# zijieli-Jlee/Temporal-Pointcloud-Upsampling-GAN

Measured on AMD Instinct MI355X. Metric: GAN train-steps/sec (G+D) on 4096-pt x3-frame clips, higher is better.
Workload: dtype bf16; 1 GPU; cfg2: 4096-pt x3-frame fluid clips, full G+D adversarial step (SRNet(3,128) + FluidTempoDis(3) + FluidSpatialDis, Adam), all-keep mask regime, gate open, even iteration; batch 8 per GPU; per_gpu_batch=8, global_batch=8, parallelism=dp1, step_mode=hipgraph (1 graph per step)

## Files before the change

include/tpgan_ops.h:

```cpp
#ifndef TPGAN_OPS_H
#define TPGAN_OPS_H

#include <stddef.h>
#include <stdint.h>

#ifdef __cplusplus
extern "C" {
#endif

typedef enum {
    TPG_OK = 0,
    TPG_ERR_ARG = -1,
    TPG_ERR_LAUNCH = -2,
    TPG_ERR_UNSUPPORTED = -3
} tpg_status;

#define TPG_MAX_K 64

const char *tpg_version(void);
const char *tpg_target_arch(void);

int tpg_knn_f32(const float *p1, const float *p2, const int64_t *len1,
                const int64_t *len2, int B, int P1, int P2, int D, int K,
                float r2, float *dist, int64_t *idx, void *stream);

int tpg_knn_grid_f32(const float *p1, const float *p2, const int64_t *len1, const int64_t *len2, int B,
                     int P1, int P2, int K, float *dist, int64_t *idx, void *ws, void *stream);

int tpg_knn_mfma_f32(const float *p1, const float *p2, const int64_t *len1,
                     const int64_t *len2, int B, int P1, int P2, int D, int K,
                     float *dist, int64_t *idx, int redo, void *stream);

size_t tpg_frnn_grid_workspace_bytes(int B, int P2);
int tpg_frnn_grid_f32(const float *p1, const float *p2, const int64_t *len1, const int64_t *len2, int B, int P1,
                      int P2, int K, float r, float *dist, int64_t *idx, void *ws, void *stream);

int tpg_chamfer_fwd_f32(const float *src, const float *tgt, int B, int N, int M,
                        float *d1, int64_t *i1, float *d2, int64_t *i2,
                        void *stream);
size_t tpg_chamfer_bwd_workspace_bytes(int B, int N, int M);
int tpg_chamfer_bwd_f32(const float *src, const float *tgt, int B, int N, int M,
                        const int64_t *i1, const int64_t *i2, const float *g1,
                        const float *g2, float *gsrc, float *gtgt, void *ws, void *stream);

int tpg_fps_f32(const float *xyz, int B, int N, int m, float *temp, int32_t *idx,
                void *stream);

int tpg_fps_prefix_f32(const float *xyz, int B, int N, int m, float *temp, int32_t *idx,
                       const int32_t *prefix_in, int32_t *prefix_out, void *stream);

int tpg_fps_start_f32(const float *xyz, const int32_t *start, int skip_origin, int B, int N, int m,
                      float *temp, int32_t *idx, void *stream);

int tpg_gather_fwd_f32(const float *feat, const int32_t *idx, int B, int C, int N,
                       int S, float *out, void *stream);
int tpg_gather_bwd_f32(const float *gout, const int32_t *idx, int B, int C, int N,
                       int S, float *gfeat, void *stream);

int tpg_gather_rows_fwd_f32(const float *rows, const int32_t *idx, int B, int N, int S, int C, float *out, void *stream);
int tpg_gather_rows_bwd_f32(const float *gout, const int32_t *idx, int B, int N, int S, int C, float *grows,
                            void *stream);

int tpg_ball_query_f32(const float *xyz, const float *new_xyz, int B, int N, int S,
                       float radius, int nsample, int32_t *idx, void *stream);

int tpg_group_fwd_f32(const float *feat, const int32_t *idx, int B, int C, int N,
                      int S, int K, float *out, void *stream);
int tpg_group_bwd_f32(const float *gout, const int32_t *idx, int B, int C, int N,
                      int S, int K, float *gfeat, void *stream);

int tpg_three_nn_f32(const float *unknown, const float *known, int B, int n, int m,
                     float *dist2, int32_t *idx, void *stream);
int tpg_three_interp_fwd_f32(const float *feat, const int32_t *idx, const float *w,
                             int B, int C, int m, int n, float *out, void *stream);
int tpg_three_interp_bwd_f32(const float *gout, const int32_t *idx, const float *w,
                             int B, int C, int m, int n, float *gfeat,
                             void *stream);

typedef enum { TPG_DTYPE_F32 = 0, TPG_DTYPE_BF16 = 1 } tpg_dtype;

int tpg_rowcombine_fwd(const void *U, const void *QE, const int32_t *idx, int mode, int dtype_in,
                       int dtype_out, int B, int N, int S, int K, int C, float slope, void *out,
                       void *stream);

int tpg_invert_index(const int32_t *idx, int B, int N, int SK, int32_t *offs, int32_t *list,
                     int32_t *tmp, void *stream);

int tpg_rowcombine_bwd(const void *gout, const int32_t *idx, const int32_t *offs, const int32_t *list,
                       const void *E, int mode, int dtype_in, int dtype_out, int B, int N, int S, int K,
                       int C, float slope, void *gU, void *gQE, void *stream);

int tpg_rowcombine_edge_fwd(const void *Y, const int32_t *idx, int dtype_in, int dtype_out, int B, int N, int K, int C,
                            float slope_a, float slope_e, void *out, void *stream);
int tpg_rowcombine_edge_bwd(const void *gout, const int32_t *idx, const int32_t *offs, const int32_t *list,
                            const void *Y, int dtype_in, int dtype_out, int B, int N, int K, int C, float slope_a,
                            float slope_e, void *gY, void *stream);

int tpg_head_bn_act_fwd(const float *h, int B, int C, const float *gamma, const float *beta, float *running_mean,
                        float *running_var, long long *num_batches_tracked, float momentum, float eps, float slope,
                        const float *mask, float *y, float *mean, float *rstd, void *stream);
int tpg_head_bn_act_bwd(const float *gy, const float *h, const float *mean, const float *rstd, const float *gamma,
                        const float *beta, float slope, const float *mask, int B, int C, float *dh, float *dgamma,
                        float *dbeta, void *stream);

#define TPG_BN_PHASE_ALL 0
#define TPG_BN_PHASE_STATS 1
#define TPG_BN_PHASE_APPLY 2
size_t tpg_rowbn_workspace_bytes(int C, int nseg);
int tpg_rowbn_fwd(const void *x, int dtype_in, long long P, int K, int C, float eps, float momentum,
                  int training, float *running_mean, float *running_var, long long *num_batches_tracked,
                  const float *mean_shift, const float *gamma, const float *beta, float slope, float *mean,
                  float *rstd, void *y,
                  int dtype_out, uint8_t *argmax, void *ws, int nseg, int phase, void *stream);
int tpg_rowbn_bwd(const void *gy, int dtype_g, const void *x, int dtype_in, const uint8_t *argmax,
                  const void *y, int dtype_y, long long P, int K, int C, int training, const float *mean,
                  const float *rstd, const float *gamma, const float *beta, float slope, float *dgamma,
                  float *dbeta, void *dx, void *ws, int nseg, int phase, void *stream);

int tpg_rowbn_bwd_sums(const void *gy, int dtype_g, const void *x, int dtype_in, const uint8_t *argmax,
                       const void *y, int dtype_y, long long P, int K, int C, int training, const float *mean,
                       const float *rstd, const float *gamma, const float *beta, float slope, float *dgamma,
                       float *dbeta, float *c12, void *ws, int nseg, void *stream);

int tpg_rowbn_stats_consts(const void *x, int dtype_in, long long P, int C, float eps, float momentum,
                           float *running_mean, float *running_var, long long *num_batches_tracked,
                           const float *mean_shift, const float *gamma, const float *beta, float *mean, float *rstd,
                           float *ci, void *ws, int nseg, void *stream);
int tpg_rowbn_bwd_sums_consts(const void *gy, int dtype_g, const void *x, int dtype_in, const uint8_t *argmax,
                              const void *y, int dtype_y, long long P, int K, int C, int training, const float *mean,
                              const float *rstd, const float *gamma, const float *beta, float slope, float *dgamma,
                              float *dbeta, float *c12, float *cb, void *ag, void *ws, int nseg, void *stream);

size_t tpg_mlp_workspace_bytes(int C, int nseg);
int tpg_mlp_fwd(const void *x, long long P, int Cin, int Cout, int nseg, const float *ss_in, int ss_stride,
                float slope_in, const float *W, int w_per_seg, void *y, float eps, float momentum,
                float *running_mean, float *running_var, long long *num_batches_tracked, const float *mean_shift,
                const float *gamma_out, const float *beta_out, float *mean_out, float *rstd_out, float *ci_out,
                void *ws, void *stream);

int tpg_mlp_consts(const float *mean, const float *rstd, const float *gamma, const float *beta, const float *c12,
                   int C, int nseg, float *ci, float *cb, void *stream);
int tpg_mlp_max_prep(const void *gout, const void *y, const float *cb_out, float slope_out, long long rows, int C,
                     int nseg, void *ag, void *stream);
int tpg_mlp_dgrad(const void *x_out, const void *g_out, const uint8_t *arg, int K, const float *cb_out,
                  const void *x_in, const float *ci_in, float slope_in, const float *W,
                  int w_per_seg, long long P, int Cin, int Cout, int nseg, int mode, void *g_in, float *c12_in,
                  float *dgamma_in, float *dbeta_in, float *cb_in, void *ws, void *stream);
size_t tpg_mlp_wgrad_workspace_bytes(long long P, int Cin, int Cout, int nseg);
int tpg_mlp_wgrad(const void *x_out, const void *g_out, const uint8_t *arg, int K, const float *cb_out,
                  const void *x_in, const float *ci_in, float slope_in, long long P, int Cin,
                  int Cout, int nseg, int mode, float *dW, void *ws, void *stream);
int tpg_mlp_bn_bwd_apply(const void *g, const void *x, const float *ci, const float *c12, long long P, int C,
                         int nseg, void *dx, void *stream);
int tpg_mlp_bn_bwd_apply_rowsum(const void *g, const void *x, const float *ci, const float *c12, long long P, int K,
                                int C, int nseg, void *dx, float *qneg, void *stream);

int tpg_spectral_norm_fwd(const float *W, float *u, float *v, int R, int Cn, int iterate, float eps,
                          float *Wsn, float *sigma, void *stream);
int tpg_spectral_norm_bwd(const float *G, const float *Wsn, const float *u, const float *v,
                          const float *sigma, int R, int Cn, float *dW, void *stream);

long long tpg_spectral_norm_multi_stride(int R, int Cn);
int tpg_spectral_norm_multi_fwd(const void *desc, int M, int max_rc, float *out, int iterate, float eps,
                                void *stream);
int tpg_spectral_norm_multi_fwd_split(const void *desc, const void *part_map, int total_parts, int max_cn, float *out,
                                      void *xws, long long xws_words, float eps, void *stream);
int tpg_spectral_norm_split_rows(void);
int tpg_spectral_norm_split_max_cn(void);
int tpg_spectral_norm_split_max_rows(void);
long long tpg_spectral_norm_multi_bwd_scratch(int M, int max_uses);
int tpg_spectral_norm_multi_bwd(const void *desc, int M, int max_uses, const float *g, const float *out,
                                float *dw, float *scratch, void *stream);

int tpg_cubic_interp_f32(const float *query, const float *pos, const float *field, int B, int Nq, int Np,
                         int F, float cutoff, float *out_plain, float *out_pad, int32_t *hits,
                         void *stream);

size_t tpg_small_tail_workspace_bytes(long long P, int K);
int tpg_small_tail_fwd(const void *h, int is_bf16, const float *W1, const float *W2, float slope1, float slope2,
                       long long P, int K, int H, int C1, int C2, void *out, unsigned char *arg, void *stream);
int tpg_small_tail_bwd(const void *h, const void *out, const void *gout, const unsigned char *arg, int is_bf16,
                       const float *W1, const float *W2, float slope1, float slope2, long long P, int K, int H,
                       int C1, int C2, void *gh, float *dW1, float *dW2, void *ws, void *stream);

int tpg_rowlinear_supported(int Cin, int Cout, int has_bias);
size_t tpg_rowlinear_wgrad_workspace_bytes(long long P, int nseg, int Cin, int Cout, int has_bias);
int tpg_rowlinear_fwd(const void *x, int dtype_in, const float *W, const float *bias, long long P, int nseg, int Cin,
                      int Cout, float slope, void *y, int dtype_out, void *stream);
int tpg_rowlinear_dgrad(const void *gy, const void *y, int dtype_g, const float *W, long long P, int nseg, int Cin,
                        int Cout, float slope, void *dx, int dtype_x, void *stream);
int tpg_rowlinear_wgrad(const void *x, int dtype_x, const void *gy, const void *y, int dtype_g, long long P, int nseg,
                        int Cin, int Cout, float slope, float *dW, float *db, void *ws, void *stream);

#define TPG_CTX_NONE (-2147483647 - 1)
size_t tpg_context_expand_workspace_bytes(int T, int N);
int tpg_context_expand_f32(const float *pos, const float *edge, const float *mask, int T, int N, int r, int t0,
                           int32_t *state, float *out, int64_t *offsets, void *ws, void *stream);

int tpg_radius_reduce_f32(const float *query, const float *pos, const int64_t *lenq, const int64_t *lenp, int B,
                          int Nq, int Np, float r, int kernel, int32_t *count, float *sum, void *ws, void *stream);
int tpg_radius_reduce_exhaustive_f32(const float *query, const float *pos, const int64_t *lenq, const int64_t *lenp,
                                     int B, int Nq, int Np, float r, int kernel, int32_t *count, float *sum,
                                     void *stream);

#define TPG_PATCH_SELECT_MAX_K 16384
int tpg_patch_select_max_k(void);
size_t tpg_patch_select_workspace_bytes(int B, int max_count, int K);
int tpg_patch_select_f32(const float *points, long long P, const int32_t *first, const int32_t *count,
                         const int32_t *seed, int B, int K, int32_t *idx, void *ws, void *stream);

int tpg_clip_gather_high_f32(const float *pos, const float *vel, long long P, const int32_t *frame_first,
                             const int32_t *count, const float *centroids, int F, const int32_t *centroid_row,
                             const int32_t *patch, int T, int B, int K, float *high_pos, float *high_vel, void *stream);

int tpg_clip_gather_low_f32(const float *high_pos, const int32_t *fps, const float *noise, float jitter,
                            const float *vel, long long P, const int32_t *frame_first, const int32_t *count, int T,
                            int B, int K, int M, float *low_pos, float *low_vel, void *stream);

#ifdef __cplusplus
}
#endif
#endif
```

temporal-pointcloud-upsampling-gan_amd/_lib.py:

```python
import ctypes as C
import os

_HERE = os.path.dirname(os.path.abspath(__file__))
LIB_PATH = os.environ.get("TPGAN_HIP_LIBRARY") or os.path.join(_HERE, "csrc", "libtpgan_hip.so")

_P = C.c_void_p
_I = C.c_int
_F = C.c_float
_L = C.c_longlong

SIGNATURES = {
    "tpg_knn_f32": [_P, _P, _P, _P, _I, _I, _I, _I, _I, _F, _P, _P, _P],
    "tpg_knn_mfma_f32": [_P, _P, _P, _P, _I, _I, _I, _I, _I, _P, _P, _I, _P],
    "tpg_knn_grid_f32": [_P, _P, _P, _P, _I, _I, _I, _I, _P, _P, _P, _P],
    "tpg_frnn_grid_f32": [_P, _P, _P, _P, _I, _I, _I, _I, _F, _P, _P, _P, _P],
    "tpg_chamfer_fwd_f32": [_P, _P, _I, _I, _I, _P, _P, _P, _P, _P],
    "tpg_chamfer_bwd_f32": [_P, _P, _I, _I, _I, _P, _P, _P, _P, _P, _P, _P, _P],
    "tpg_fps_f32": [_P, _I, _I, _I, _P, _P, _P],
    "tpg_fps_prefix_f32": [_P, _I, _I, _I, _P, _P, _P, _P, _P],
    "tpg_fps_start_f32": [_P, _P, _I, _I, _I, _I, _P, _P, _P],
    "tpg_gather_fwd_f32": [_P, _P, _I, _I, _I, _I, _P, _P],
    "tpg_gather_bwd_f32": [_P, _P, _I, _I, _I, _I, _P, _P],
    "tpg_ball_query_f32": [_P, _P, _I, _I, _I, _F, _I, _P, _P],
    "tpg_group_fwd_f32": [_P, _P, _I, _I, _I, _I, _I, _P, _P],
    "tpg_group_bwd_f32": [_P, _P, _I, _I, _I, _I, _I, _P, _P],
    "tpg_three_nn_f32": [_P, _P, _I, _I, _I, _P, _P, _P],
    "tpg_three_interp_fwd_f32": [_P, _P, _P, _I, _I, _I, _I, _P, _P],
    "tpg_three_interp_bwd_f32": [_P, _P, _P, _I, _I, _I, _I, _P, _P],
    "tpg_gather_rows_fwd_f32": [_P, _P, _I, _I, _I, _I, _P, _P],
    "tpg_gather_rows_bwd_f32": [_P, _P, _I, _I, _I, _I, _P, _P],
    "tpg_rowcombine_fwd": [_P, _P, _P, _I, _I, _I, _I, _I, _I, _I, _I, _F, _P, _P],
    "tpg_invert_index": [_P, _I, _I, _I, _P, _P, _P, _P],
    "tpg_rowcombine_bwd": [_P, _P, _P, _P, _P, _I, _I, _I, _I, _I, _I, _I, _I, _F, _P, _P, _P],
    "tpg_rowcombine_edge_fwd": [_P, _P, _I, _I, _I, _I, _I, _I, _F, _F, _P, _P],
    "tpg_rowcombine_edge_bwd": [_P, _P, _P, _P, _P, _I, _I, _I, _I, _I, _I, _F, _F, _P, _P],
    "tpg_head_bn_act_fwd": [_P, _I, _I, _P, _P, _P, _P, _P, _F, _F, _F, _P, _P, _P, _P, _P],
    "tpg_head_bn_act_bwd": [_P, _P, _P, _P, _P, _P, _F, _P, _I, _I, _P, _P, _P, _P],
    "tpg_rowbn_fwd": [_P, _I, _L, _I, _I, _F, _F, _I, _P, _P, _P, _P, _P, _P, _F, _P, _P, _P, _I, _P, _P, _I, _I, _P],
    "tpg_rowbn_bwd": [_P, _I, _P, _I, _P, _P, _I, _L, _I, _I, _I, _P, _P, _P, _P, _F, _P, _P, _P, _P, _I, _I, _P],
    "tpg_cubic_interp_f32": [_P, _P, _P, _I, _I, _I, _I, _F, _P, _P, _P, _P],
    "tpg_spectral_norm_fwd": [_P, _P, _P, _I, _I, _I, _F, _P, _P, _P],
    "tpg_spectral_norm_bwd": [_P, _P, _P, _P, _P, _I, _I, _P, _P],
    "tpg_spectral_norm_multi_fwd": [_P, _I, _I, _P, _I, _F, _P],
    "tpg_spectral_norm_multi_fwd_split": [_P, _P, _I, _I, _P, _P, _L, _F, _P],
    "tpg_spectral_norm_multi_bwd": [_P, _I, _I, _P, _P, _P, _P, _P],
    "tpg_rowbn_bwd_sums": [_P, _I, _P, _I, _P, _P, _I, _L, _I, _I, _I, _P, _P, _P, _P, _F, _P, _P, _P, _P, _I, _P],
    "tpg_rowbn_bwd_sums_consts": [_P, _I, _P, _I, _P, _P, _I, _L, _I, _I, _I, _P, _P, _P, _P, _F, _P, _P, _P, _P, _P, _P, _I, _P],
    "tpg_rowbn_stats_consts": [_P, _I, _L, _I, _F, _F, _P, _P, _P, _P, _P, _P, _P, _P, _P, _P, _I, _P],
    "tpg_mlp_consts": [_P, _P, _P, _P, _P, _I, _I, _P, _P, _P],
    "tpg_mlp_max_prep": [_P, _P, _P, _F, _L, _I, _I, _P, _P],
    "tpg_mlp_dgrad": [_P, _P, _P, _I, _P, _P, _P, _F, _P, _I, _L, _I, _I, _I, _I, _P, _P, _P, _P, _P, _P, _P],
    "tpg_mlp_wgrad": [_P, _P, _P, _I, _P, _P, _P, _F, _L, _I, _I, _I, _I, _P, _P, _P],
    "tpg_mlp_bn_bwd_apply": [_P, _P, _P, _P, _L, _I, _I, _P, _P],
    "tpg_mlp_bn_bwd_apply_rowsum": [_P, _P, _P, _P, _L, _I, _I, _I, _P, _P, _P],
    "tpg_small_tail_fwd": [_P, _I, _P, _P, _F, _F, _L, _I, _I, _I, _I, _P, _P, _P],
    "tpg_small_tail_bwd": [_P, _P, _P, _P, _I, _P, _P, _F, _F, _L, _I, _I, _I, _I, _P, _P, _P, _P, _P],
    "tpg_rowlinear_fwd": [_P, _I, _P, _P, _L, _I, _I, _I, _F, _P, _I, _P],
    "tpg_rowlinear_dgrad": [_P, _P, _I, _P, _L, _I, _I, _I, _F, _P, _I, _P],
    "tpg_rowlinear_wgrad": [_P, _I, _P, _P, _I, _L, _I, _I, _I, _F, _P, _P, _P, _P],
    "tpg_mlp_fwd": [_P, _L, _I, _I, _I, _P, _I, _F, _P, _I, _P, _F, _F, _P, _P, _P, _P, _P, _P, _P, _P, _P, _P, _P],
    "tpg_context_expand_f32": [_P, _P, _P, _I, _I, _I, _I, _P, _P, _P, _P, _P],
    "tpg_radius_reduce_f32": [_P, _P, _P, _P, _I, _I, _I, _F, _I, _P, _P, _P, _P],
    "tpg_radius_reduce_exhaustive_f32": [_P, _P, _P, _P, _I, _I, _I, _F, _I, _P, _P, _P],
    "tpg_patch_select_f32": [_P, _L, _P, _P, _P, _I, _I, _P, _P, _P],
    "tpg_clip_gather_high_f32": [_P, _P, _L, _P, _P, _P, _I, _P, _P, _I, _I, _I, _P, _P, _P],
    "tpg_clip_gather_low_f32": [_P, _P, _P, _F, _P, _L, _P, _P, _I, _I, _I, _I, _P, _P, _P],
}
SIZE_GETTERS = ("tpg_rowbn_workspace_bytes", "tpg_mlp_workspace_bytes", "tpg_context_expand_workspace_bytes")
OTHER_GETTERS = ("tpg_spectral_norm_multi_stride", "tpg_spectral_norm_multi_bwd_scratch",
                 "tpg_mlp_wgrad_workspace_bytes", "tpg_frnn_grid_workspace_bytes", "tpg_small_tail_workspace_bytes",
                 "tpg_chamfer_bwd_workspace_bytes", "tpg_rowlinear_wgrad_workspace_bytes", "tpg_rowlinear_supported",
                 "tpg_spectral_norm_split_rows", "tpg_spectral_norm_split_max_cn", "tpg_spectral_norm_split_max_rows",
                 "tpg_patch_select_workspace_bytes", "tpg_patch_select_max_k")
STRING_GETTERS = ("tpg_version", "tpg_target_arch")

STATUS = {0: "TPG_OK", -1: "TPG_ERR_ARG", -2: "TPG_ERR_LAUNCH", -3: "TPG_ERR_UNSUPPORTED"}

_lib = None


class HipLibraryMissing(RuntimeError):
    pass


def load():
    global _lib
    if _lib is not None:
        return _lib
    if not os.path.exists(LIB_PATH):
        raise HipLibraryMissing(
            f"{LIB_PATH} not found: build it with `python __graft_entry__.py` "
            "(hipcc --offload-arch=gfx950).  There is no CPU fallback.")
    lib = C.CDLL(LIB_PATH)
    for name, argtypes in SIGNATURES.items():
        fn = getattr(lib, name)
        fn.argtypes = argtypes
        fn.restype = C.c_int
    for name in STRING_GETTERS:
        getattr(lib, name).restype = C.c_char_p
    for name in SIZE_GETTERS:
        getattr(lib, name).argtypes = [C.c_int, C.c_int]
        getattr(lib, name).restype = C.c_size_t
    lib.tpg_spectral_norm_multi_stride.argtypes = [C.c_int, C.c_int]
    lib.tpg_spectral_norm_multi_stride.restype = C.c_longlong
    lib.tpg_spectral_norm_multi_bwd_scratch.argtypes = [C.c_int, C.c_int]
    lib.tpg_spectral_norm_multi_bwd_scratch.restype = C.c_longlong
    lib.tpg_mlp_wgrad_workspace_bytes.argtypes = [C.c_longlong, C.c_int, C.c_int, C.c_int]
    lib.tpg_mlp_wgrad_workspace_bytes.restype = C.c_size_t
    lib.tpg_small_tail_workspace_bytes.argtypes = [C.c_longlong, C.c_int]
    lib.tpg_small_tail_workspace_bytes.restype = C.c_size_t
    lib.tpg_frnn_grid_workspace_bytes.argtypes = [C.c_int, C.c_int]
    lib.tpg_frnn_grid_workspace_bytes.restype = C.c_size_t
    lib.tpg_chamfer_bwd_workspace_bytes.argtypes = [C.c_int, C.c_int, C.c_int]
    lib.tpg_chamfer_bwd_workspace_bytes.restype = C.c_size_t
    lib.tpg_rowlinear_wgrad_workspace_bytes.argtypes = [C.c_longlong, C.c_int, C.c_int, C.c_int, C.c_int]
    lib.tpg_rowlinear_wgrad_workspace_bytes.restype = C.c_size_t
    lib.tpg_patch_select_workspace_bytes.argtypes = [C.c_int, C.c_int, C.c_int]
    lib.tpg_patch_select_workspace_bytes.restype = C.c_size_t
    for name in ("tpg_spectral_norm_split_rows", "tpg_spectral_norm_split_max_cn", "tpg_spectral_norm_split_max_rows",
                 "tpg_patch_select_max_k"):
        getattr(lib, name).argtypes = []
        getattr(lib, name).restype = C.c_int
    lib.tpg_rowlinear_supported.argtypes = [C.c_int, C.c_int, C.c_int]
    lib.tpg_rowlinear_supported.restype = C.c_int
    _lib = lib
    return lib


def check(rc, name):
    if rc != 0:
        raise RuntimeError(f"{name} failed: {STATUS.get(rc, rc)}")
```

temporal-pointcloud-upsampling-gan_amd/csrc/mlp_fused.hip:

```cpp
#include "tpg_bn_finalize.hpp"
#include "tpg_rows.hpp"

namespace {

typedef __attribute__((ext_vector_type(8))) short bf16x8;

constexpr int ML_THREADS = 256;
constexpr int ML_WAVES = ML_THREADS / 64;
constexpr int ML_MAX_BLOCKS = 512;
constexpr int ML_WPAD = 8;

template <int COUT> __device__ __forceinline__ int w_lds_row(int n) {
    constexpr int T = COUT / 16;
    return (n % T) * 16 + n / T;
}

template <int CIN, int COUT, int STRIPS>
__global__ __launch_bounds__(ML_THREADS, 2) void mlp_fwd_kernel(
    const __hip_bfloat16 *__restrict__ x, long long P, const float *__restrict__ ss, int ss_stride, float slope,
    const float *__restrict__ W, int w_per_seg, __hip_bfloat16 *__restrict__ y, float *__restrict__ part) {
    constexpr int T = COUT / 16;
    constexpr int KS = CIN / 32;
    constexpr int BM = ML_WAVES * STRIPS * 16;
    constexpr int WROW = CIN + ML_WPAD;
    extern __shared__ __attribute__((aligned(16))) unsigned char ml_smem[];
    unsigned short *wl = reinterpret_cast<unsigned short *>(ml_smem);
    float *cst = reinterpret_cast<float *>(ml_smem + (size_t)COUT * WROW * 2);
    float *red = reinterpret_cast<float *>(ml_smem);
    const int tid = threadIdx.x, lane = tid & 63, wave = tid >> 6;
    const int li = lane & 15, lq = lane >> 4;
    const int seg = blockIdx.y;
    x += (size_t)seg * P * CIN;
    y += (size_t)seg * P * COUT;
    {
        const float *Ws = W + (w_per_seg ? (size_t)seg * COUT * CIN : 0);
        for (int e = tid; e < COUT * CIN / 4; e += ML_THREADS) {
            const int n = e / (CIN / 4), k = (e - n * (CIN / 4)) * 4;
            const float4 w4 = *reinterpret_cast<const float4 *>(Ws + (size_t)n * CIN + k);
            uint2 p;
            p.x = tpg_pack_bf16x2(w4.x, w4.y);
            p.y = tpg_pack_bf16x2(w4.z, w4.w);
            *reinterpret_cast<uint2 *>(wl + (size_t)w_lds_row<COUT>(n) * WROW + k) = p;
        }
        for (int c = tid; c < 2 * CIN; c += ML_THREADS)
            cst[c] = ss ? ss[(size_t)seg * ss_stride + c] : (c < CIN ? 1.0f : 0.0f);
    }
    __syncthreads();
    float piv[T], s1[T], s2[T];
#pragma unroll
    for (int t = 0; t < T; ++t) { piv[t] = 0.0f; s1[t] = 0.0f; s2[t] = 0.0f; }
    bool have_piv = false;
    float nrows = 0.0f;
    const long long ntiles = (P + BM - 1) / BM;
    const unsigned short *wfrag = wl + (size_t)li * WROW + 8 * lq;
    const float *csc = cst + 8 * lq, *csh = cst + CIN + 8 * lq;
    uint4 araw[STRIPS][KS];
    auto load_tile = [&](long long tile) {
#pragma unroll
        for (int st = 0; st < STRIPS; ++st) {
            long long row = tile * BM + (wave * STRIPS + st) * 16 + li;
            row = row < P ? row : P - 1;
            const __hip_bfloat16 *px = x + (size_t)row * CIN + 8 * lq;
#pragma unroll
            for (int s = 0; s < KS; ++s) araw[st][s] = *reinterpret_cast<const uint4 *>(px + 32 * s);
        }
    };
    long long tile = blockIdx.x;
    if (tile < ntiles) load_tile(tile);
    for (; tile < ntiles; tile += gridDim.x) {
        const long long row_base = tile * BM + (long long)wave * STRIPS * 16;
        tpg_f32x4 acc[STRIPS][T];
#pragma unroll
        for (int st = 0; st < STRIPS; ++st)
#pragma unroll
            for (int t = 0; t < T; ++t) acc[st][t] = tpg_f32x4{0.0f, 0.0f, 0.0f, 0.0f};
#pragma unroll
        for (int s = 0; s < KS; ++s) {
            float sc[8], sh[8];
            {
                const float4 a0 = *reinterpret_cast<const float4 *>(csc + 32 * s), a1 = *reinterpret_cast<const float4 *>(csc + 32 * s + 4);
                const float4 b0 = *reinterpret_cast<const float4 *>(csh + 32 * s), b1 = *reinterpret_cast<const float4 *>(csh + 32 * s + 4);
                sc[0] = a0.x; sc[1] = a0.y; sc[2] = a0.z; sc[3] = a0.w; sc[4] = a1.x; sc[5] = a1.y; sc[6] = a1.z; sc[7] = a1.w;
                sh[0] = b0.x; sh[1] = b0.y; sh[2] = b0.z; sh[3] = b0.w; sh[4] = b1.x; sh[5] = b1.y; sh[6] = b1.z; sh[7] = b1.w;
            }
            bf16x8 afrag[STRIPS];
#pragma unroll
            for (int st = 0; st < STRIPS; ++st) {
                const unsigned w[4] = {araw[st][s].x, araw[st][s].y, araw[st][s].z, araw[st][s].w};
                union { unsigned u[4]; bf16x8 v; } cv;
#pragma unroll
                for (int i = 0; i < 4; ++i) {
                    float a = __builtin_fmaf(tpg_bf16_lo(w[i]), sc[2 * i], sh[2 * i]);
                    float b = __builtin_fmaf(tpg_bf16_hi(w[i]), sc[2 * i + 1], sh[2 * i + 1]);
                    a = fmaxf(a, a * slope);
                    b = fmaxf(b, b * slope);
                    cv.u[i] = tpg_pack_bf16x2(a, b);
                }
                afrag[st] = cv.v;
            }
#pragma unroll
            for (int t = 0; t < T; ++t) {
                const bf16x8 b = *reinterpret_cast<const bf16x8 *>(wfrag + (size_t)t * 16 * WROW + 32 * s);
#pragma unroll
                for (int st = 0; st < STRIPS; ++st)
                    acc[st][t] = __builtin_amdgcn_mfma_f32_16x16x32_bf16(afrag[st], b, acc[st][t], 0, 0, 0);
                if ((t & 3) == 3) __builtin_amdgcn_sched_barrier(0);
            }
        }
        if (tile + gridDim.x < ntiles) load_tile(tile + gridDim.x);
        if (!have_piv) {
#pragma unroll
            for (int t = 0; t < T; ++t) {
                const float v = tpg_bf16_lo(tpg_pack_bf16x2(acc[0][t][0], 0.0f));
                piv[t] = __shfl(v, li, 64);
            }
            have_piv = true;
        }
#pragma unroll
        for (int st = 0; st < STRIPS; ++st)
#pragma unroll
            for (int r = 0; r < 4; ++r) {
                const long long row = row_base + st * 16 + 4 * lq + r;
                const bool valid = row < P;
                unsigned o[T / 2];
#pragma unroll
                for (int t = 0; t < T; t += 2) {
                    const unsigned w = tpg_pack_bf16x2(acc[st][t][r], acc[st][t + 1][r]);
                    o[t / 2] = w;
                    const float d0 = valid ? tpg_bf16_lo(w) - piv[t] : 0.0f;
                    const float d1 = valid ? tpg_bf16_hi(w) - piv[t + 1] : 0.0f;
                    s1[t] += d0;
                    s1[t + 1] += d1;
                    s2[t] = __builtin_fmaf(d0, d0, s2[t]);
                    s2[t + 1] = __builtin_fmaf(d1, d1, s2[t + 1]);
                }
                if (valid) {
                    __hip_bfloat16 *py = y + (size_t)row * COUT + li * T;
#pragma unroll
                    for (int v4 = 0; v4 < T / 8; ++v4)
                        reinterpret_cast<uint4 *>(py)[v4] = make_uint4(o[4 * v4], o[4 * v4 + 1], o[4 * v4 + 2], o[4 * v4 + 3]);
                    if constexpr (T == 4) *reinterpret_cast<uint2 *>(py) = make_uint2(o[0], o[1]);
                }
            }
        {
            const long long left = P - row_base;
            nrows += (float)(left <= 0 ? 0 : (left < STRIPS * 16 ? left : STRIPS * 16));
        }
    }
#pragma unroll
    for (int t = 0; t < T; ++t) {
        s1[t] += __shfl_xor(s1[t], 16, 64);
        s1[t] += __shfl_xor(s1[t], 32, 64);
        s2[t] += __shfl_xor(s2[t], 16, 64);
        s2[t] += __shfl_xor(s2[t], 32, 64);
    }
    __syncthreads();
    if (lq == 0) {
#pragma unroll
        for (int t = 0; t < T; ++t) {
            const int c = li * T + t;
            const float n = nrows;
            const float m = n > 0.0f ? s1[t] / n : 0.0f;
            red[(wave * 3 + 0) * COUT + c] = piv[t] + m;
            red[(wave * 3 + 1) * COUT + c] = n > 0.0f ? s2[t] - s1[t] * m : 0.0f;
            red[(wave * 3 + 2) * COUT + c] = n;
        }
    }
    __syncthreads();
    float *out = part + ((size_t)seg * gridDim.x + blockIdx.x) * 3 * COUT;
    for (int c = tid; c < COUT; c += ML_THREADS) {
        float n = 0.0f, mean = 0.0f, m2 = 0.0f;
#pragma unroll
        for (int w = 0; w < ML_WAVES; ++w) {
            const float nw = red[(w * 3 + 2) * COUT + c];
            if (nw > 0.0f) {
                const float mw = red[(w * 3 + 0) * COUT + c], qw = red[(w * 3 + 1) * COUT + c];
                const float tot = n + nw, delta = mw - mean;
                mean += delta * (nw / tot);
                m2 += qw + delta * delta * (n * nw / tot);
                n = tot;
            }
        }
        out[c] = mean;
        out[COUT + c] = m2;
        out[2 * COUT + c] = n;
    }
}

using tpg_bn::FIN_CH;
using tpg_bn::FIN_THREADS;
using tpg_bn::FIN_R;

__global__ __launch_bounds__(FIN_THREADS) void mlp_stats_finalize_kernel(
    const float *__restrict__ part, int G, int C, int nseg, float eps, float momentum,
    float *__restrict__ running_mean, float *__restrict__ running_var, long long *__restrict__ num_batches_tracked,
    const float *__restrict__ mean_shift, const float *__restrict__ gamma, const float *__restrict__ beta,
    float *__restrict__ mean, float *__restrict__ rstd, float *__restrict__ ci_out) {
    const int lane = threadIdx.x & 63;
    const int c = blockIdx.x * FIN_CH + (threadIdx.x >> 6);
    if (num_batches_tracked && blockIdx.x == 0 && threadIdx.x == 0) *num_batches_tracked += nseg;
    if (c >= C) return;
    const tpg_bn::Split sp = tpg_bn::split(nseg);
    const int grp = lane / sp.L, sub = lane - grp * sp.L;
    const bool fits = G <= sp.L * FIN_R;
    float rmean = running_mean ? running_mean[c] : 0.0f, rvar = running_mean ? running_var[c] : 0.0f;
    const double shift = mean_shift ? (double)mean_shift[c] : 0.0;
    for (int seg0 = 0; seg0 < nseg; seg0 += sp.SP) {
        const int seg = seg0 + grp;
        const bool live = seg < nseg;
        const float *ps = part + (size_t)(live ? seg : nseg - 1) * G * 3 * C + c;
        float pn[FIN_R], pm[FIN_R], pq[FIN_R];
        auto fetch = [&](int g0) {
#pragma unroll
            for (int i = 0; i < FIN_R; ++i) {
                const int g = g0 + sub + i * sp.L;
                const bool ok = live && g < G;
                const float *pg = ps + (size_t)(ok ? g : 0) * 3 * C;
                const float m_ = pg[0], q_ = pg[C], n_ = pg[2 * C];
                pm[i] = m_;
                pq[i] = q_;
                pn[i] = ok ? n_ : 0.0f;
            }
        };
        double n = 0.0, sm = 0.0;
        for (int g0 = 0; g0 < G; g0 += sp.L * FIN_R) {
            fetch(g0);
#pragma unroll
            for (int i = 0; i < FIN_R; ++i) {
                n += (double)pn[i];
                sm += (double)pn[i] * (double)pm[i];
            }
        }
        const double N = tpg_bn::group_sum(n, sp.L);
        const double m = N > 0.0 ? tpg_bn::group_sum(sm, sp.L) / N : 0.0;
        double q = 0.0;
        for (int g0 = 0; g0 < G; g0 += sp.L * FIN_R) {
            if (!fits) fetch(g0);
#pragma unroll
            for (int i = 0; i < FIN_R; ++i) {
                const double d = (double)pm[i] - m;
                q += pn[i] > 0.0f ? (double)pq[i] + (double)pn[i] * d * d : 0.0;
            }
        }
        double var = N > 0.0 ? tpg_bn::group_sum(q, sp.L) / N : 0.0;
        var = var < 0.0 ? 0.0 : var;
        const float mu = (float)m, rs = (float)(1.0 / sqrt(var + (double)eps));
        if (live && sub == 0) {
            if (mean) mean[(size_t)seg * C + c] = mu;
            if (rstd) rstd[(size_t)seg * C + c] = rs;
            if (ci_out) {
                const float a = (gamma ? gamma[c] : 1.0f) * rs;
                tpg_bn::write_ci(ci_out + (size_t)seg * 4 * C + c, C, a, beta ? beta[c] : 0.0f, mu, rs);
            }
        }
        if (running_mean) {
            const int last = nseg - seg0 < sp.SP ? nseg - seg0 : sp.SP;
            for (int k = 0; k < last; ++k) {
                const double Nk = tpg_bn::readlane(N, k * sp.L), mk = tpg_bn::readlane(m, k * sp.L), vk = tpg_bn::readlane(var, k * sp.L);
                const double unbiased = Nk > 1.0 ? vk * Nk / (Nk - 1.0) : vk;
                rmean = (float)((1.0 - momentum) * rmean + momentum * (mk + shift));
                rvar = (float)((1.0 - momentum) * rvar + momentum * unbiased);
            }
        }
    }
    if (running_mean && lane == 0) { running_mean[c] = rmean; running_var[c] = rvar; }
}

enum { MODE_DENSE = 0, MODE_MAX = 1 };

__device__ __forceinline__ void ld8(const float *p, float (&v)[8]) {
    const float4 a = *reinterpret_cast<const float4 *>(p), b = *reinterpret_cast<const float4 *>(p + 4);
    v[0] = a.x; v[1] = a.y; v[2] = a.z; v[3] = a.w; v[4] = b.x; v[5] = b.y; v[6] = b.z; v[7] = b.w;
}

template <int MODE>
__device__ __forceinline__ void d_out8(const uint4 xr, const uint4 gr, const uint2 ar, int k, const float (&a)[8],
                                       const float (&f)[8], const float (&fm)[8], unsigned (&o)[4]) {
    const unsigned xw[4] = {xr.x, xr.y, xr.z, xr.w}, gw[4] = {gr.x, gr.y, gr.z, gr.w};
#pragma unroll
    for (int i = 0; i < 4; ++i) {
        float v[2];
#pragma unroll
        for (int h = 0; h < 2; ++h) {
            const int j = 2 * i + h;
            const float x = h ? tpg_bf16_hi(xw[i]) : tpg_bf16_lo(xw[i]);
            const float g = h ? tpg_bf16_hi(gw[i]) : tpg_bf16_lo(gw[i]);
            const float c = __builtin_fmaf(-f[j], x, fm[j]);
            if (MODE == MODE_MAX) {
                const int ak = (int)__builtin_amdgcn_ubfe(j < 4 ? ar.x : ar.y, 8 * (j & 3), 8);
                v[h] = c + (ak == k ? g : 0.0f);
            } else {
                v[h] = __builtin_fmaf(a[j], g, c);
            }
        }
        o[i] = tpg_pack_bf16x2(v[0], v[1]);
    }
}

__global__ void mlp_max_prep_kernel(const __hip_bfloat16 *__restrict__ g, const __hip_bfloat16 *__restrict__ y,
                                    const float *__restrict__ cb, float slope, long long rows, int C,
                                    __hip_bfloat16 *__restrict__ ag) {
    const int seg = blockIdx.y;
    const long long n8 = rows * C / 8;
    const float *a = cb + (size_t)seg * 4 * C;
    for (long long i = (long long)blockIdx.x * blockDim.x + threadIdx.x; i < n8; i += (long long)gridDim.x * blockDim.x) {
        const size_t off = (size_t)seg * rows * C + (size_t)i * 8;
        const int c = (int)((i * 8) % C);
        const uint4 gv = *reinterpret_cast<const uint4 *>(g + off), yv = *reinterpret_cast<const uint4 *>(y + off);
        const unsigned gw[4] = {gv.x, gv.y, gv.z, gv.w}, yw[4] = {yv.x, yv.y, yv.z, yv.w};
        float av[8];
        ld8(a + c, av);
        unsigned o[4];
#pragma unroll
        for (int q = 0; q < 4; ++q) {
            const float g0 = tpg_bf16_lo(gw[q]), g1 = tpg_bf16_hi(gw[q]);
            const float v0 = av[2 * q] * (tpg_bf16_lo(yw[q]) > 0.0f ? g0 : g0 * slope);
            const float v1 = av[2 * q + 1] * (tpg_bf16_hi(yw[q]) > 0.0f ? g1 : g1 * slope);
            o[q] = tpg_pack_bf16x2(v0, v1);
        }
        *reinterpret_cast<uint4 *>(ag + off) = make_uint4(o[0], o[1], o[2], o[3]);
    }
}

template <int CIN, int COUT, int MODE, int STRIPS, int OCC>
__global__ __launch_bounds__(ML_THREADS, OCC) void mlp_dgrad_kernel(
    const __hip_bfloat16 *__restrict__ x_out, const __hip_bfloat16 *__restrict__ g_out,
    const uint8_t *__restrict__ arg, int K, const float *__restrict__ cbo,
    const __hip_bfloat16 *__restrict__ x_in, const float *__restrict__ cbi, float slope_in,
    const float *__restrict__ W, int w_per_seg, long long P, __hip_bfloat16 *__restrict__ g_in,
    float *__restrict__ part) {
    constexpr int TI = CIN / 16;
    constexpr int KS = COUT / 32;
    constexpr int BM = ML_WAVES * STRIPS * 16;
    constexpr int WROW = COUT + ML_WPAD;
    extern __shared__ __attribute__((aligned(16))) unsigned char ml_smem[];
    unsigned short *wl = reinterpret_cast<unsigned short *>(ml_smem);
    float *cst = reinterpret_cast<float *>(ml_smem + (size_t)CIN * WROW * 2);
    float *bias = cst + 4 * COUT;
    float *red = bias + CIN;
    const int tid = threadIdx.x, lane = tid & 63, wave = tid >> 6;
    const int li = lane & 15, lq = lane >> 4;
    const int seg = blockIdx.y;
    x_out += (size_t)seg * P * COUT;
    x_in += (size_t)seg * P * CIN;
    g_in += (size_t)seg * P * CIN;
    if (MODE == MODE_DENSE) g_out += (size_t)seg * P * COUT;
    else { g_out += (size_t)seg * (P / K) * COUT; arg += (size_t)seg * (P / K) * COUT; }
    {
        const float *Ws = W + (w_per_seg ? (size_t)seg * COUT * CIN : 0);
        for (int e = tid; e < COUT * CIN / 4; e += ML_THREADS) {
            const int n = e / (CIN / 4), k = (e - n * (CIN / 4)) * 4;
            const float4 w4 = *reinterpret_cast<const float4 *>(Ws + (size_t)n * CIN + k);
            const float wv[4] = {w4.x, w4.y, w4.z, w4.w};
#pragma unroll
            for (int i = 0; i < 4; ++i) wl[(size_t)w_lds_row<CIN>(k + i) * WROW + n] = tpg_bf16_bits(wv[i]);
        }
        const float *cb = cbo + (size_t)seg * 4 * COUT;
        for (int c = tid; c < COUT; c += ML_THREADS) {
            cst[c] = cb[c];
            cst[COUT + c] = cb[3 * COUT + c];
            cst[2 * COUT + c] = cb[2 * COUT + c];
            cst[3 * COUT + c] = cb[COUT + c];
        }
    }
    __syncthreads();
    for (int ci = tid; ci < CIN; ci += ML_THREADS) {
        const unsigned short *wr = wl + (size_t)w_lds_row<CIN>(ci) * WROW;
        float acc = 0.0f;
        for (int co = 0; co < COUT; ++co) acc = __builtin_fmaf(cst[2 * COUT + co], __uint_as_float((unsigned)wr[co] << 16), acc);
        bias[ci] = acc;
    }
    __syncthreads();
    float sc[TI], sh[TI], mu[TI], bi[TI], sg[TI], sgx[TI];
#pragma unroll
    for (int t = 0; t < TI; ++t) {
        const int c = li * TI + t;
        sc[t] = cbi[((size_t)seg * 4 + 0) * CIN + c];
        sh[t] = cbi[((size_t)seg * 4 + 1) * CIN + c];
        mu[t] = cbi[((size_t)seg * 4 + 2) * CIN + c];
        bi[t] = bias[c];
        sg[t] = 0.0f;
        sgx[t] = 0.0f;
    }
    const long long ntiles = (P + BM - 1) / BM;
    const unsigned short *wfrag = wl + (size_t)li * WROW + 8 * lq;
    uint4 xraw[STRIPS][KS], graw[STRIPS][KS];
    uint2 araw[STRIPS][KS];
    unsigned xin[STRIPS][4][TI / 2];
    constexpr bool DEFER = OCC == 1 && CIN == 128;
    unsigned xnext[DEFER ? STRIPS : 1][4][TI / 2];
    unsigned held[DEFER ? STRIPS : 1][4][TI / 2];
    long long held_base = -1;
    auto load_xin = [&](long long tile, unsigned (&xin)[STRIPS][4][TI / 2]) {
#pragma unroll
        for (int st = 0; st < STRIPS; ++st) {
#pragma unroll
            for (int r = 0; r < 4; ++r) {
                long long rr = tile * BM + (wave * STRIPS + st) * 16 + 4 * lq + r;
                rr = rr < P ? rr : P - 1;
                const __hip_bfloat16 *pi = x_in + (size_t)rr * CIN + li * TI;
                if constexpr (TI == 4) {
                    const uint2 v = *reinterpret_cast<const uint2 *>(pi);
                    xin[st][r][0] = v.x; xin[st][r][1] = v.y;
                } else {
#pragma unroll
                    for (int v4 = 0; v4 < TI / 8; ++v4) {
                        const uint4 v = reinterpret_cast<const uint4 *>(pi)[v4];
                        xin[st][r][4 * v4] = v.x; xin[st][r][4 * v4 + 1] = v.y; xin[st][r][4 * v4 + 2] = v.z; xin[st][r][4 * v4 + 3] = v.w;
                    }
                }
            }
        }
    };
    const __hip_bfloat16 *px[STRIPS], *pg[STRIPS];
    const uint8_t *pa[STRIPS];
    auto point_at = [&](long long tile) {
#pragma unroll
        for (int st = 0; st < STRIPS; ++st) {
            long long row = tile * BM + (wave * STRIPS + st) * 16 + li;
            row = row < P ? row : P - 1;
            px[st] = x_out + (size_t)row * COUT + 8 * lq;
            const long long grow = MODE == MODE_MAX ? (long long)((unsigned)row / (unsigned)K) : row;
            pg[st] = g_out + (size_t)grow * COUT + 8 * lq;
            pa[st] = MODE == MODE_MAX ? arg + (size_t)grow * COUT + 8 * lq : nullptr;
        }
    };
    auto load_step = [&](int st, int s) {
        xraw[st][s] = *reinterpret_cast<const uint4 *>(px[st] + 32 * s);
        graw[st][s] = *reinterpret_cast<const uint4 *>(pg[st] + 32 * s);
        if (MODE == MODE_MAX) araw[st][s] = *reinterpret_cast<const uint2 *>(pa[st] + 32 * s);
        else araw[st][s] = make_uint2(0u, 0u);
    };
    long long tile = blockIdx.x;
    if (tile < ntiles) {
        point_at(tile);
#pragma unroll
        for (int st = 0; st < STRIPS; ++st)
#pragma unroll
            for (int s = 0; s < KS; ++s) load_step(st, s);
        load_xin(tile, xin);
    }
    for (; tile < ntiles; tile += gridDim.x) {
        const long long row_base = tile * BM + (long long)wave * STRIPS * 16;
        const bool has_next = tile + gridDim.x < ntiles;
        const long long tnext = has_next ? tile + gridDim.x : tile;
        point_at(tnext);
        if constexpr (DEFER) load_xin(tnext, xnext);
        auto store_held = [&]() {
#pragma unroll
            for (int st = 0; st < STRIPS; ++st)
#pragma unroll
                for (int r = 0; r < 4; ++r) {
                    const long long row = held_base + st * 16 + 4 * lq + r;
                    if (row < P) {
                        __hip_bfloat16 *pgo = g_in + (size_t)row * CIN + li * TI;
#pragma unroll
                        for (int v4 = 0; v4 < TI / 8; ++v4)
                            reinterpret_cast<uint4 *>(pgo)[v4] = make_uint4(held[DEFER ? st : 0][r][4 * v4], held[DEFER ? st : 0][r][4 * v4 + 1],
                                                                            held[DEFER ? st : 0][r][4 * v4 + 2], held[DEFER ? st : 0][r][4 * v4 + 3]);
                    }
                }
        };
        tpg_f32x4 acc[STRIPS][TI];
#pragma unroll
        for (int st = 0; st < STRIPS; ++st)
#pragma unroll
            for (int t = 0; t < TI; ++t) acc[st][t] = tpg_f32x4{0.0f, 0.0f, 0.0f, 0.0f};
#pragma unroll
        for (int s = 0; s < KS; ++s) {
            float ca[8], cf[8], cfm[8];
            if (MODE == MODE_DENSE) ld8(cst + 32 * s + 8 * lq, ca);
            ld8(cst + COUT + 32 * s + 8 * lq, cf);
            ld8(cst + 3 * COUT + 32 * s + 8 * lq, cfm);
            bf16x8 afrag[STRIPS];
#pragma unroll
            for (int st = 0; st < STRIPS; ++st) {
                const long long row = row_base + st * 16 + li;
                union { unsigned u[4]; bf16x8 v; } cv;
                d_out8<MODE>(xraw[st][s], graw[st][s], araw[st][s], MODE == MODE_MAX ? (int)((unsigned)row % (unsigned)K) : 0, ca,
                             cf, cfm, cv.u);
                if (row >= P) { cv.u[0] = 0u; cv.u[1] = 0u; cv.u[2] = 0u; cv.u[3] = 0u; }
                afrag[st] = cv.v;
                load_step(st, s);
            }
#pragma unroll
            for (int t = 0; t < TI; ++t) {
                const bf16x8 b = *reinterpret_cast<const bf16x8 *>(wfrag + (size_t)t * 16 * WROW + 32 * s);
#pragma unroll
                for (int st = 0; st < STRIPS; ++st)
                    acc[st][t] = __builtin_amdgcn_mfma_f32_16x16x32_bf16(afrag[st], b, acc[st][t], 0, 0, 0);
                if ((t & 3) == 3) __builtin_amdgcn_sched_barrier(0);
            }
            if constexpr (DEFER) {
                if (s == 0 && held_base >= 0) store_held();
            }
        }
#pragma unroll
        for (int st = 0; st < STRIPS; ++st)
#pragma unroll
            for (int r = 0; r < 4; ++r) {
                const long long row = row_base + st * 16 + 4 * lq + r;
                const bool valid = row < P;
                const float vm = valid ? 1.0f : 0.0f;
                unsigned o[TI / 2];
#pragma unroll
                for (int t = 0; t < TI; t += 2) {
                    const float x0 = tpg_bf16_lo(xin[st][r][t / 2]), x1 = tpg_bf16_hi(xin[st][r][t / 2]);
                    const float z0 = __builtin_fmaf(x0, sc[t], sh[t]), z1 = __builtin_fmaf(x1, sc[t + 1], sh[t + 1]);
                    const float g0 = (acc[st][t][r] + bi[t]) * (z0 > 0.0f ? vm : vm * slope_in);
                    const float g1 = (acc[st][t + 1][r] + bi[t + 1]) * (z1 > 0.0f ? vm : vm * slope_in);
                    o[t / 2] = tpg_pack_bf16x2(g0, g1);
                    sg[t] += g0;
                    sg[t + 1] += g1;
                    sgx[t] = __builtin_fmaf(g0, x0 - mu[t], sgx[t]);
                    sgx[t + 1] = __builtin_fmaf(g1, x1 - mu[t + 1], sgx[t + 1]);
                }
                if constexpr (DEFER) {
#pragma unroll
                    for (int w = 0; w < TI / 2; ++w) held[st][r][w] = o[w];
                } else if (valid) {
                    __hip_bfloat16 *pgo = g_in + (size_t)row * CIN + li * TI;
#pragma unroll
                    for (int v4 = 0; v4 < TI / 8; ++v4)
                        reinterpret_cast<uint4 *>(pgo)[v4] = make_uint4(o[4 * v4], o[4 * v4 + 1], o[4 * v4 + 2], o[4 * v4 + 3]);
                    if constexpr (TI == 4) *reinterpret_cast<uint2 *>(pgo) = make_uint2(o[0], o[1]);
                }
            }
        if constexpr (DEFER) {
            held_base = row_base;
#pragma unroll
            for (int st = 0; st < STRIPS; ++st)
#pragma unroll
                for (int r = 0; r < 4; ++r)
#pragma unroll
                    for (int w = 0; w < TI / 2; ++w) xin[st][r][w] = xnext[st][r][w];
        } else {
            load_xin(tnext, xin);
        }
    }
    if constexpr (DEFER) {
        if (held_base >= 0) {
            auto store_last = [&]() {
#pragma unroll
                for (int st = 0; st < STRIPS; ++st)
#pragma unroll
                    for (int r = 0; r < 4; ++r) {
                        const long long row = held_base + st * 16 + 4 * lq + r;
                        if (row < P) {
                            __hip_bfloat16 *pgo = g_in + (size_t)row * CIN + li * TI;
#pragma unroll
                            for (int v4 = 0; v4 < TI / 8; ++v4)
                                reinterpret_cast<uint4 *>(pgo)[v4] = make_uint4(held[st][r][4 * v4], held[st][r][4 * v4 + 1], held[st][r][4 * v4 + 2], held[st][r][4 * v4 + 3]);
                        }
                    }
            };
            store_last();
        }
    }
#pragma unroll
    for (int t = 0; t < TI; ++t) {
        sg[t] += __shfl_xor(sg[t], 16, 64);
        sg[t] += __shfl_xor(sg[t], 32, 64);
        sgx[t] += __shfl_xor(sgx[t], 16, 64);
        sgx[t] += __shfl_xor(sgx[t], 32, 64);
    }
    if (lq == 0) {
#pragma unroll
        for (int t = 0; t < TI; ++t) {
            red[(wave * 2 + 0) * CIN + li * TI + t] = sg[t];
            red[(wave * 2 + 1) * CIN + li * TI + t] = sgx[t];
        }
    }
    __syncthreads();
    float *out = part + ((size_t)seg * gridDim.x + blockIdx.x) * 2 * CIN;
    for (int c = tid; c < 2 * CIN; c += ML_THREADS) {
        float v = 0.0f;
#pragma unroll
        for (int w = 0; w < ML_WAVES; ++w) v += red[w * 2 * CIN + c];
        out[c] = v;
    }
}

__global__ __launch_bounds__(FIN_THREADS) void mlp_bwd_finalize_kernel(const float *__restrict__ part, int G, long long P,
                                                                      int C, int nseg, const float *__restrict__ rstd,
                                                                      int rstd_stride, float *__restrict__ c12,
                                                                      float *__restrict__ dgamma,
                                                                      float *__restrict__ dbeta,
                                                                      const float *__restrict__ ci,
                                                                      float *__restrict__ cb) {
    const int lane = threadIdx.x & 63;
    const int c = blockIdx.x * FIN_CH + (threadIdx.x >> 6);
    if (c >= C) return;
    const tpg_bn::Split sp = tpg_bn::split(nseg);
    const int grp = lane / sp.L, sub = lane - grp * sp.L;
    double ts = 0.0, tsx = 0.0;
    for (int seg0 = 0; seg0 < nseg; seg0 += sp.SP) {
        const int seg = seg0 + grp;
        const bool live = seg < nseg;
        const int segc = live ? seg : nseg - 1;
        const float *ps = part + (size_t)segc * G * 2 * C + c;
        const float rs = rstd[(size_t)segc * rstd_stride + c];
        double s, sx;
        tpg_bn::pair_sums(ps, C, sub, sp.L, G, live, s, sx);
        sx *= (double)rs;
        const bool owner = live && sub == 0;
        ts += tpg_bn::wave_sum(owner ? s : 0.0);
        tsx += tpg_bn::wave_sum(owner ? sx : 0.0);
        if (owner) {
            const float c1 = (float)(s / (double)P), c2 = (float)(sx / (double)P);
            if (c12) {
                c12[((size_t)seg * 2 + 0) * C + c] = c1;
                c12[((size_t)seg * 2 + 1) * C + c] = c2;
            }
            if (cb) {
                const float *ip = ci + (size_t)seg * 4 * C + c;
                tpg_bn::write_cb(cb + (size_t)seg * 4 * C + c, C, ip[0], ip[2 * C], ip[3 * C], c1, c2);
            }
        }
    }
    if (lane == 0) {
        if (dbeta) dbeta[c] = (float)ts;
        if (dgamma) dgamma[c] = (float)tsx;
    }
}

__global__ void mlp_consts_kernel(const float *__restrict__ mean, const float *__restrict__ rstd,
                                  const float *__restrict__ gamma, const float *__restrict__ beta,
                                  const float *__restrict__ c12, int C, int nseg, float *__restrict__ ci,
                                  float *__restrict__ cb) {
    const int i = blockIdx.x * blockDim.x + threadIdx.x;
    if (i >= nseg * C) return;
    const int seg = i / C, c = i - seg * C;
    const float mu = mean[i], rs = rstd[i];
    const float a = (gamma ? gamma[c] : 1.0f) * rs;
    const float be = beta ? beta[c] : 0.0f;
    if (ci) tpg_bn::write_ci(ci + (size_t)seg * 4 * C + c, C, a, be, mu, rs);
    if (cb) {
        const float c1 = c12[((size_t)seg * 2 + 0) * C + c], c2 = c12[((size_t)seg * 2 + 1) * C + c];
        tpg_bn::write_cb(cb + (size_t)seg * 4 * C + c, C, a, mu, rs, c1, c2);
    }
}

constexpr int WG_ROWS = 64;
constexpr int WG_PAD = 8;

__device__ __forceinline__ bf16x8 tr_frag(const unsigned short *tile, int row_stride, int r0, int c0, int lane) {
    typedef __attribute__((ext_vector_type(4))) short s4;
    const int i = lane & 15, q = i >> 2, p = i & 3;
    const unsigned short *a0 = tile + (size_t)(r0 + q) * row_stride + c0 + 4 * p;
    const s4 lo = __builtin_amdgcn_ds_read_tr16_b64_v4i16((__attribute__((address_space(3))) s4 *)(a0));
    const s4 hi = __builtin_amdgcn_ds_read_tr16_b64_v4i16((__attribute__((address_space(3))) s4 *)(a0 + 4 * row_stride));
    bf16x8 f;
    f[0] = lo[0]; f[1] = lo[1]; f[2] = lo[2]; f[3] = lo[3];
    f[4] = hi[0]; f[5] = hi[1]; f[6] = hi[2]; f[7] = hi[3];
    return f;
}

template <int CIN, int COUT, int MODE, int OCC>
__global__ __launch_bounds__(ML_THREADS, OCC) void mlp_wgrad_kernel(
    const __hip_bfloat16 *__restrict__ x_out, const __hip_bfloat16 *__restrict__ g_out,
    const uint8_t *__restrict__ arg, int K, const float *__restrict__ cbo,
    const __hip_bfloat16 *__restrict__ x_in, const float *__restrict__ cbi, float slope_in, long long P,
    float *__restrict__ slab) {
    constexpr int MT = COUT / 16 / ML_WAVES;
    constexpr int NT = CIN / 16;
    constexpr int DROW = COUT + WG_PAD, AROW = CIN + WG_PAD;
    constexpr int DCH = COUT / 8, ACH = CIN / 8;
    constexpr int DN = WG_ROWS * DCH / ML_THREADS;
    constexpr int AN = WG_ROWS * ACH / ML_THREADS;
    constexpr int DR = ML_THREADS / DCH, AR = ML_THREADS / ACH;
    static_assert(MT >= 1 && DN >= 1 && AN >= 1, "tile shape");
    extern __shared__ __attribute__((aligned(16))) unsigned char ml_smem[];
    unsigned short *dxt = reinterpret_cast<unsigned short *>(ml_smem);
    unsigned short *at = dxt + (size_t)WG_ROWS * DROW;
    float *ssum = reinterpret_cast<float *>(at + (size_t)WG_ROWS * AROW);
    const int tid = threadIdx.x, lane = tid & 63, wave = tid >> 6;
    const int lq = lane >> 4, li = lane & 15;
    const int seg = blockIdx.y;
    x_out += (size_t)seg * P * COUT;
    x_in += (size_t)seg * P * CIN;
    if (MODE == MODE_DENSE) g_out += (size_t)seg * P * COUT;
    else { g_out += (size_t)seg * (P / K) * COUT; arg += (size_t)seg * (P / K) * COUT; }
    const int dch = tid % DCH, drow = tid / DCH, ach = tid % ACH, arow = tid / ACH;
    float ca[8], cf[8], cfm[8], sc[8], sh[8], asum[8];
    ld8(cbo + ((size_t)seg * 4 + 0) * COUT + 8 * dch, ca);
    ld8(cbo + ((size_t)seg * 4 + 3) * COUT + 8 * dch, cf);
    ld8(cbo + ((size_t)seg * 4 + 1) * COUT + 8 * dch, cfm);
    ld8(cbi + ((size_t)seg * 4 + 0) * CIN + 8 * ach, sc);
    ld8(cbi + ((size_t)seg * 4 + 1) * CIN + 8 * ach, sh);
#pragma unroll
    for (int i = 0; i < 8; ++i) asum[i] = 0.0f;
    tpg_f32x4 acc[MT][NT];
#pragma unroll
    for (int m = 0; m < MT; ++m)
#pragma unroll
        for (int n = 0; n < NT; ++n) acc[m][n] = tpg_f32x4{0.0f, 0.0f, 0.0f, 0.0f};
    const long long ntiles = (P + WG_ROWS - 1) / WG_ROWS;
    uint4 xr[DN], gr[DN], xi[AN];
    uint2 ar[DN];
    auto load_raw = [&](long long tile) {
        const long long r0 = tile * WG_ROWS;
#pragma unroll
        for (int i = 0; i < DN; ++i) {
            long long rr = r0 + drow + i * DR;
            rr = rr < P ? rr : P - 1;
            const long long grow = MODE == MODE_MAX ? (long long)((unsigned)rr / (unsigned)K) : rr;
            xr[i] = *reinterpret_cast<const uint4 *>(x_out + (size_t)rr * COUT + 8 * dch);
            gr[i] = *reinterpret_cast<const uint4 *>(g_out + (size_t)grow * COUT + 8 * dch);
            ar[i] = MODE == MODE_MAX ? *reinterpret_cast<const uint2 *>(arg + (size_t)grow * COUT + 8 * dch) : make_uint2(0u, 0u);
        }
#pragma unroll
        for (int i = 0; i < AN; ++i) {
            long long rr = r0 + arow + i * AR;
            rr = rr < P ? rr : P - 1;
            xi[i] = *reinterpret_cast<const uint4 *>(x_in + (size_t)rr * CIN + 8 * ach);
        }
    };
    long long tile = blockIdx.x;
    if (tile < ntiles) load_raw(tile);
    for (; tile < ntiles; tile += gridDim.x) {
        const long long r0 = tile * WG_ROWS;
#pragma unroll
        for (int i = 0; i < DN; ++i) {
            const int r = drow + i * DR;
            const long long row = r0 + r;
            unsigned o[4];
            d_out8<MODE>(xr[i], gr[i], ar[i], MODE == MODE_MAX ? (int)((unsigned)(row < P ? row : P - 1) % (unsigned)K) : 0, ca, cf, cfm, o);
            if (row >= P) { o[0] = 0u; o[1] = 0u; o[2] = 0u; o[3] = 0u; }
            *reinterpret_cast<uint4 *>(dxt + (size_t)r * DROW + 8 * dch) = make_uint4(o[0], o[1], o[2], o[3]);
        }
#pragma unroll
        for (int i = 0; i < AN; ++i) {
            const int r = arow + i * AR;
            const bool valid = r0 + r < P;
            const unsigned xw[4] = {xi[i].x, xi[i].y, xi[i].z, xi[i].w};
            unsigned o[4];
#pragma unroll
            for (int q = 0; q < 4; ++q) {
                float a = __builtin_fmaf(tpg_bf16_lo(xw[q]), sc[2 * q], sh[2 * q]);
                float b = __builtin_fmaf(tpg_bf16_hi(xw[q]), sc[2 * q + 1], sh[2 * q + 1]);
                a = fmaxf(a, a * slope_in);
                b = fmaxf(b, b * slope_in);
                o[q] = valid ? tpg_pack_bf16x2(a, b) : 0u;
                asum[2 * q] += tpg_bf16_lo(o[q]);
                asum[2 * q + 1] += tpg_bf16_hi(o[q]);
            }
            *reinterpret_cast<uint4 *>(at + (size_t)r * AROW + 8 * ach) = make_uint4(o[0], o[1], o[2], o[3]);
        }
        __syncthreads();
        if (tile + gridDim.x < ntiles) load_raw(tile + gridDim.x);
#pragma unroll
        for (int ks = 0; ks < WG_ROWS / 32; ++ks) {
            bf16x8 af[MT];
#pragma unroll
            for (int m = 0; m < MT; ++m) af[m] = tr_frag(dxt, DROW, 32 * ks + 8 * lq, 16 * (wave * MT + m), lane);
#pragma unroll
            for (int n = 0; n < NT; ++n) {
                const bf16x8 bfr = tr_frag(at, AROW, 32 * ks + 8 * lq, 16 * n, lane);
#pragma unroll
                for (int m = 0; m < MT; ++m)
                    acc[m][n] = __builtin_amdgcn_mfma_f32_16x16x32_bf16(af[m], bfr, acc[m][n], 0, 0, 0);
                if ((n & 3) == 3) __builtin_amdgcn_sched_barrier(0);
            }
        }
        __syncthreads();
    }
#pragma unroll
    for (int i = 0; i < 8; ++i) ssum[(size_t)arow * CIN + 8 * ach + i] = asum[i];
    __syncthreads();
    float sv[NT];
#pragma unroll
    for (int n = 0; n < NT; ++n) {
        float t = 0.0f;
        for (int r = 0; r < AR; ++r) t += ssum[(size_t)r * CIN + 16 * n + li];
        sv[n] = t;
    }
    float *out = slab + ((size_t)seg * gridDim.x + blockIdx.x) * COUT * CIN;
    const float *ce = cbo + ((size_t)seg * 4 + 2) * COUT;
#pragma unroll
    for (int m = 0; m < MT; ++m)
#pragma unroll
        for (int r = 0; r < 4; ++r) {
            const int co = 16 * (wave * MT + m) + 4 * lq + r;
            const float e = ce[co];
#pragma unroll
            for (int n = 0; n < NT; ++n) out[(size_t)co * CIN + 16 * n + li] = __builtin_fmaf(e, sv[n], acc[m][n][r]);
        }
}

__global__ __launch_bounds__(256) void mlp_wgrad_reduce_kernel(const float *__restrict__ slab, int G, int n,
                                                                float *__restrict__ dW) {
    __shared__ float4 part[4][64];
    const int seg = blockIdx.y, col = threadIdx.x & 63, grp = threadIdx.x >> 6;
    const int i = (blockIdx.x * 64 + col) * 4;
    float4 s = make_float4(0.0f, 0.0f, 0.0f, 0.0f);
    if (i < n) {
        const float *ps = slab + (size_t)seg * G * n + i;
#pragma unroll 4
        for (int g = grp; g < G; g += 4) {
            const float4 v = *reinterpret_cast<const float4 *>(ps + (size_t)g * n);
            s.x += v.x; s.y += v.y; s.z += v.z; s.w += v.w;
        }
    }
    part[grp][col] = s;
    __syncthreads();
    if (grp == 0 && i < n) {
        float4 t = part[0][col];
#pragma unroll
        for (int q = 1; q < 4; ++q) { t.x += part[q][col].x; t.y += part[q][col].y; t.z += part[q][col].z; t.w += part[q][col].w; }
        *reinterpret_cast<float4 *>(dW + (size_t)seg * n + i) = t;
    }
}

__global__ __launch_bounds__(ML_THREADS) void mlp_bn_bwd_apply_kernel(
    const __hip_bfloat16 *__restrict__ g, const __hip_bfloat16 *__restrict__ x, long long P, int C,
    const float *__restrict__ ci, const float *__restrict__ c12, __hip_bfloat16 *__restrict__ dx) {
    const int cpr = C / 8, rpi = ML_THREADS / cpr;
    const int chunk = threadIdx.x % cpr, rsub = threadIdx.x / cpr, col = chunk * 8;
    if (rsub >= rpi) return;
    const int seg = blockIdx.y;
    g += (size_t)seg * P * C;
    x += (size_t)seg * P * C;
    dx += (size_t)seg * P * C;
    float a[8], mu[8], rs[8], c1[8], c2[8];
    ld8(ci + ((size_t)seg * 4 + 0) * C + col, a);
    ld8(ci + ((size_t)seg * 4 + 2) * C + col, mu);
    ld8(ci + ((size_t)seg * 4 + 3) * C + col, rs);
    ld8(c12 + ((size_t)seg * 2 + 0) * C + col, c1);
    ld8(c12 + ((size_t)seg * 2 + 1) * C + col, c2);
    float e[8], f[8];
#pragma unroll
    for (int i = 0; i < 8; ++i) {
        f[i] = a[i] * rs[i] * c2[i];
        e[i] = a[i] * (mu[i] * rs[i] * c2[i] - c1[i]);
    }
    const long long step = (long long)gridDim.x * rpi;
    long long r = (long long)blockIdx.x * rpi + rsub;
    for (; r + 3 * step < P; r += 4 * step) {
        uint4 gv[4], xv[4];
#pragma unroll
        for (int u = 0; u < 4; ++u) {
            gv[u] = *reinterpret_cast<const uint4 *>(g + (size_t)(r + u * step) * C + col);
            xv[u] = *reinterpret_cast<const uint4 *>(x + (size_t)(r + u * step) * C + col);
        }
#pragma unroll
        for (int u = 0; u < 4; ++u) {
            const unsigned gw[4] = {gv[u].x, gv[u].y, gv[u].z, gv[u].w}, xw[4] = {xv[u].x, xv[u].y, xv[u].z, xv[u].w};
            unsigned o[4];
#pragma unroll
            for (int i = 0; i < 4; ++i) {
                const float v0 = __builtin_fmaf(a[2 * i], tpg_bf16_lo(gw[i]), __builtin_fmaf(-f[2 * i], tpg_bf16_lo(xw[i]), e[2 * i]));
                const float v1 = __builtin_fmaf(a[2 * i + 1], tpg_bf16_hi(gw[i]), __builtin_fmaf(-f[2 * i + 1], tpg_bf16_hi(xw[i]), e[2 * i + 1]));
                o[i] = tpg_pack_bf16x2(v0, v1);
            }
            *reinterpret_cast<uint4 *>(dx + (size_t)(r + u * step) * C + col) = make_uint4(o[0], o[1], o[2], o[3]);
        }
    }
    for (; r < P; r += step) {
        const uint4 gv = *reinterpret_cast<const uint4 *>(g + (size_t)r * C + col);
        const uint4 xv = *reinterpret_cast<const uint4 *>(x + (size_t)r * C + col);
        const unsigned gw[4] = {gv.x, gv.y, gv.z, gv.w}, xw[4] = {xv.x, xv.y, xv.z, xv.w};
        unsigned o[4];
#pragma unroll
        for (int i = 0; i < 4; ++i) {
            const float v0 = __builtin_fmaf(a[2 * i], tpg_bf16_lo(gw[i]), __builtin_fmaf(-f[2 * i], tpg_bf16_lo(xw[i]), e[2 * i]));
            const float v1 = __builtin_fmaf(a[2 * i + 1], tpg_bf16_hi(gw[i]), __builtin_fmaf(-f[2 * i + 1], tpg_bf16_hi(xw[i]), e[2 * i + 1]));
            o[i] = tpg_pack_bf16x2(v0, v1);
        }
        *reinterpret_cast<uint4 *>(dx + (size_t)r * C + col) = make_uint4(o[0], o[1], o[2], o[3]);
    }
}

__global__ __launch_bounds__(ML_THREADS) void mlp_bn_bwd_apply_rowsum_kernel(
    const __hip_bfloat16 *__restrict__ g, const __hip_bfloat16 *__restrict__ x, long long P, int K, int C,
    const float *__restrict__ ci, const float *__restrict__ c12, __hip_bfloat16 *__restrict__ dx,
    float *__restrict__ qneg) {
    const int cpr = C / 8, gpi = ML_THREADS / cpr;
    const int chunk = threadIdx.x % cpr, gsub = threadIdx.x / cpr, col = chunk * 8;
    if (gsub >= gpi) return;
    const int seg = blockIdx.y;
    const long long groups = P / K;
    g += (size_t)seg * P * C;
    x += (size_t)seg * P * C;
    dx += (size_t)seg * P * C;
    qneg += (size_t)seg * groups * C;
    float a[8], mu[8], rs[8], c1[8], c2[8];
    ld8(ci + ((size_t)seg * 4 + 0) * C + col, a);
    ld8(ci + ((size_t)seg * 4 + 2) * C + col, mu);
    ld8(ci + ((size_t)seg * 4 + 3) * C + col, rs);
    ld8(c12 + ((size_t)seg * 2 + 0) * C + col, c1);
    ld8(c12 + ((size_t)seg * 2 + 1) * C + col, c2);
    float e[8], f[8];
#pragma unroll
    for (int i = 0; i < 8; ++i) {
        f[i] = a[i] * rs[i] * c2[i];
        e[i] = a[i] * (mu[i] * rs[i] * c2[i] - c1[i]);
    }
    for (long long s = (long long)blockIdx.x * gpi + gsub; s < groups; s += (long long)gridDim.x * gpi) {
        const size_t base = (size_t)s * K * C + col;
        float acc[8];
#pragma unroll
        for (int i = 0; i < 8; ++i) acc[i] = 0.0f;
        auto one = [&](const uint4 gv, const uint4 xv, size_t off) {
            const unsigned gw[4] = {gv.x, gv.y, gv.z, gv.w}, xw[4] = {xv.x, xv.y, xv.z, xv.w};
            unsigned o[4];
#pragma unroll
            for (int i = 0; i < 4; ++i) {
                const float v0 = __builtin_fmaf(a[2 * i], tpg_bf16_lo(gw[i]), __builtin_fmaf(-f[2 * i], tpg_bf16_lo(xw[i]), e[2 * i]));
                const float v1 = __builtin_fmaf(a[2 * i + 1], tpg_bf16_hi(gw[i]), __builtin_fmaf(-f[2 * i + 1], tpg_bf16_hi(xw[i]), e[2 * i + 1]));
                o[i] = tpg_pack_bf16x2(v0, v1);
                acc[2 * i] -= tpg_bf16_lo(o[i]);
                acc[2 * i + 1] -= tpg_bf16_hi(o[i]);
            }
            *reinterpret_cast<uint4 *>(dx + off) = make_uint4(o[0], o[1], o[2], o[3]);
        };
        int k = 0;
        for (; k + 4 <= K; k += 4) {
            uint4 gv[4], xv[4];
#pragma unroll
            for (int u = 0; u < 4; ++u) {
                gv[u] = *reinterpret_cast<const uint4 *>(g + base + (size_t)(k + u) * C);
                xv[u] = *reinterpret_cast<const uint4 *>(x + base + (size_t)(k + u) * C);
            }
#pragma unroll
            for (int u = 0; u < 4; ++u) one(gv[u], xv[u], base + (size_t)(k + u) * C);
        }
        for (; k < K; ++k)
            one(*reinterpret_cast<const uint4 *>(g + base + (size_t)k * C), *reinterpret_cast<const uint4 *>(x + base + (size_t)k * C),
                base + (size_t)k * C);
        float *q = qneg + (size_t)s * C + col;
        *reinterpret_cast<float4 *>(q) = make_float4(acc[0], acc[1], acc[2], acc[3]);
        *reinterpret_cast<float4 *>(q + 4) = make_float4(acc[4], acc[5], acc[6], acc[7]);
    }
}

template <int CIN, int COUT> constexpr int fwd_strips() {
    return (COUT <= 128 && CIN <= 128) ? 2 : 1;
}
template <int CIN, int COUT> constexpr size_t fwd_smem() {
    constexpr size_t w = (size_t)COUT * (CIN + ML_WPAD) * 2, red = sizeof(float) * ML_WAVES * 3 * COUT;
    return (w > red ? w : red) + sizeof(float) * 2 * CIN;
}

int fwd_blocks(long long P, int bm, int nseg, int slots = ML_MAX_BLOCKS) {
    const long long tiles = (P + bm - 1) / bm;
    long long cap = slots / nseg;
    if (cap < 16) cap = 16;
    return (int)(tiles < cap ? tiles : cap);
}

template <int CIN, int COUT>
int fwd_launch(const void *x, long long P, int nseg, const float *ss, int ss_stride, float slope, const float *W,
               int w_per_seg, void *y, float *part, int *G_out, hipStream_t st) {
    constexpr int STRIPS = fwd_strips<CIN, COUT>();
    constexpr int BM = ML_WAVES * STRIPS * 16;
    constexpr size_t smem = fwd_smem<CIN, COUT>();
    constexpr auto kern = mlp_fwd_kernel<CIN, COUT, STRIPS>;
    if (smem > 64 * 1024 && !tpg_allow_dynamic_lds<kern>((int)smem)) return TPG_ERR_UNSUPPORTED;
    const int G = fwd_blocks(P, BM, nseg, 2 * smem > 160 * 1024 ? 256 : 512);
    *G_out = G;
    hipLaunchKernelGGL(kern, dim3(G, nseg), dim3(ML_THREADS), smem, st, static_cast<const __hip_bfloat16 *>(x), P, ss,
                       ss_stride, slope, W, w_per_seg, static_cast<__hip_bfloat16 *>(y), part);
    return TPG_OK;
}

template <int CIN, int COUT> constexpr int bwd_strips() { return (CIN == 64 && COUT <= 128) ? 2 : 1; }
template <int CIN, int COUT> constexpr size_t dgrad_smem() {
    return (size_t)CIN * (COUT + ML_WPAD) * 2 + sizeof(float) * (4 * COUT + CIN + ML_WAVES * 2 * CIN);
}
template <int CIN, int COUT> constexpr size_t wgrad_smem() {
    return (size_t)WG_ROWS * ((COUT + WG_PAD) + (CIN + WG_PAD)) * 2 + sizeof(float) * (ML_THREADS / (CIN / 8)) * CIN;
}

template <int CIN, int COUT, int MODE>
int dgrad_launch(const void *x_out, const void *g_out, const uint8_t *arg, int K, const float *cbo,
                 const void *x_in, const float *cbi, float slope_in, const float *W, int w_per_seg, long long P, int nseg,
                 void *g_in, float *part, int *G_out, hipStream_t st) {
    constexpr int STRIPS = bwd_strips<CIN, COUT>();
    constexpr int BM = ML_WAVES * STRIPS * 16;
    constexpr size_t smem = dgrad_smem<CIN, COUT>();
    constexpr int OCC = (smem > 60 * 1024 || CIN == 256) ? 1 : 2;
    constexpr auto kern = mlp_dgrad_kernel<CIN, COUT, MODE, STRIPS, OCC>;
    if (smem > 64 * 1024 && !tpg_allow_dynamic_lds<kern>((int)smem)) return TPG_ERR_UNSUPPORTED;
    const int G = fwd_blocks(P, BM, nseg, OCC == 1 ? 256 : 512);
    *G_out = G;
    hipLaunchKernelGGL(kern, dim3(G, nseg), dim3(ML_THREADS), smem, st, static_cast<const __hip_bfloat16 *>(x_out),
                       static_cast<const __hip_bfloat16 *>(g_out), arg, K, cbo,
                       static_cast<const __hip_bfloat16 *>(x_in), cbi, slope_in, W, w_per_seg, P,
                       static_cast<__hip_bfloat16 *>(g_in), part);
    return TPG_OK;
}

int wgrad_blocks(long long P, int nseg, int Cin, int Cout) {
    const long long tiles = (P + WG_ROWS - 1) / WG_ROWS;
    const int d = nseg > 4 ? 4 : nseg;
    long long g = P * (Cin + Cout) / (8LL * Cin * Cout);
    const long long lo = 256 / d, hi = 768 / d;
    g = g < lo ? lo : (g > hi ? hi : g);
    const long long slots = ((long long)Cout * Cin / ML_THREADS >= 128) ? 256 : 512;
    long long k = g * nseg / slots;
    if (k < 1) k = 1;
    g = k * slots / nseg;
    if (g < 1) g = 1;
    return (int)(g < tiles ? g : tiles);
}

template <int CIN, int COUT, int MODE>
int wgrad_launch(const void *x_out, const void *g_out, const uint8_t *arg, int K, const float *cbo,
                 const void *x_in, const float *cbi, float slope_in, long long P, int nseg, float *slab, int G,
                 hipStream_t st) {
    constexpr size_t smem = wgrad_smem<CIN, COUT>();
    constexpr int OCC = (COUT * CIN / ML_THREADS >= 128) ? 1 : 2;
    constexpr auto kern = mlp_wgrad_kernel<CIN, COUT, MODE, OCC>;
    if (smem > 64 * 1024 && !tpg_allow_dynamic_lds<kern>((int)smem)) return TPG_ERR_UNSUPPORTED;
    hipLaunchKernelGGL(kern, dim3(G, nseg), dim3(ML_THREADS), smem, st, static_cast<const __hip_bfloat16 *>(x_out),
                       static_cast<const __hip_bfloat16 *>(g_out), arg, K, cbo,
                       static_cast<const __hip_bfloat16 *>(x_in), cbi, slope_in, P, slab);
    return TPG_OK;
}

bool ml_shape_ok(int Cin, int Cout) {
    return (Cin == 64 || Cin == 128 || Cin == 256) && (Cout == 64 || Cout == 128 || Cout == 256) &&
           !(Cin == 64 && Cout == 256) && !(Cin == 256 && Cout == 64);
}

}

#define TPG_ML_SHAPES(X) X(64, 64) X(64, 128) X(128, 64) X(128, 128) X(128, 256) X(256, 128) X(256, 256)

extern "C" size_t tpg_mlp_workspace_bytes(int C, int nseg) {
    if (nseg < 1) nseg = 1;
    return sizeof(float) * ((size_t)nseg * ML_MAX_BLOCKS * 3 * C + 64);
}

extern "C" int tpg_mlp_fwd(const void *x, long long P, int Cin, int Cout, int nseg, const float *ss_in, int ss_stride,
                           float slope_in, const float *W, int w_per_seg, void *y, float eps, float momentum,
                           float *running_mean, float *running_var, long long *num_batches_tracked,
                           const float *mean_shift, const float *gamma_out, const float *beta_out, float *mean_out,
                           float *rstd_out, float *ci_out, void *ws, void *stream) {
    if (P <= 0 || nseg < 1 || nseg > 65535 || P % nseg) return TPG_ERR_ARG;
    if (!x || !W || !y || !ws || (ss_in && ss_stride < 2 * Cin)) return TPG_ERR_ARG;
    if ((reinterpret_cast<uintptr_t>(x) | reinterpret_cast<uintptr_t>(y) | reinterpret_cast<uintptr_t>(W) |
         reinterpret_cast<uintptr_t>(ws)) & 15)
        return TPG_ERR_UNSUPPORTED;
    P /= nseg;
    hipStream_t st = tpg_stream(stream);
    float *part = static_cast<float *>(ws);
    int G = 0, rc = TPG_ERR_UNSUPPORTED;
#define TPG_ML_FWD(CI, CO)                                                                                 \
    if (Cin == CI && Cout == CO)                                                                           \
        rc = fwd_launch<CI, CO>(x, P, nseg, ss_in, ss_stride, slope_in, W, w_per_seg, y, part, &G, st);
    TPG_ML_SHAPES(TPG_ML_FWD)
#undef TPG_ML_FWD
    if (rc) return rc;
    if (mean_out || rstd_out || ci_out || running_mean)
        hipLaunchKernelGGL(mlp_stats_finalize_kernel, dim3((Cout + FIN_CH - 1) / FIN_CH), dim3(FIN_THREADS), 0, st, part, G,
                           Cout, nseg, eps, momentum, running_mean, running_var, num_batches_tracked, mean_shift,
                           gamma_out, beta_out, mean_out, rstd_out, ci_out);
    TPG_RETURN_IF_LAUNCH_FAILED();
    return TPG_OK;
}

extern "C" int tpg_mlp_consts(const float *mean, const float *rstd, const float *gamma, const float *beta,
                              const float *c12, int C, int nseg, float *ci, float *cb, void *stream) {
    if (C <= 0 || nseg < 1 || !mean || !rstd || (!ci && !cb) || (cb && !c12)) return TPG_ERR_ARG;
    const int n = nseg * C;
    hipLaunchKernelGGL(mlp_consts_kernel, dim3((n + 255) / 256), dim3(256), 0, tpg_stream(stream), mean, rstd, gamma,
                       beta, c12, C, nseg, ci, cb);
    TPG_RETURN_IF_LAUNCH_FAILED();
    return TPG_OK;
}

extern "C" int tpg_mlp_max_prep(const void *gout, const void *y, const float *cb_out, float slope_out, long long rows,
                                int C, int nseg, void *ag, void *stream) {
    if (rows <= 0 || nseg < 1 || nseg > 65535 || rows % nseg || C <= 0 || C % 8 || !gout || !y || !cb_out || !ag)
        return TPG_ERR_ARG;
    if ((reinterpret_cast<uintptr_t>(gout) | reinterpret_cast<uintptr_t>(y) | reinterpret_cast<uintptr_t>(ag)) & 15)
        return TPG_ERR_UNSUPPORTED;
    rows /= nseg;
    const long long n8 = rows * C / 8;
    long long b = (n8 + 255) / 256;
    b = b > 1024 ? 1024 : b;
    hipLaunchKernelGGL(mlp_max_prep_kernel, dim3((unsigned)b, nseg), dim3(256), 0, tpg_stream(stream),
                       static_cast<const __hip_bfloat16 *>(gout), static_cast<const __hip_bfloat16 *>(y), cb_out,
                       slope_out, rows, C, static_cast<__hip_bfloat16 *>(ag));
    TPG_RETURN_IF_LAUNCH_FAILED();
    return TPG_OK;
}

extern "C" int tpg_mlp_dgrad(const void *x_out, const void *g_out, const uint8_t *arg, int K, const float *cb_out,
                             const void *x_in, const float *ci_in, float slope_in, const float *W,
                             int w_per_seg, long long P, int Cin, int Cout, int nseg, int mode, void *g_in,
                             float *c12_in, float *dgamma_in, float *dbeta_in, float *cb_in, void *ws, void *stream) {
    if (P <= 0 || nseg < 1 || nseg > 65535 || P % nseg || (mode != MODE_DENSE && mode != MODE_MAX)) return TPG_ERR_ARG;
    if (!x_out || !g_out || !cb_out || !x_in || !ci_in || !W || !g_in || !ws) return TPG_ERR_ARG;
    P /= nseg;
    if (mode == MODE_MAX && (!arg || K <= 0 || K > 256 || P % K)) return TPG_ERR_ARG;
    if (P >= 0x7fffffffLL || !ml_shape_ok(Cin, Cout)) return TPG_ERR_UNSUPPORTED;
    if ((reinterpret_cast<uintptr_t>(x_out) | reinterpret_cast<uintptr_t>(g_out) | reinterpret_cast<uintptr_t>(x_in) |
         reinterpret_cast<uintptr_t>(g_in) | reinterpret_cast<uintptr_t>(W) | reinterpret_cast<uintptr_t>(ws) |
         reinterpret_cast<uintptr_t>(arg)) & 7)
        return TPG_ERR_UNSUPPORTED;
    hipStream_t st = tpg_stream(stream);
    float *part = static_cast<float *>(ws);
    int G = 0, rc = TPG_ERR_UNSUPPORTED;
#define TPG_ML_DG(CI, CO)                                                                                            \
    if (Cin == CI && Cout == CO)                                                                                     \
        rc = mode == MODE_MAX ? dgrad_launch<CI, CO, MODE_MAX>(x_out, g_out, arg, K, cb_out, x_in, ci_in,   \
                                                               slope_in, W, w_per_seg, P, nseg, g_in, part, &G, st)  \
                              : dgrad_launch<CI, CO, MODE_DENSE>(x_out, g_out, arg, K, cb_out, x_in, ci_in, \
                                                                 slope_in, W, w_per_seg, P, nseg, g_in, part, &G, st);
    TPG_ML_SHAPES(TPG_ML_DG)
#undef TPG_ML_DG
    if (rc) return rc;
    if (c12_in || dgamma_in || dbeta_in || cb_in)
        hipLaunchKernelGGL(mlp_bwd_finalize_kernel, dim3((Cin + FIN_CH - 1) / FIN_CH), dim3(FIN_THREADS), 0, st, part, G, P,
                           Cin, nseg, ci_in + 3 * Cin, 4 * Cin, c12_in, dgamma_in, dbeta_in, ci_in, cb_in);
    TPG_RETURN_IF_LAUNCH_FAILED();
    return TPG_OK;
}

extern "C" size_t tpg_mlp_wgrad_workspace_bytes(long long P, int Cin, int Cout, int nseg) {
    if (nseg < 1 || P <= 0) return 0;
    const int G = wgrad_blocks(P / nseg, nseg, Cin, Cout);
    return sizeof(float) * (size_t)G * nseg * Cin * Cout;
}

extern "C" int tpg_mlp_wgrad(const void *x_out, const void *g_out, const uint8_t *arg, int K, const float *cb_out,
                             const void *x_in, const float *ci_in, float slope_in, long long P, int Cin,
                             int Cout, int nseg, int mode, float *dW, void *ws, void *stream) {
    if (P <= 0 || nseg < 1 || nseg > 65535 || P % nseg || (mode != MODE_DENSE && mode != MODE_MAX)) return TPG_ERR_ARG;
    if (!x_out || !g_out || !cb_out || !x_in || !ci_in || !dW || !ws) return TPG_ERR_ARG;
    P /= nseg;
    if (mode == MODE_MAX && (!arg || K <= 0 || K > 256 || P % K)) return TPG_ERR_ARG;
    if (P >= 0x7fffffffLL || !ml_shape_ok(Cin, Cout)) return TPG_ERR_UNSUPPORTED;
    if ((reinterpret_cast<uintptr_t>(x_out) | reinterpret_cast<uintptr_t>(g_out) | reinterpret_cast<uintptr_t>(x_in) |
         reinterpret_cast<uintptr_t>(dW) | reinterpret_cast<uintptr_t>(ws) | reinterpret_cast<uintptr_t>(arg)) & 7)
        return TPG_ERR_UNSUPPORTED;
    hipStream_t st = tpg_stream(stream);
    float *slab = static_cast<float *>(ws);
    const int G = wgrad_blocks(P, nseg, Cin, Cout);
    int rc = TPG_ERR_UNSUPPORTED;
#define TPG_ML_WG(CI, CO)                                                                                           \
    if (Cin == CI && Cout == CO)                                                                                    \
        rc = mode == MODE_MAX ? wgrad_launch<CI, CO, MODE_MAX>(x_out, g_out, arg, K, cb_out, x_in, ci_in,  \
                                                               slope_in, P, nseg, slab, G, st)                      \
                              : wgrad_launch<CI, CO, MODE_DENSE>(x_out, g_out, arg, K, cb_out, x_in, ci_in, \
                                                                 slope_in, P, nseg, slab, G, st);
    TPG_ML_SHAPES(TPG_ML_WG)
#undef TPG_ML_WG
    if (rc) return rc;
    const int n = Cin * Cout;
    hipLaunchKernelGGL(mlp_wgrad_reduce_kernel, dim3((n / 4 + 63) / 64, nseg), dim3(256), 0, st, slab, G, n, dW);
    TPG_RETURN_IF_LAUNCH_FAILED();
    return TPG_OK;
}

extern "C" int tpg_mlp_bn_bwd_apply(const void *g, const void *x, const float *ci, const float *c12, long long P, int C,
                                    int nseg, void *dx, void *stream) {
    if (P <= 0 || nseg < 1 || nseg > 65535 || P % nseg || !g || !x || !ci || !c12 || !dx) return TPG_ERR_ARG;
    if (C <= 0 || C % 8 || C > 2048) return TPG_ERR_UNSUPPORTED;
    if ((reinterpret_cast<uintptr_t>(g) | reinterpret_cast<uintptr_t>(x) | reinterpret_cast<uintptr_t>(dx)) & 15)
        return TPG_ERR_UNSUPPORTED;
    P /= nseg;
    const int rpi = ML_THREADS / (C / 8);
    long long b = (P + (long long)rpi * 8 - 1) / ((long long)rpi * 8);
    const long long cap = 512 / (nseg > 4 ? 4 : nseg);
    b = b < 1 ? 1 : (b > cap ? cap : b);
    hipLaunchKernelGGL(mlp_bn_bwd_apply_kernel, dim3((unsigned)b, nseg), dim3(ML_THREADS), 0, tpg_stream(stream),
                       static_cast<const __hip_bfloat16 *>(g), static_cast<const __hip_bfloat16 *>(x), P, C, ci, c12,
                       static_cast<__hip_bfloat16 *>(dx));
    TPG_RETURN_IF_LAUNCH_FAILED();
    return TPG_OK;
}

extern "C" int tpg_mlp_bn_bwd_apply_rowsum(const void *g, const void *x, const float *ci, const float *c12, long long P,
                                           int K, int C, int nseg, void *dx, float *qneg, void *stream) {
    if (P <= 0 || K <= 0 || nseg < 1 || nseg > 65535 || P % nseg || (P / nseg) % K || !g || !x || !ci || !c12 || !dx || !qneg)
        return TPG_ERR_ARG;
    if (C <= 0 || C % 8 || C > 2048) return TPG_ERR_UNSUPPORTED;
    if ((reinterpret_cast<uintptr_t>(g) | reinterpret_cast<uintptr_t>(x) | reinterpret_cast<uintptr_t>(dx) |
         reinterpret_cast<uintptr_t>(qneg)) & 15)
        return TPG_ERR_UNSUPPORTED;
    P /= nseg;
    const int gpi = ML_THREADS / (C / 8);
    long long b = (P / K + gpi - 1) / gpi;
    static const long long slots = [] { const char *e = getenv("TPG_BNROWSUM_SLOTS"); return e ? atoll(e) : 1024ll; }();
    const long long cap = slots / nseg > 0 ? slots / nseg : 1;
    b = b < 1 ? 1 : (b > cap ? cap : b);
    hipLaunchKernelGGL(mlp_bn_bwd_apply_rowsum_kernel, dim3((unsigned)b, nseg), dim3(ML_THREADS), 0, tpg_stream(stream),
                       static_cast<const __hip_bfloat16 *>(g), static_cast<const __hip_bfloat16 *>(x), P, K, C, ci, c12,
                       static_cast<__hip_bfloat16 *>(dx), qneg);
    TPG_RETURN_IF_LAUNCH_FAILED();
    return TPG_OK;
}
```

temporal-pointcloud-upsampling-gan_amd/ops.py:

```python
import ctypes as C

import os

import numpy as np
import torch

from . import _lib

_BACKENDS = {}


class OpTimer:

    def __init__(self):
        self.pending = {}

    def record(self, name, nbytes, stream_of, launch, flops=0):
        st = torch.cuda.current_stream(stream_of.device)
        a = torch.cuda.Event(enable_timing=True)
        b = torch.cuda.Event(enable_timing=True)
        a.record(st)
        out = launch()
        b.record(st)
        self.pending.setdefault(name, []).append((a, b, nbytes, flops))
# ... 282 lines not shown
                   _ptr(rows), _ptr(idx), B, N, S, Cc, _ptr(out))
        return out

    def gather_rows_bwd(self, gout, idx, N):
        B, S, Cc = gout.shape
        g = torch.empty((B, N, Cc), dtype=torch.float32, device=gout.device)
        self._call("tpg_gather_rows_bwd_f32", "gather_bwd", 4 * B * (Cc * N + S + 2 * Cc * S), gout,
                   _ptr(gout), _ptr(idx), B, N, S, Cc, _ptr(g))
        return g

    def ball_query(self, radius, nsample, xyz, new_xyz):
        B, N, _ = xyz.shape
        S = new_xyz.shape[1]
        idx = torch.empty((B, S, nsample), dtype=torch.int32, device=xyz.device)
        self._call("tpg_ball_query_f32", "ball_query", 12 * B * (N + S) + 4 * B * S * nsample, xyz,
                   _ptr(xyz), _ptr(new_xyz), B, N, S, float(radius), nsample, _ptr(idx))
        return idx

    def group_fwd(self, feat, idx):
        B, Cc, N = feat.shape
        _, S, K = idx.shape
        out = torch.empty((B, Cc, S, K), dtype=torch.float32, device=feat.device)
        self._call("tpg_group_fwd_f32", "group_fwd", 4 * B * (Cc * N + S * K + Cc * S * K), feat,
                   _ptr(feat), _ptr(idx), B, Cc, N, S, K, _ptr(out))
        return out

    def group_bwd(self, gout, idx, N):
        B, Cc, S, K = gout.shape
        g = torch.empty((B, Cc, N), dtype=torch.float32, device=gout.device)
        self._call("tpg_group_bwd_f32", "group_bwd", 4 * B * (Cc * N + S * K + Cc * S * K), gout,
                   _ptr(gout), _ptr(idx), B, Cc, N, S, K, _ptr(g))
        return g

    def three_nn(self, unknown, known):
        B, n, _ = unknown.shape
        m = known.shape[1]
        d2 = torch.empty((B, n, 3), dtype=torch.float32, device=unknown.device)
        idx = torch.empty((B, n, 3), dtype=torch.int32, device=unknown.device)
        self._call("tpg_three_nn_f32", "three_nn", 12 * B * (n + m) + 24 * B * n, unknown,
                   _ptr(unknown), _ptr(known), B, n, m, _ptr(d2), _ptr(idx))
        return d2, idx

    def three_interp_fwd(self, feat, idx, w):
        B, Cc, m = feat.shape
        n = idx.shape[1]
        out = torch.empty((B, Cc, n), dtype=torch.float32, device=feat.device)
        self._call("tpg_three_interp_fwd_f32", "three_interp_fwd", 4 * B * (Cc * m + 6 * n + Cc * n), feat,
                   _ptr(feat), _ptr(idx), _ptr(w), B, Cc, m, n, _ptr(out))
        return out

    def three_interp_bwd(self, gout, idx, w, m):
        B, Cc, n = gout.shape
        g = torch.empty((B, Cc, m), dtype=torch.float32, device=gout.device)
        self._call("tpg_three_interp_bwd_f32", "three_interp_bwd", 4 * B * (Cc * m + 6 * n + Cc * n), gout,
                   _ptr(gout), _ptr(idx), _ptr(w), B, Cc, m, n, _ptr(g))
        return g

    def rowcombine_fwd(self, U, QE, idx, mode, slope, out_dtype):
        B, N, Cc = U.shape
        _, S, K = idx.shape
        out = torch.empty((B, S, K, Cc), dtype=out_dtype, device=U.device)
        nbytes = (U.element_size() * B * Cc * (N + (S if QE is not None else 0)) + 4 * B * S * K
                  + out.element_size() * B * S * K * Cc)
        self._call("tpg_rowcombine_fwd", "rowcombine_fwd", nbytes, U,
                   _ptr(U), _ptr(QE), _ptr(idx), mode, _DTYPE_CODE[U.dtype], _DTYPE_CODE[out_dtype],
                   B, N, S, K, Cc, float(slope), _ptr(out))
        return out

    def invert_index(self, idx, N):
        B = idx.shape[0]
        SK = idx[0].numel()
        offs = torch.empty((B, N + 1), dtype=torch.int32, device=idx.device)
        lst = torch.empty((B, SK), dtype=torch.int32, device=idx.device)
        tmp = torch.empty((B, SK), dtype=torch.int32, device=idx.device) if N > 256 else None
        self._call("tpg_invert_index", "invert_index", 4 * B * (2 * SK + N + 1), idx,
                   _ptr(idx), B, N, SK, _ptr(offs), _ptr(lst), _ptr(tmp))
        return offs, lst

    def rowcombine_bwd(self, gout, idx, E, mode, N, slope, in_dtype, inverse=None):
        B, S, K, Cc = gout.shape
        if inverse is None:
            inverse = self.invert_index(idx, N)
        offs, lst = inverse
        gU = torch.empty((B, N, Cc), dtype=in_dtype, device=gout.device)
        gQE = torch.empty((B, S, Cc), dtype=in_dtype, device=gout.device) if mode != 0 else None
        nbytes = (gout.element_size() * B * S * K * Cc * (2 if mode == 1 else 1) + 8 * B * S * K
                  + gU.element_size() * B * Cc * (N + (S if mode else 0)))
        self._call("tpg_rowcombine_bwd", "rowcombine_bwd", nbytes, gout,
                   _ptr(gout), _ptr(idx), _ptr(offs), _ptr(lst), _ptr(E), mode, _DTYPE_CODE[in_dtype],
                   _DTYPE_CODE[gout.dtype], B, N, S, K, Cc, float(slope), _ptr(gU), _ptr(gQE))
        return gU, gQE


    def rowcombine_edge_fwd(self, Y, idx, slope_a, slope_e, out_dtype):
        B, N, C2 = Y.shape
        Cc, K = C2 // 2, idx.shape[2]
        out = torch.empty((B, N, K, Cc), dtype=out_dtype, device=Y.device)
        nbytes = Y.element_size() * B * N * C2 + 4 * B * N * K + out.element_size() * B * N * K * Cc
        self._call("tpg_rowcombine_edge_fwd", "rowcombine_fwd", nbytes, Y,
                   _ptr(Y), _ptr(idx), _DTYPE_CODE[Y.dtype], _DTYPE_CODE[out_dtype], B, N, K, Cc, float(slope_a),
                   float(slope_e), _ptr(out))
        return out

    def rowcombine_edge_bwd(self, gout, idx, Y, slope_a, slope_e, inverse=None):
        B, N, K, Cc = gout.shape
        if inverse is None:
            inverse = self.invert_index(idx, N)
        offs, lst = inverse
        gY = torch.empty_like(Y)
        nbytes = gout.element_size() * B * N * K * Cc * 2 + 8 * B * N * K + 2 * Y.element_size() * B * N * 2 * Cc
        self._call("tpg_rowcombine_edge_bwd", "rowcombine_bwd", nbytes, gout,
                   _ptr(gout), _ptr(idx), _ptr(offs), _ptr(lst), _ptr(Y), _DTYPE_CODE[Y.dtype], _DTYPE_CODE[gout.dtype],
                   B, N, K, Cc, float(slope_a), float(slope_e), _ptr(gY))
        return gY

    def head_bn_act_fwd(self, h, gamma, beta, running_mean, running_var, nbt, momentum, eps, slope, mask):
        B, Cc = h.shape
        y = torch.empty_like(h)
        mean = torch.empty(Cc, dtype=torch.float32, device=h.device)
        rstd = torch.empty(Cc, dtype=torch.float32, device=h.device)
        self._call("tpg_head_bn_act_fwd", "head_bn_act", 4 * B * Cc * (3 if mask is not None else 2), h,
                   _ptr(h), B, Cc, _ptr(gamma), _ptr(beta), _ptr(running_mean), _ptr(running_var), _ptr(nbt),
                   float(momentum), float(eps), float(slope), _ptr(mask), _ptr(y), _ptr(mean), _ptr(rstd))
        return y, mean, rstd

    def head_bn_act_bwd(self, gy, h, mean, rstd, gamma, beta, slope, mask, need_affine):
        B, Cc = h.shape
        dh = torch.empty_like(h)
        dg = torch.empty(Cc, dtype=torch.float32, device=h.device) if need_affine else None
        db = torch.empty(Cc, dtype=torch.float32, device=h.device) if need_affine else None
        self._call("tpg_head_bn_act_bwd", "head_bn_act_bwd", 4 * B * Cc * (4 if mask is not None else 3), h,
                   _ptr(gy), _ptr(h), _ptr(mean), _ptr(rstd), _ptr(gamma), _ptr(beta), float(slope), _ptr(mask), B, Cc,
                   _ptr(dh), _ptr(dg), _ptr(db))
        return dh, dg, db

    def _bn_ws(self, x, C_, nseg=1):
        need = self.lib.tpg_rowbn_workspace_bytes(max(C_, 256), max(nseg, 1)) // 4
        return self._workspace("rowbn", x, need, zeroed=True)

    def rowbn_fwd(self, x, K, eps, momentum, training, running_mean, running_var, gamma, beta, slope,
                  mean, rstd, out_dtype, num_batches_tracked=None, nseg=1, mean_shift=None):
        P, Cc = x.shape
        rows = P // K if K else P
        y = torch.empty((rows, Cc), dtype=out_dtype, device=x.device)
        arg = torch.empty((rows, Cc), dtype=torch.uint8, device=x.device) if K else None
        ws = self._bn_ws(x, Cc, nseg)
        args = (_ptr(x), _DTYPE_CODE[x.dtype], P, K, Cc, float(eps), float(momentum), int(training),
                _ptr(running_mean), _ptr(running_var), _ptr(num_batches_tracked), _ptr(mean_shift), _ptr(gamma),
                _ptr(beta),
                float(slope), _ptr(mean),
                _ptr(rstd), _ptr(y), _DTYPE_CODE[out_dtype], _ptr(arg), _ptr(ws), int(nseg))
        b_stats = x.element_size() * P * Cc
        b_apply = x.element_size() * P * Cc + y.element_size() * rows * Cc + (rows * Cc if K else 0)
        if _timer is None:
            self._call("tpg_rowbn_fwd", "rowbn_fwd", b_stats + b_apply, x, *args, 0)
        else:
            if training:
                self._call("tpg_rowbn_fwd", "rowbn_fwd_stats", b_stats, x, *args, 1)
            self._call("tpg_rowbn_fwd", "rowbn_fwd_apply_max" if K else "rowbn_fwd_apply", b_apply, x, *args, 2)
        return y, arg

    def rowbn_bwd(self, gy, x, arg, K, training, mean, rstd, gamma, beta, slope, need_affine, y=None, nseg=1):
        P, Cc = x.shape
        dx = torch.empty_like(x)
        dgamma = torch.empty(Cc, dtype=torch.float32, device=x.device) if need_affine else None
        dbeta = torch.empty(Cc, dtype=torch.float32, device=x.device) if need_affine else None
        ws = self._bn_ws(x, Cc, nseg)
        if y is not None and (not K or y.dtype != gy.dtype):
            y = None
        args = (_ptr(gy), _DTYPE_CODE[gy.dtype], _ptr(x), _DTYPE_CODE[x.dtype], _ptr(arg), _ptr(y),
                _DTYPE_CODE[y.dtype] if y is not None else 0, P, K, Cc,
                int(training), _ptr(mean), _ptr(rstd), _ptr(gamma), _ptr(beta), float(slope), _ptr(dgamma),
                _ptr(dbeta), _ptr(dx), _ptr(ws), int(nseg))
        b_gy = gy.element_size() * gy.numel() + (gy.numel() if K else 0)
        b_reduce = (2 * gy.element_size() * gy.numel() if y is not None
                    else b_gy + x.element_size() * (gy.numel() if K else P * Cc))
        b_apply = b_gy + 2 * x.element_size() * P * Cc
        if _timer is None:
            self._call("tpg_rowbn_bwd", "rowbn_bwd", b_reduce + b_apply, x, *args, 0)
        else:
            self._call("tpg_rowbn_bwd", "rowbn_bwd_reduce", b_reduce, x, *args, 1)
            self._call("tpg_rowbn_bwd", "rowbn_bwd_apply", b_apply, x, *args, 2)
        return dx, dgamma, dbeta


    def _mlp_ws(self, x, C_, nseg):
        need = self.lib.tpg_mlp_workspace_bytes(max(C_, 256), max(nseg, 1)) // 4
        return self._workspace("mlp", x, need, zeroed=True)

    def mlp_fwd(self, x, ss_in, slope_in, W, nseg, eps=0.0, momentum=0.0, running_mean=None, running_var=None,
                num_batches_tracked=None, mean_shift=None, gamma_out=None, beta_out=None, stats=True, mean_rstd=False):
        P, Cin = x.shape
        w_per_seg = int(W.dim() == 3 and W.shape[0] == nseg and nseg > 1)
        Cout = W.shape[-2]
        y = torch.empty((P, Cout), dtype=torch.bfloat16, device=x.device)
        ci_out = torch.empty((nseg, 4, Cout), dtype=torch.float32, device=x.device) if stats else None
        ws = self._mlp_ws(x, max(Cin, Cout), nseg)
        mr = torch.empty((2, nseg, Cout), dtype=torch.float32, device=x.device) if (stats and mean_rstd) else None
        ss_stride = 0 if ss_in is None else ss_in.shape[1] * ss_in.shape[2]
        self._call("tpg_mlp_fwd", "mlp_fwd", 2 * P * (Cin + Cout), x,
                   _ptr(x), P, Cin, Cout, nseg, _ptr(ss_in), ss_stride, float(slope_in), _ptr(W), w_per_seg, _ptr(y),
                   float(eps), float(momentum), _ptr(running_mean), _ptr(running_var), _ptr(num_batches_tracked),
                   _ptr(mean_shift), _ptr(gamma_out), _ptr(beta_out), _ptr(None if mr is None else mr[0]),
                   _ptr(None if mr is None else mr[1]), _ptr(ci_out), _ptr(ws), flops=2 * P * Cin * Cout)
        if mr is not None:
            return y, ci_out, mr[0], mr[1]
        return y, ci_out

    def rowbn_stats(self, x, eps, momentum, running_mean, running_var, num_batches_tracked, nseg, mean_shift,
                    consts=None):
        P, Cc = x.shape
        mean = torch.empty((nseg, Cc), dtype=torch.float32, device=x.device)
        rstd = torch.empty((nseg, Cc), dtype=torch.float32, device=x.device)
        ws = self._bn_ws(x, Cc, nseg)
        if consts is not None:
            ci = torch.empty((nseg, 4, Cc), dtype=torch.float32, device=x.device)
            self._call("tpg_rowbn_stats_consts", "rowbn_fwd_stats", x.element_size() * P * Cc, x,
                       _ptr(x), _DTYPE_CODE[x.dtype], P, Cc, float(eps), float(momentum), _ptr(running_mean),
                       _ptr(running_var), _ptr(num_batches_tracked), _ptr(mean_shift), _ptr(consts[0]), _ptr(consts[1]),
                       _ptr(mean), _ptr(rstd), _ptr(ci), _ptr(ws), int(nseg))
            return mean, rstd, ci
        self._call("tpg_rowbn_fwd", "rowbn_fwd_stats", x.element_size() * P * Cc, x,
                   _ptr(x), _DTYPE_CODE[x.dtype], P, 0, Cc, float(eps), float(momentum), 1, _ptr(running_mean),
                   _ptr(running_var), _ptr(num_batches_tracked), _ptr(mean_shift), None, None, 1.0, _ptr(mean),
                   _ptr(rstd), _ptr(x), _DTYPE_CODE[x.dtype], None, _ptr(ws), int(nseg), 1)
        return mean, rstd

    def rowbn_apply_max(self, x, K, mean, rstd, gamma, beta, slope, out_dtype, nseg):
        P, Cc = x.shape
        rows = P // K if K else P
        y = torch.empty((rows, Cc), dtype=out_dtype, device=x.device)
        arg = torch.empty((rows, Cc), dtype=torch.uint8, device=x.device) if K else None
        ws = self._bn_ws(x, Cc, nseg)
        self._call("tpg_rowbn_fwd", "rowbn_fwd_apply_max" if K else "rowbn_fwd_apply",
                   x.element_size() * P * Cc + y.element_size() * rows * Cc + (rows * Cc if K else 0), x,
                   _ptr(x), _DTYPE_CODE[x.dtype], P, K, Cc, 0.0, 0.0, 1, None, None, None, None, _ptr(gamma), _ptr(beta),
                   float(slope), _ptr(mean), _ptr(rstd), _ptr(y), _DTYPE_CODE[out_dtype], _ptr(arg), _ptr(ws), int(nseg), 2)
        return y, arg

    def rowbn_bwd_sums(self, gy, x, arg, y, K, mean, rstd, gamma, beta, slope, need_affine, nseg, want_cb=False):
        P, Cc = x.shape
        c12 = torch.empty((nseg, 2, Cc), dtype=torch.float32, device=x.device)
        dgamma = torch.empty(Cc, dtype=torch.float32, device=x.device) if need_affine else None
        dbeta = torch.empty(Cc, dtype=torch.float32, device=x.device) if need_affine else None
        ws = self._bn_ws(x, Cc, nseg)
        if y is not None and (not K or y.dtype != gy.dtype):
            y = None
        if want_cb:
            cb = torch.empty((nseg, 4, Cc), dtype=torch.float32, device=x.device)
            ag = torch.empty_like(gy) if (K and y is not None) else None
            self._call("tpg_rowbn_bwd_sums_consts", "rowbn_bwd_reduce", (3 if ag is not None else 2) * gy.element_size() * gy.numel(), x,
                       _ptr(gy), _DTYPE_CODE[gy.dtype], _ptr(x), _DTYPE_CODE[x.dtype], _ptr(arg), _ptr(y),
                       _DTYPE_CODE[y.dtype] if y is not None else 0, P, K, Cc, 1, _ptr(mean), _ptr(rstd), _ptr(gamma),
                       _ptr(beta), float(slope), _ptr(dgamma), _ptr(dbeta), _ptr(c12), _ptr(cb), _ptr(ag), _ptr(ws), int(nseg))
            return c12, dgamma, dbeta, cb, ag
        self._call("tpg_rowbn_bwd_sums", "rowbn_bwd_reduce", 2 * gy.element_size() * gy.numel(), x,
                   _ptr(gy), _DTYPE_CODE[gy.dtype], _ptr(x), _DTYPE_CODE[x.dtype], _ptr(arg), _ptr(y),
                   _DTYPE_CODE[y.dtype] if y is not None else 0, P, K, Cc, 1, _ptr(mean), _ptr(rstd), _ptr(gamma),
                   _ptr(beta), float(slope), _ptr(dgamma), _ptr(dbeta), _ptr(c12), _ptr(ws), int(nseg))
        return c12, dgamma, dbeta

    def mlp_consts(self, mean, rstd, gamma, beta, c12, want_ci, want_cb):
        nseg, Cc = mean.shape
        ci = torch.empty((nseg, 4, Cc), dtype=torch.float32, device=mean.device) if want_ci else None
        cb = torch.empty((nseg, 4, Cc), dtype=torch.float32, device=mean.device) if want_cb else None
        self._call("tpg_mlp_consts", "mlp_consts", 32 * nseg * Cc, mean, _ptr(mean), _ptr(rstd), _ptr(gamma), _ptr(beta),
                   _ptr(c12), Cc, nseg, _ptr(ci), _ptr(cb))
        return ci, cb

    def mlp_max_prep(self, gout, y, cb_out, slope_out, nseg):
        rows, Cc = gout.shape
        ag = torch.empty_like(gout)
        self._call("tpg_mlp_max_prep", "mlp_max_prep", 6 * rows * Cc, gout, _ptr(gout), _ptr(y), _ptr(cb_out),
                   float(slope_out), rows, Cc, nseg, _ptr(ag))
        return ag

    def mlp_dgrad(self, x_out, g_out, arg, K, cb_out, x_in, ci_in, slope_in, W, nseg, need_affine, sums=True):
        P, Cout = x_out.shape
        Cin = x_in.shape[1]
        mode = 1 if arg is not None else 0
        w_per_seg = int(W.dim() == 3 and W.shape[0] == nseg and nseg > 1)
        dev = x_out.device
        g_in = torch.empty((P, Cin), dtype=torch.bfloat16, device=dev)
        c12 = torch.empty((nseg, 2, Cin), dtype=torch.float32, device=dev) if sums else None
        cb_in = torch.empty((nseg, 4, Cin), dtype=torch.float32, device=dev) if sums else None
        dgamma = torch.empty(Cin, dtype=torch.float32, device=dev) if (need_affine and sums) else None
        dbeta = torch.empty(Cin, dtype=torch.float32, device=dev) if (need_affine and sums) else None
        ws = self._mlp_ws(x_out, max(Cin, Cout), nseg)
        self._call("tpg_mlp_dgrad", "mlp_dgrad", 2 * P * (Cout + 2 * Cin) + (0 if mode else 2 * P * Cout), x_out,
                   _ptr(x_out), _ptr(g_out), _ptr(arg), int(K), _ptr(cb_out), _ptr(x_in), _ptr(ci_in),
                   float(slope_in), _ptr(W), w_per_seg, P, Cin, Cout, nseg, mode, _ptr(g_in), _ptr(c12), _ptr(dgamma),
                   _ptr(dbeta), _ptr(cb_in), _ptr(ws), flops=2 * P * Cin * Cout)
        return g_in, c12, cb_in, dgamma, dbeta

    def mlp_wgrad(self, x_out, g_out, arg, K, cb_out, x_in, ci_in, slope_in, nseg):
        P, Cout = x_out.shape
        Cin = x_in.shape[1]
        mode = 1 if arg is not None else 0
        dW = torch.empty((nseg, Cout, Cin), dtype=torch.float32, device=x_out.device)
        ws = self._workspace("wgrad", x_out, self.lib.tpg_mlp_wgrad_workspace_bytes(P, Cin, Cout, nseg) // 4)
        self._call("tpg_mlp_wgrad", "mlp_wgrad", 2 * P * (Cout + Cin) + (0 if mode else 2 * P * Cout), x_out,
                   _ptr(x_out), _ptr(g_out), _ptr(arg), int(K), _ptr(cb_out), _ptr(x_in), _ptr(ci_in),
                   float(slope_in), P, Cin, Cout, nseg, mode, _ptr(dW), _ptr(ws), flops=2 * P * Cin * Cout)
        return dW

    def small_tail_fwd(self, h, W1, W2, s1, s2, K):
        E, H = h.shape
        P = E // K
        C1, C2 = W1.shape[0], W2.shape[0]
        out = torch.empty((P, C2), dtype=h.dtype, device=h.device)
        arg = torch.empty((P, C2), dtype=torch.uint8, device=h.device)
        self._call("tpg_small_tail_fwd", "small_tail_fwd", h.element_size() * (E * H + P * C2) + P * C2, h,
                   _ptr(h), 1 if h.dtype == torch.bfloat16 else 0, _ptr(W1), _ptr(W2), float(s1), float(s2), P, int(K),
                   H, C1, C2, _ptr(out), _ptr(arg), flops=2 * E * (H * C1 + C1 * C2))
        return out, arg

    def small_tail_bwd(self, h, out, gout, arg, W1, W2, s1, s2, K):
        E, H = h.shape
        P = E // K
        C1, C2 = W1.shape[0], W2.shape[0]
        gh = torch.empty_like(h)
        dW1 = torch.empty((C1, H), dtype=torch.float32, device=h.device)
        dW2 = torch.empty((C2, C1), dtype=torch.float32, device=h.device)
        ws = self._workspace("small_tail", h, max(16, self.lib.tpg_small_tail_workspace_bytes(P, int(K)) // 4))
        self._call("tpg_small_tail_bwd", "small_tail_bwd", h.element_size() * (2 * E * H + 2 * P * C2) + P * C2, h,
                   _ptr(h), _ptr(out), _ptr(gout), _ptr(arg), 1 if h.dtype == torch.bfloat16 else 0, _ptr(W1), _ptr(W2),
                   float(s1), float(s2), P, int(K), H, C1, C2, _ptr(gh), _ptr(dW1), _ptr(dW2), _ptr(ws),
                   flops=2 * E * (2 * H * C1 + 2 * C1 * C2 + H * C1))
        return gh, dW1, dW2

    def mlp_bn_bwd_apply(self, g, x, ci, c12, nseg, K=0):
        P, Cc = x.shape
        dx = torch.empty_like(x)
        if K:
            qneg = torch.empty((P // K, Cc), dtype=torch.float32, device=x.device)
            self._call("tpg_mlp_bn_bwd_apply_rowsum", "mlp_bn_bwd_apply", 6 * P * Cc + 4 * (P // K) * Cc, x, _ptr(g),
                       _ptr(x), _ptr(ci), _ptr(c12), P, K, Cc, nseg, _ptr(dx), _ptr(qneg))
            return dx, qneg
        self._call("tpg_mlp_bn_bwd_apply", "mlp_bn_bwd_apply", 6 * P * Cc, x, _ptr(g), _ptr(x), _ptr(ci), _ptr(c12), P,
                   Cc, nseg, _ptr(dx))
        return dx

    def spectral_norm_fwd(self, W, u, v, iterate, eps):
        R, Cn = W.shape
        Wsn = torch.empty_like(W)
        sigma = torch.empty(1, dtype=torch.float32, device=W.device)
        self._call("tpg_spectral_norm_fwd", "spectral_norm_fwd", 4 * (2 * R * Cn + 2 * (R + Cn)), W,
                   _ptr(W), _ptr(u), _ptr(v), R, Cn, int(iterate), float(eps), _ptr(Wsn), _ptr(sigma))
        return Wsn, sigma

    def spectral_norm_bwd(self, G, Wsn, u, v, sigma):
        R, Cn = Wsn.shape
        dW = torch.empty_like(Wsn)
        self._call("tpg_spectral_norm_bwd", "spectral_norm_bwd", 4 * 3 * R * Cn, G,
                   _ptr(G), _ptr(Wsn), _ptr(u), _ptr(v), _ptr(sigma), R, Cn, _ptr(dW))
        return dW


    def _sn_plan(self, Ws, us, vs, uses):
        key = tuple(t.data_ptr() for t in (*Ws, *us, *vs)) + tuple(uses)
        plan = self._sn_plans.get(key)
        if plan is None:
            _need(max(int(n) for n in uses) <= 64, "at most 64 uses of one spectrally-normalised weight per forward")
            dev = Ws[0].device
            fwd, bwd, layout, goffs, dwoffs = [], [], [], [], []
            out_total = g_total = dw_total = 0
            for W, u, v, n in zip(Ws, us, vs, uses):
                R, Cn = W.shape
                st = sn_multi_stride(R, Cn)
                fwd += [W.data_ptr(), u.data_ptr(), v.data_ptr(), R, Cn, n, out_total]
                bwd += [R, Cn, n, out_total, g_total, dw_total]
                layout.append((out_total, st))
                goffs.append(g_total)
                dwoffs.append(dw_total)
                out_total += st * n
                g_total += R * Cn * n
                dw_total += R * Cn
            rows, split = self.lib.tpg_spectral_norm_split_rows(), None
            if (SN_SPLIT[0] and max(W.shape[1] for W in Ws) <= self.lib.tpg_spectral_norm_split_max_cn()
                    and max(W.shape[0] for W in Ws) <= self.lib.tpg_spectral_norm_split_max_rows()):
                sd, pmap, words, off = [], [], 0, 0
                for m, (W, u, v, n) in enumerate(zip(Ws, us, vs, uses)):
                    R, Cn = W.shape
                    parts = (R + rows - 1) // rows
                    sd += [W.data_ptr(), u.data_ptr(), v.data_ptr(), R, Cn, n, off, parts, words]
                    pmap += [(m, g) for g in range(parts)]
                    words += 2 * parts * (Cn + 1)
                    off += sn_multi_stride(R, Cn) * n
                words = (words + 1 + 1) & ~1
                split = dict(desc=torch.tensor(sd, dtype=torch.int64).to(dev),
                             pmap=torch.tensor(pmap, dtype=torch.int32).to(dev).contiguous(), parts=len(pmap),
                             xws=torch.zeros(words, dtype=torch.int64, device=dev), words=words,
                             max_cn=max(W.shape[1] for W in Ws))
            plan = dict(split=split,
                        fwd=torch.tensor(fwd, dtype=torch.int64).to(dev), bwd=torch.tensor(bwd, dtype=torch.int64).to(dev),
                        layout=layout, goffs=goffs, dwoffs=dwoffs, out_total=out_total, g_total=g_total,
                        dw_total=dw_total, max_rc=max(W.shape[0] + W.shape[1] for W in Ws), M=len(Ws),
                        max_uses=max(int(n) for n in uses))
            self._sn_plans[key] = plan
        return plan

    def rowlinear_fwd(self, x, W, bias, nseg, slope, out_dtype):
        P, Cin = x.shape
        Cout = W.shape[-2]
        y = torch.empty((P, Cout), dtype=out_dtype, device=x.device)
        self._call("tpg_rowlinear_fwd", "rowlinear_fwd", x.element_size() * P * Cin + y.element_size() * P * Cout + 4 * W.numel(), x,
                   _ptr(x), _DTYPE_CODE[x.dtype], _ptr(W), _ptr(bias), P, int(nseg), Cin, Cout, float(slope), _ptr(y),
                   _DTYPE_CODE[out_dtype], flops=2 * P * Cin * Cout)
        return y

    def rowlinear_dgrad(self, gy, y, W, nseg, slope, x_dtype):
        P, Cout = gy.shape
        Cin = W.shape[-1]
        dx = torch.empty((P, Cin), dtype=x_dtype, device=gy.device)
        self._call("tpg_rowlinear_dgrad", "rowlinear_dgrad", gy.element_size() * P * Cout * (2 if y is not None else 1)
                   + dx.element_size() * P * Cin + 4 * W.numel(), gy,
                   _ptr(gy), _ptr(y), _DTYPE_CODE[gy.dtype], _ptr(W), P, int(nseg), Cin, Cout, float(slope), _ptr(dx),
                   _DTYPE_CODE[x_dtype], flops=2 * P * Cin * Cout)
        return dx

    def rowlinear_wgrad(self, x, gy, y, nseg, slope, need_bias):
        P, Cin = x.shape
        Cout = gy.shape[1]
        dW = torch.empty((nseg, Cout, Cin), dtype=torch.float32, device=x.device)
        db = torch.empty(Cout, dtype=torch.float32, device=x.device) if need_bias else None
        need = self.lib.tpg_rowlinear_wgrad_workspace_bytes(P, int(nseg), Cin, Cout, int(bool(need_bias))) // 4 + 4
        ws = self._workspace("rowlinear", x, need)
        self._call("tpg_rowlinear_wgrad", "rowlinear_wgrad", x.element_size() * P * Cin + gy.element_size() * P * Cout
                   * (2 if y is not None else 1), x,
                   _ptr(x), _DTYPE_CODE[x.dtype], _ptr(gy), _ptr(y), _DTYPE_CODE[gy.dtype], P, int(nseg), Cin, Cout,
                   float(slope), _ptr(dW), _ptr(db), _ptr(ws), flops=2 * P * Cin * Cout)
        return dW, db

    def spectral_norm_multi_fwd(self, Ws, us, vs, uses, iterate, eps):
        plan = self._sn_plan(Ws, us, vs, uses)
        out = torch.empty(plan["out_total"], dtype=torch.float32, device=Ws[0].device)
        nbytes = 4 * sum((1 + n) * W.numel() for W, n in zip(Ws, uses))
        sp = plan["split"]
        if iterate and sp is not None:
            self._call("tpg_spectral_norm_multi_fwd_split", "spectral_norm_fwd", nbytes, out,
                       _ptr(sp["desc"]), _ptr(sp["pmap"]), sp["parts"], sp["max_cn"], _ptr(out), _ptr(sp["xws"]),
                       sp["words"], float(eps))
            return out, plan
        self._call("tpg_spectral_norm_multi_fwd", "spectral_norm_fwd", nbytes, out,
                   _ptr(plan["fwd"]), plan["M"], plan["max_rc"], _ptr(out), int(iterate), float(eps))
        return out, plan

    def spectral_norm_multi_bwd(self, out, plan, gflat):
        dw = torch.empty(plan["dw_total"], dtype=torch.float32, device=out.device)
        maxu = plan["max_uses"]
        scratch = torch.empty(self.lib.tpg_spectral_norm_multi_bwd_scratch(plan["M"], maxu), dtype=torch.float32,
                              device=out.device)
        self._call("tpg_spectral_norm_multi_bwd", "spectral_norm_bwd", 4 * (3 * plan["g_total"] + plan["dw_total"]),
                   out, _ptr(plan["bwd"]), plan["M"], maxu, _ptr(gflat), _ptr(out), _ptr(dw), _ptr(scratch))
        return dw


SN_SPLIT = [os.environ.get("TPGAN_SN_SPLIT", "1") != "0"]


def sn_multi_stride(R, Cn):
    return (R * Cn + R + Cn + 1 + 3) & ~3


_DTYPE_CODE = {torch.float32: 0, torch.bfloat16: 1}
_hip = None


def backend_for(t):
    global _hip
    if t.is_cuda:
        if _hip is None:
            _hip = HipBackend()
        return _hip
    impl = _BACKENDS.get(t.device.type)
    if impl is None:
        raise RuntimeError(
            f"tpgan_amd ops: {t.device.type} tensors are not supported (HIP only); "
            "the product has no CPU fallback")
    return impl


def _need(cond, msg):
    if not cond:
        raise RuntimeError(msg)


def _check_float(t, name, ndim):
    _need(isinstance(t, torch.Tensor), f"{name} must be a tensor")
    _need(t.dim() == ndim, f"{name} must have {ndim} dims, got {tuple(t.shape)}")
    _need(t.dtype == torch.float32, f"{name} must be a float tensor, got {t.dtype}")
    _need(t.is_contiguous(), f"{name} must be a contiguous tensor")


def _check_int(t, name, ndim):
    _need(isinstance(t, torch.Tensor), f"{name} must be a tensor")
    _need(t.dim() == ndim, f"{name} must have {ndim} dims, got {tuple(t.shape)}")
    _need(t.dtype == torch.int32, f"{name} must be an int tensor, got {t.dtype}")
    _need(t.is_contiguous(), f"{name} must be a contiguous tensor")


def _same_device(*ts):
    d = ts[0].device
    for t in ts[1:]:
        _need(t.device == d, "all tensors must be on the same device")


def furthest_point_sample(xyz, npoint):
    _check_float(xyz, "xyz", 3)
    _need(xyz.shape[2] == 3, "xyz must be (B,N,3)")
    _need(int(npoint) > 0 and xyz.shape[1] > 0, "npoint and N must be positive")
    with torch.no_grad():
        return backend_for(xyz).fps(xyz.detach(), int(npoint))


def furthest_point_sample_prefix(xyz, npoint, prefix_flag=None):
    _check_float(xyz, "xyz", 3)
    _need(xyz.shape[2] == 3 and int(npoint) > 0 and xyz.shape[1] > 0, "xyz must be (B,N,3), npoint and N positive")
    be = backend_for(xyz)
    with torch.no_grad():
        if hasattr(be, "fps_prefix"):
            return be.fps_prefix(xyz.detach(), int(npoint), prefix_flag)
        return be.fps(xyz.detach(), int(npoint)), None


CONTEXT_WINDOW = 25
CONTEXT_NONE = -2 ** 31


def context_state(N, device):
    return torch.full((2, N), CONTEXT_NONE, dtype=torch.int32, device=device)


def context_keep(mask, state, t0):
    T = mask.shape[0]
    t = torch.arange(t0, t0 + T, dtype=torch.int32, device=mask.device).view(T, 1)
    none = torch.full_like(mask, CONTEXT_NONE, dtype=torch.int32)
    hit = torch.cummax(torch.cat([state[:1], torch.where(mask >= 0.6, t, none)]), 0).values[1:]
    nan = torch.cummax(torch.cat([state[1:], torch.where(torch.isnan(mask), t, none)]), 0).values[1:]
    lo = t - (CONTEXT_WINDOW - 1)
    state.copy_(torch.stack([hit[-1], nan[-1]]))
    return (hit >= lo) & (nan < lo)


def _context_expand_torch(pos, edge, mask, state, t0):
    T, N, _ = pos.shape
    r = edge.shape[1] // N
    keep = context_keep(mask, state, t0).view(T, N, 1)
    expanded = pos.repeat(1, 1, r).view(T, -1, 3) + (edge.view(T, N, 3 * r) * keep.float()).view(T, -1, 3)
    hard = keep.repeat(1, 1, r)
    hard[:, :, 0] = True
    counts = hard.view(T, -1).sum(1)
    offsets = torch.cat([counts.new_zeros(1), torch.cumsum(counts, 0)])
    return expanded[hard.view(T, -1)], offsets


def context_expand(pos, edge, mask, state, t0):
    _check_float(pos, "pos", 3)
    _check_float(edge, "edge", 3)
    _check_int(state, "state", 2)
    if mask.dim() == 3 and mask.shape[2] == 1:
        mask = mask.view(mask.shape[0], mask.shape[1])
    _check_float(mask, "mask", 2)
    _same_device(pos, edge, mask, state)
    T, N, _ = pos.shape
    _need(pos.shape[2] == 3 and edge.shape[2] == 3, "pos and edge must hold 3-D points")
    _need(N > 0 and edge.shape[0] == T and edge.shape[1] % N == 0, "edge must be (T, N*r, 3)")
    _need(tuple(mask.shape) == (T, N) and tuple(state.shape) == (2, N), "mask must be (T, N) and state (2, N)")
    _need(2 <= edge.shape[1] // N <= 16, "upsampling ratio must be 2..16")
    _need(int(t0) >= 0, "t0 must be >= 0")
    be = backend_for(pos)
    with torch.no_grad():
        if hasattr(be, "context_expand"):
            return be.context_expand(pos.detach(), edge.detach(), mask.detach(), state, int(t0))
        return _context_expand_torch(pos.detach(), edge.detach(), mask.detach(), state, int(t0))


PATCH_SELECT_NAN_KEY = 0x7FC00000


def _host_ints(a, name, shape):
    if isinstance(a, torch.Tensor):
        _need(not a.is_cuda, f"{name} is a host table (the sampler draws it on the host): pass a CPU tensor or a list")
        a = a.numpy()
    a = np.asarray(a)
    _need(a.dtype.kind in "iu", f"{name} must hold integers, got {a.dtype}")
    _need(a.shape == tuple(shape), f"{name} must have shape {tuple(shape)}, got {a.shape}")
    _need(a.size == 0 or (a.min() >= -2 ** 31 and a.max() < 2 ** 31), f"{name} does not fit int32")
    return np.ascontiguousarray(a, dtype=np.int32)


def _patch_select_torch(points, first, count, seed, K):
    out = []
    for f, n, s in zip(first.tolist(), count.tolist(), seed.tolist()):
        x = points[f:f + n]
        d = x - x[s]
        d2 = (d[:, 0] * d[:, 0] + d[:, 1] * d[:, 1]) + d[:, 2] * d[:, 2]
        bits = d2.view(torch.int32).long()
        bits = torch.where(torch.isnan(d2), torch.full_like(bits, PATCH_SELECT_NAN_KEY), bits)
        key = (bits << 32) | torch.arange(n, device=points.device)
        out.append((torch.sort(key).values[:K] & 0xFFFFFFFF).int())
    return torch.stack(out)


def patch_select(points, first, count, seed, K):
    _check_float(points, "points", 2)
# ... 378 lines not shown
    _ROWSUM_SLOT[("dev", dx0.device.index)] = (dx0, qneg, K)


def _take_rowsum(gout):
    slot = _ROWSUM_SLOT.pop(("dev", gout.device.index), None)
    if slot is None:
        return None
    dx0, qneg, K = slot
    if (gout.data_ptr() == dx0.data_ptr() and gout.numel() == dx0.numel() and gout.dtype == dx0.dtype
            and gout.dim() == 4 and gout.shape[2] == K and gout.shape[3] == dx0.shape[1]):
        return qneg
    return None


class _RowCombine(torch.autograd.Function):
    @staticmethod
    def forward(ctx, U, QE, idx, mode, slope, out_dtype, inverse):
        be = backend_for(U)
        out = be.rowcombine_fwd(U, QE, idx, mode, slope, out_dtype)
        ctx.save_for_backward(idx, QE if mode == ROW_EDGE else None)
        ctx.inverse = inverse
        ctx.mode, ctx.slope, ctx.N, ctx.in_dtype = mode, slope, U.shape[1], U.dtype
        ctx.has_q = QE is not None
        return out

    @staticmethod
    def backward(ctx, gout):
        idx, E = ctx.saved_tensors
        gout = gout.contiguous()
        if gout.dtype not in _DTYPE_CODE:
            gout = gout.float()
        kw = {} if ctx.inverse is None else {"inverse": ctx.inverse}
        ready = _take_rowsum(gout) if (ctx.mode == ROW_SUB and ctx.in_dtype == torch.float32) else None
        if ready is not None:
            gU, _ = backend_for(gout).rowcombine_bwd(gout, idx, None, ROW_GATHER, ctx.N, ctx.slope, ctx.in_dtype, **kw)
            return gU, (ready.view(gout.shape[0], gout.shape[1], gout.shape[3]) if ctx.has_q else None), None, None, None, None, None
        gU, gQE = backend_for(gout).rowcombine_bwd(gout, idx, E, ctx.mode, ctx.N, ctx.slope, ctx.in_dtype, **kw)
        return gU, (gQE if ctx.has_q else None), None, None, None, None, None


_DEFERRED_INVERSES = []


class NeighbourList:
    __slots__ = ("idx", "n_src", "inverse")

    def __init__(self, idx, n_src, inverse=None):
        _need(idx.dtype == torch.int32 and idx.dim() == 3 and idx.is_contiguous(), "idx must be contiguous (B,S,K) int32")
        self.idx, self.n_src, self.inverse = idx, int(n_src), inverse

    def clouds(self, lo, hi):
        return NeighbourList(self.idx[lo:hi], self.n_src)

    @staticmethod
    def cat(lists):
        _need(all(l.n_src == lists[0].n_src for l in lists), "neighbour lists into different numbers of source rows")
        return NeighbourList(torch.cat([l.idx for l in lists], 0), lists[0].n_src)

    def with_inverse(self):
        if _DEFERRED_INVERSES:
            _DEFERRED_INVERSES[-1].append(self)
            return self
        be = backend_for(self.idx)
        if hasattr(be, "invert_index"):
            self.inverse = be.invert_index(self.idx, self.n_src)
        return self

    def tensors(self):
        return [self.idx] + list(self.inverse or ())


def neighbour_list(idx, n_src):
    if isinstance(idx, NeighbourList):
        _need(idx.n_src == n_src, f"neighbour list into {idx.n_src} source rows used on {n_src}")
        return idx
    _need(torch.is_tensor(idx) and idx.dim() == 3 and idx.dtype == torch.int32, "idx must be (B,S,K) int32")
    return NeighbourList(idx.contiguous(), n_src)


def row_combine(U, QE, idx, mode, slope=0.2, out_dtype=None):
    _need(U.dim() == 3, "U (B,N,C), idx (B,S,K) int32")
    nl = neighbour_list(idx, U.shape[1])
    idx = nl.idx
    _need(U.dtype in _DTYPE_CODE, f"row_combine supports fp32/bf16, got {U.dtype}")
    _need(U.shape[0] == idx.shape[0], "batch mismatch")
    out_dtype = out_dtype or U.dtype
    U = U.contiguous()
    if mode == ROW_GATHER:
        QE = None
    else:
        _need(QE is not None and QE.shape == (U.shape[0], idx.shape[1], U.shape[2]), "QE must be (B,S,C)")
        QE = QE.to(U.dtype).contiguous()
        if mode == ROW_EDGE:
            _need(idx.shape[1] == U.shape[1], "EDGE mode needs S == N")
    ne = 4 if (U.dtype == torch.float32 and out_dtype == torch.float32) else 8
    _need(U.shape[2] % ne == 0, f"channel count {U.shape[2]} must be a multiple of {ne}")
    return _RowCombine.apply(U, QE, idx, mode, float(slope), out_dtype, nl.inverse)


class deferred_inverses:

    def __enter__(self):
        self.pending = []
        _DEFERRED_INVERSES.append(self.pending)
        return self.pending

    def __exit__(self, *exc):
        _DEFERRED_INVERSES.pop()
        return False


def run_inverses(pending):
    for nl in pending:
        nl.with_inverse()
    del pending[:]


def attach_inverse(idx, N):
    return NeighbourList(idx, N).with_inverse()


class _HeadBNAct(torch.autograd.Function):
    @staticmethod
    def forward(ctx, h, gamma, beta, running_mean, running_var, nbt, momentum, eps, slope, mask):
        be = backend_for(h)
        y, mean, rstd = be.head_bn_act_fwd(h, gamma, beta, running_mean, running_var, nbt, momentum, eps, slope, mask)
        ctx.save_for_backward(h, mean, rstd, gamma, beta, mask)
        ctx.slope = slope
        return y

    @staticmethod
    def backward(ctx, gy):
        h, mean, rstd, gamma, beta, mask = ctx.saved_tensors
        need_affine = (gamma is not None and ctx.needs_input_grad[1]) or (beta is not None and ctx.needs_input_grad[2])
        dh, dg, db = backend_for(gy).head_bn_act_bwd(gy.contiguous().float(), h, mean, rstd, gamma, beta, ctx.slope, mask,
                                                     need_affine)
        return (dh, dg if gamma is not None else None, db if beta is not None else None, None, None, None, None, None,
                None, None)


def head_bn_act(h, bn, slope, mask=None):
    _need(h.dim() == 2 and h.dtype == torch.float32, "h must be (B,C) fp32")
    _need(bn.momentum is not None and bn.track_running_stats, "needs a BatchNorm1d with a fixed momentum and running statistics")
    _need(h.shape[0] > 1, "Expected more than 1 value per channel when training")
    return _HeadBNAct.apply(h.contiguous(), bn.weight, bn.bias, bn.running_mean, bn.running_var, bn.num_batches_tracked,
                            float(bn.momentum), float(bn.eps), float(slope),
                            None if mask is None else mask.contiguous().float())


class _RowBNAct(torch.autograd.Function):
    @staticmethod
    def forward(ctx, x, gamma, beta, running_mean, running_var, training, momentum, eps, slope, K, out_dtype,
                num_batches_tracked, nseg, mean_shift):
        be = backend_for(x)
        C_ = x.shape[1]
        if training:
            mean = torch.empty((nseg, C_), dtype=torch.float32, device=x.device)
            rstd = torch.empty((nseg, C_), dtype=torch.float32, device=x.device)
        elif running_mean is None:
            mean = rstd = None
        else:
            mean = running_mean.float().contiguous()
            if mean_shift is not None:
                mean = mean - mean_shift.float()
            rstd = torch.rsqrt(running_var.float() + eps)
        y, arg = be.rowbn_fwd(x, K, eps, momentum, training, running_mean if training else None,
                              running_var if training else None, gamma, beta, slope, mean, rstd, out_dtype,
                              num_batches_tracked if training else None, **({"nseg": nseg} if nseg != 1 else {}),
                              **({"mean_shift": mean_shift} if mean_shift is not None and training else {}))
        ctx.save_for_backward(x, gamma, beta, mean, rstd, arg, y if K else None)
        ctx.cfg = (training, slope, K, nseg)
        return y

    @staticmethod
    def backward(ctx, gy):
        x, gamma, beta, mean, rstd, arg, y = ctx.saved_tensors
        training, slope, K, nseg = ctx.cfg
        gy = gy.contiguous()
        if gy.dtype not in _DTYPE_CODE:
            gy = gy.float()
        need_affine = gamma is not None and (ctx.needs_input_grad[1] or ctx.needs_input_grad[2])
        dx, dgamma, dbeta = backend_for(x).rowbn_bwd(gy, x, arg, K, training, mean, rstd, gamma, beta, slope,
                                                    need_affine, y, **({"nseg": nseg} if nseg != 1 else {}))
        return dx, dgamma, dbeta, None, None, None, None, None, None, None, None, None, None, None


def row_bn_act(x, gamma, beta, running_mean, running_var, training, momentum, eps, slope=1.0, K=0,
               out_dtype=None, num_batches_tracked=None, nseg=1, mean_shift=None):
    _need(x.dim() == 2 and x.dtype in _DTYPE_CODE, "x must be (P,C) fp32/bf16")
    _need(K == 0 or (0 < K <= 256 and x.shape[0] % K == 0), "K must divide the row count (<= 256)")
    _need(nseg >= 1 and x.shape[0] % nseg == 0 and (K == 0 or (x.shape[0] // nseg) % K == 0),
          "nseg must divide the rows (and K the rows of a segment)")
    if not training:
        nseg = 1
    out_dtype = out_dtype or x.dtype
    ne = 4 if (x.dtype == torch.float32 and out_dtype == torch.float32) else 8
    _need(x.shape[1] % ne == 0 and x.shape[1] <= 1024, f"channels must be a multiple of {ne}, <= 1024")
    if not training:
        _need((running_mean is None) == (running_var is None), "eval mode: both running statistics or neither")
    if num_batches_tracked is not None:
        _need(num_batches_tracked.dtype == torch.int64 and num_batches_tracked.numel() == 1
              and num_batches_tracked.device == x.device, "num_batches_tracked must be an int64 scalar on x's device")
    g = None if gamma is None else gamma.float().contiguous()
    b = None if beta is None else beta.float().contiguous()
    return _RowBNAct.apply(x.contiguous(), g, b, running_mean, running_var, bool(training), float(momentum),
                           float(eps), float(slope), int(K), out_dtype, num_batches_tracked, int(nseg),
                           None if mean_shift is None else mean_shift.detach().float().contiguous())


def row_act_max(x, slope, K, out_dtype=None):
    return row_bn_act(x, None, None, None, None, False, 0.0, 0.0, slope, K, out_dtype)


MLP_CHANNELS = ((64, 64), (64, 128), (128, 64), (128, 128), (128, 256), (256, 128), (256, 256))


class _MlpTail(torch.autograd.Function):

    @staticmethod
    def forward(ctx, x0, cfg, *tensors):
        nseg, K, slopes, eps, moms, states, shifts = cfg
        be = backend_for(x0)
        L = (len(tensors) - 2) // 3
        gam = [tensors[0]] + [tensors[3 * l + 3] for l in range(L)]
        bet = [tensors[1]] + [tensors[3 * l + 4] for l in range(L)]
        Ws = [tensors[3 * l + 2] for l in range(L)]
        xs, cis = [x0], []
        rm, rv, nbt = states[0]
        cis.append(be.rowbn_stats(x0, eps[0], moms[0], rm, rv, nbt, nseg, shifts[0], consts=(gam[0], bet[0]))[2])
        for l in range(L):
            rm, rv, nbt = states[l + 1]
            y, ci, *mr = be.mlp_fwd(xs[-1], cis[-1], slopes[l], Ws[l], nseg, eps[l + 1], moms[l + 1], rm, rv, nbt,
                                    shifts[l + 1], gam[l + 1], bet[l + 1], mean_rstd=(l == L - 1))
            xs.append(y)
            cis.append(ci)
        mean_L, rstd_L = mr
        out, arg = be.rowbn_apply_max(xs[-1], K, mean_L, rstd_L, gam[-1], bet[-1], slopes[L], torch.bfloat16, nseg)
        ctx.save_for_backward(*xs, *cis, *gam, *bet, *Ws, mean_L, rstd_L, out, *([arg] if arg is not None else []))
        ctx.cfg = (nseg, K, slopes, L)
        return out

    @staticmethod
    def backward(ctx, gout):
        nseg, K, slopes, L = ctx.cfg
        t = list(ctx.saved_tensors)
        n = L + 1
        xs, cis, gam, bet = t[:n], t[n:2 * n], t[2 * n:3 * n], t[3 * n:4 * n]
        Ws = t[4 * n:4 * n + L]
        mean_L, rstd_L, out = t[4 * n + L:4 * n + L + 3]
        arg = t[4 * n + L + 3] if K else None
        be = backend_for(xs[0])
        gout = gout.contiguous()
        if gout.dtype != torch.bfloat16:
            gout = gout.to(torch.bfloat16)
        need = ctx.needs_input_grad
        need_aff = [need[2] or need[3]] + [need[3 * l + 5] or need[3 * l + 6] for l in range(L)]
        need_w = [need[3 * l + 4] for l in range(L)]
        grads_aff = [None] * n
        grads_w = [None] * L
        c12, dg, db, cb, ag = be.rowbn_bwd_sums(gout, xs[L], arg, out if K else None, K, mean_L, rstd_L, gam[L], bet[L],
                                                slopes[L], need_aff[L], nseg, want_cb=True)
        grads_aff[L] = (dg, db)
        g_next, arg_next, K_next = (ag if ag is not None else be.mlp_max_prep(gout, out, cb, slopes[L], nseg)), arg, K
        for l in range(L, 0, -1):
            if need_w[l - 1]:
                grads_w[l - 1] = be.mlp_wgrad(xs[l], g_next, arg_next, K_next, cb, xs[l - 1], cis[l - 1], slopes[l - 1],
                                              nseg)
            g_in, c12, cb, dg, db = be.mlp_dgrad(xs[l], g_next, arg_next, K_next, cb, xs[l - 1], cis[l - 1],
                                                 slopes[l - 1], Ws[l - 1], nseg, need_aff[l - 1])
            grads_aff[l - 1] = (dg, db)
            g_next, arg_next, K_next = g_in, None, 0
        dx0 = None
        if need[0] and K and _ROWSUM_HANDOFF[0]:
            dx0, qneg = be.mlp_bn_bwd_apply(g_next, xs[0], cis[0], c12, nseg, K)
            _offer_rowsum(dx0, qneg, K)
        elif need[0]:
            dx0 = be.mlp_bn_bwd_apply(g_next, xs[0], cis[0], c12, nseg)
        res = [dx0, None, grads_aff[0][0], grads_aff[0][1]]
        for l in range(L):
            gw = grads_w[l]
            if gw is not None and Ws[l].dim() == 2:
                gw = gw.sum(0) if gw.shape[0] > 1 else gw[0]
            elif gw is not None and Ws[l].shape[0] != gw.shape[0]:
                gw = gw.sum(0, keepdim=True)
            res += [gw, grads_aff[l + 1][0], grads_aff[l + 1][1]]
        return tuple(res)


_IDENT = {}


def _ident_consts(C_, device):
    key = (C_, device)
    if key not in _IDENT:
        cb = torch.zeros((1, 4, C_), dtype=torch.float32, device=device)
        cb[0, 0] = 1.0
        ci = torch.zeros((1, 4, C_), dtype=torch.float32, device=device)
        ci[0, 0] = 1.0
        ci[0, 3] = 1.0
        _IDENT[key] = (cb, ci)
    return _IDENT[key]


class _MlpTailPlain(torch.autograd.Function):

    @staticmethod
    def forward(ctx, x0, K, slopes, *Ws):
        be = backend_for(x0)
        L = len(Ws)
        xs = [x0]
        for l in range(L):
            y, _ = be.mlp_fwd(xs[-1], None, slopes[l], Ws[l], 1, stats=False)
            xs.append(y)
        out, arg = be.rowbn_fwd(xs[-1], K, 0.0, 0.0, False, None, None, None, None, slopes[L], None, None, torch.bfloat16)
        ctx.save_for_backward(*xs, *Ws, out, arg)
        ctx.cfg = (K, slopes, L)
        return out

    @staticmethod
    def backward(ctx, gout):
        K, slopes, L = ctx.cfg
        t = list(ctx.saved_tensors)
        xs, Ws, out, arg = t[:L + 1], t[L + 1:2 * L + 1], t[2 * L + 1], t[2 * L + 2]
        be = backend_for(xs[0])
        gout = gout.contiguous()
        if gout.dtype != torch.bfloat16:
            gout = gout.to(torch.bfloat16)
        need = ctx.needs_input_grad
        grads_w = [None] * L
        cb = _ident_consts(out.shape[1], out.device)[0]
        g_next, arg_next, K_next = be.mlp_max_prep(gout, out, cb, slopes[L], 1), arg, K
        for l in range(L, 0, -1):
            cb = _ident_consts(xs[l].shape[1], out.device)[0]
            ci = _ident_consts(xs[l - 1].shape[1], out.device)[1]
            if need[3 + l - 1]:
                grads_w[l - 1] = be.mlp_wgrad(xs[l], g_next, arg_next, K_next, cb, xs[l - 1], ci, slopes[l - 1], 1)[0]
            if l > 1 or need[0]:
                g_next = be.mlp_dgrad(xs[l], g_next, arg_next, K_next, cb, xs[l - 1], ci, slopes[l - 1], Ws[l - 1], 1,
                                      False, sums=False)[0]
            arg_next, K_next = None, 0
        return (g_next if need[0] else None, None, None) + tuple(grads_w)


def mlp_tail_plain(x0, weights, slopes, K):
    L = len(weights)
    _need(len(slopes) == L + 1 and L >= 1, "mlp_tail_plain: L weights, L+1 slopes")
    _need(all(0.0 <= float(sl) <= 1.0 for sl in slopes), "mlp_tail_plain: LeakyReLU slopes in [0, 1]")
    _need(all(w.dtype == torch.float32 and w.dim() == 2 for w in weights), "mlp_tail_plain: 2-D fp32 weights")
    return _MlpTailPlain.apply(x0.contiguous(), int(K), tuple(float(s) for s in slopes), *[w.contiguous() for w in weights])


SMALL_TAIL_CHANNELS = (16, 16, 32)


class _SmallTail(torch.autograd.Function):

    @staticmethod
    def forward(ctx, h, W1, W2, s1, s2, K):
        be = backend_for(h)
        w1, w2 = W1.detach().float().contiguous(), W2.detach().float().contiguous()
        out, arg = be.small_tail_fwd(h, w1, w2, s1, s2, K)
        ctx.save_for_backward(h, out, arg, w1, w2)
        ctx.cfg = (s1, s2, K, W1.dtype, W2.dtype)
        return out

    @staticmethod
    def backward(ctx, gout):
        h, out, arg, w1, w2 = ctx.saved_tensors
        s1, s2, K, t1, t2 = ctx.cfg
        be = backend_for(h)
        gh, dW1, dW2 = be.small_tail_bwd(h, out, gout.to(h.dtype).contiguous(), arg, w1, w2, s1, s2, K)
        return (gh if ctx.needs_input_grad[0] else None, dW1.to(t1) if ctx.needs_input_grad[1] else None,
                dW2.to(t2) if ctx.needs_input_grad[2] else None, None, None, None)


def small_tail_supported(h, channels, K):
    return (h.is_cuda and h.dtype in (torch.bfloat16, torch.float32) and tuple(channels) == SMALL_TAIL_CHANNELS
            and 0 < K <= 255)


def small_tail(h, W1, W2, slope1, slope2, K):
    _need(0.0 <= float(slope1) <= 1.0 and 0.0 <= float(slope2) <= 1.0, "small_tail: LeakyReLU slopes in [0, 1]")
    _need(h.dim() == 2 and h.shape[0] % int(K) == 0, "small_tail: (P*K, 16) rows")
    return _SmallTail.apply(h.contiguous(), W1, W2, float(slope1), float(slope2), int(K))


def mlp_tail_supported(x, channels, K):
    if not (x.is_cuda and x.dtype == torch.bfloat16 and 0 < K <= 255 and len(channels) >= 2):
        return False
    return all((a, b) in MLP_CHANNELS for a, b in zip(channels[:-1], channels[1:]))


def mlp_tail(x0, bns, weights, slopes, K, nseg=1, shifts=None):
    L = len(weights)
    _need(len(bns) == L + 1 and len(slopes) == L + 1 and L >= 1, "mlp_tail: L weights, L+1 BatchNorms / slopes")
    _need(all(0.0 <= float(sl) <= 1.0 for sl in slopes), "mlp_tail: LeakyReLU slopes in [0, 1] (lrelu = max(z, slope*z))")
    shifts = list(shifts) if shifts is not None else [None] * (L + 1)
    states, eps, moms = [], [], []
    for bn in bns:
        _need(bn.training and bn.momentum is not None, "mlp_tail needs training-mode BatchNorm with a fixed momentum")
        track = bn.track_running_stats and bn.running_mean is not None
        states.append((bn.running_mean if track else None, bn.running_var if track else None,
                       bn.num_batches_tracked if (track and bn.num_batches_tracked is not None) else None))
        eps.append(float(bn.eps))
        moms.append(float(bn.momentum))
    tensors = [bns[0].weight.float(), bns[0].bias.float()]
    for l in range(L):
        w = weights[l]
        _need(w.dtype == torch.float32, "mlp_tail weights are fp32 (rounded to bf16 inside the kernel)")
        tensors += [w.contiguous(), bns[l + 1].weight.float(), bns[l + 1].bias.float()]
    cfg = (int(nseg), int(K), tuple(float(s) for s in slopes), tuple(eps), tuple(moms), tuple(states),
           tuple(None if s is None else s.detach().float().contiguous() for s in shifts))
    return _MlpTail.apply(x0.contiguous(), cfg, *tensors)


class _RowLinear(torch.autograd.Function):

    @staticmethod
    def forward(ctx, x, W, bias, nseg, slope, out_dtype):
        be = backend_for(x)
        Wf = W if W.dtype == torch.float32 else W.float()
        Wf = Wf.contiguous()
        bf = None if bias is None else bias.float().contiguous()
        y = be.rowlinear_fwd(x, Wf, bf, nseg, slope, out_dtype)
        ctx.save_for_backward(x, Wf, y if slope != 1.0 else None)
        ctx.cfg = (int(nseg), float(slope), W.dtype, W.shape, None if bias is None else bias.dtype)
        return y

    @staticmethod
    def backward(ctx, gy):
        x, Wf, y = ctx.saved_tensors
        nseg, slope, w_dtype, w_shape, b_dtype = ctx.cfg
        be = backend_for(x)
        gy = gy.contiguous()
        if gy.dtype not in _DTYPE_CODE:
            gy = gy.float()
        if y is not None and y.dtype != gy.dtype:
            gy = gy.to(y.dtype)
        dx = dW = db = None
        if ctx.needs_input_grad[0]:
            dx = be.rowlinear_dgrad(gy, y, Wf, nseg, slope, x.dtype)
        if ctx.needs_input_grad[1] or (b_dtype is not None and ctx.needs_input_grad[2]):
            dW, db = be.rowlinear_wgrad(x, gy, y, nseg, slope, b_dtype is not None and ctx.needs_input_grad[2])
            dW = dW.view(w_shape).to(w_dtype) if ctx.needs_input_grad[1] else None
            if db is not None:
                db = db.to(b_dtype)
        return dx, dW, db, None, None, None


ROW_LINEAR = [False]


def row_linear_supported(x, W, nseg=1):
    if not (ROW_LINEAR[0] and x.is_cuda and x.dtype in _DTYPE_CODE and W.dtype in (torch.float32, torch.bfloat16)):
        return False
    P = x.numel() // x.shape[-1] if x.numel() else 0
    if P == 0 or not _lib.load().tpg_rowlinear_supported(int(x.shape[-1]), int(W.shape[-2]), 1):
        return False
    return nseg == 1 or (P % nseg == 0 and (P // nseg) % 128 == 0)


def row_linear(x, W, bias=None, slope=1.0, nseg=1, out_dtype=None):
    _need(x.dtype in _DTYPE_CODE, f"row_linear supports fp32/bf16 rows, got {x.dtype}")
    _need(0.0 <= float(slope) <= 1.0, "row_linear: LeakyReLU slope in [0, 1]")
    lead = x.shape[:-1]
    x2 = x.reshape(-1, x.shape[-1]).contiguous()
    if x2.data_ptr() % 16:
        x2 = x2.clone()
    _need((W.dim() == 2 and nseg == 1) or (W.dim() == 3 and W.shape[0] == nseg), "W (Cout,Cin) or (nseg,Cout,Cin)")
    _need(W.shape[-1] == x2.shape[1], "row_linear: channel mismatch")
    y = _RowLinear.apply(x2, W, bias, int(nseg), float(slope), out_dtype or x.dtype)
    return y.view(*lead, W.shape[-2])


class _SpectralNorm(torch.autograd.Function):
    @staticmethod
    def forward(ctx, W, u, v, iterate, eps):
        Wsn, sigma = backend_for(W).spectral_norm_fwd(W, u, v, iterate, eps)
        ctx.save_for_backward(Wsn, u.clone(), v.clone(), sigma)
        return Wsn

    @staticmethod
    def backward(ctx, G):
        Wsn, u, v, sigma = ctx.saved_tensors
        return backend_for(Wsn).spectral_norm_bwd(G.float().contiguous(), Wsn, u, v, sigma), None, None, None, None


def spectral_normalize(weight_orig, u, v, training, eps=1e-12):
    _need(weight_orig.dtype == torch.float32 and u.dtype == torch.float32 and v.dtype == torch.float32,
          "spectral_normalize works on fp32 parameters")
    W2 = weight_orig.reshape(weight_orig.shape[0], -1).contiguous()
    _need(u.numel() == W2.shape[0] and v.numel() == W2.shape[1] and u.is_contiguous() and v.is_contiguous(),
          "u / v do not match the weight")
    return _SpectralNorm.apply(W2, u, v, bool(training), float(eps)).view_as(weight_orig)


class _SpectralNormMulti(torch.autograd.Function):

    @staticmethod
    def forward(ctx, training, eps, uses, *tensors):
        n = len(uses)
        Ws, us, vs = tensors[:n], tensors[n:2 * n], tensors[2 * n:]
        flat, plan = backend_for(Ws[0]).spectral_norm_multi_fwd(list(Ws), list(us), list(vs), list(uses),
                                                                training, eps)
        outs = []
        for W, (off, st), k in zip(Ws, plan["layout"], uses):
            R, Cn = W.shape
            for t in range(k):
                outs.append(flat[off + t * st: off + t * st + R * Cn].view(R, Cn))
        ctx.flat, ctx.plan, ctx.uses = flat, plan, tuple(uses)
        ctx.shapes = [tuple(W.shape) for W in Ws]
        return tuple(outs)

    @staticmethod
    def backward(ctx, *grads):
        parts, i = [], 0
        for (R, Cn), k in zip(ctx.shapes, ctx.uses):
            for _ in range(k):
                g = grads[i]
                i += 1
                parts.append(torch.zeros(R * Cn, dtype=torch.float32, device=ctx.flat.device) if g is None
                             else g.reshape(-1).float())
        gflat = torch.cat(parts)
        dw = backend_for(ctx.flat).spectral_norm_multi_bwd(ctx.flat, ctx.plan, gflat)
        dWs = [dw[off:off + R * Cn].view(R, Cn) for (R, Cn), off in zip(ctx.shapes, ctx.plan["dwoffs"])]
        n = len(ctx.uses)
        return (None, None, None) + tuple(dWs) + (None,) * (2 * n)


def spectral_normalize_many(modules, uses, training, eps=1e-12):
    Ws = [m.weight_orig.reshape(m.weight_orig.shape[0], -1) for m in modules]
    for W in Ws:
        _need(W.dtype == torch.float32 and W.is_contiguous(), "spectral norm works on contiguous fp32 weights")
    us = [m.weight_u for m in modules]
    vs = [m.weight_v for m in modules]
    outs = _SpectralNormMulti.apply(bool(training), float(eps), tuple(int(k) for k in uses), *Ws, *us, *vs)
    res, i = [], 0
    for k in uses:
        res.append(list(outs[i:i + k]))
        i += k
    return res
```

Before: 82.49 steps/s.

## Fuse last plain-tail MLP layer with K-group max pooling in forward and backward

The last layer of the plain MLP tail now computes the matmul, applies LeakyReLU and max-reduces over each K-row group inside the forward kernel. It writes only the pooled output and argmax indices, so the full-resolution activation never goes to memory and the separate rowbn max pass is dropped. The backward path gains a MAX_PLAIN mode for dgrad and wgrad that rebuilds the routed gradient from the pooled output, gout and argmax on the fly, which removes the mlp_max_prep kernel. This adds in-kernel cross-strip reduction through shared memory and extra syncs when K does not divide 16, and it depends on K fitting within a tile.

Result: no change. 81.90 steps/s (-0.7%).

```diff
diff --git a/include/tpgan_ops.h b/include/tpgan_ops.h
--- a/include/tpgan_ops.h
+++ b/include/tpgan_ops.h
@@ -150,6 +150,15 @@
 int tpg_mlp_wgrad(const void *x_out, const void *g_out, const uint8_t *arg, int K, const float *cb_out,
                   const void *x_in, const float *ci_in, float slope_in, long long P, int Cin,
                   int Cout, int nseg, int mode, float *dW, void *ws, void *stream);
+int tpg_mlp_fwd_max_tile_rows(int Cin, int Cout);
+int tpg_mlp_fwd_max(const void *x, long long P, int Cin, int Cout, int nseg, float slope_in, const float *W,
+                    int w_per_seg, int K, float slope_out, void *y, uint8_t *arg, void *stream);
+int tpg_mlp_dgrad_max_plain(const void *y, const void *gout, const uint8_t *arg, int K, float slope_out,
+                            const void *x_in, const float *ci_in, float slope_in, const float *W, int w_per_seg,
+                            long long P, int Cin, int Cout, int nseg, void *g_in, void *ws, void *stream);
+int tpg_mlp_wgrad_max_plain(const void *y, const void *gout, const uint8_t *arg, int K, float slope_out,
+                            const void *x_in, const float *ci_in, float slope_in, long long P, int Cin, int Cout,
+                            int nseg, float *dW, void *ws, void *stream);
 int tpg_mlp_bn_bwd_apply(const void *g, const void *x, const float *ci, const float *c12, long long P, int C,
                          int nseg, void *dx, void *stream);
 int tpg_mlp_bn_bwd_apply_rowsum(const void *g, const void *x, const float *ci, const float *c12, long long P, int K,
diff --git a/temporal-pointcloud-upsampling-gan_amd/_lib.py b/temporal-pointcloud-upsampling-gan_amd/_lib.py
--- a/temporal-pointcloud-upsampling-gan_amd/_lib.py
+++ b/temporal-pointcloud-upsampling-gan_amd/_lib.py
@@ -51,6 +51,9 @@
     "tpg_mlp_max_prep": [_P, _P, _P, _F, _L, _I, _I, _P, _P],
     "tpg_mlp_dgrad": [_P, _P, _P, _I, _P, _P, _P, _F, _P, _I, _L, _I, _I, _I, _I, _P, _P, _P, _P, _P, _P, _P],
     "tpg_mlp_wgrad": [_P, _P, _P, _I, _P, _P, _P, _F, _L, _I, _I, _I, _I, _P, _P, _P],
+    "tpg_mlp_fwd_max": [_P, _L, _I, _I, _I, _F, _P, _I, _I, _F, _P, _P, _P],
+    "tpg_mlp_dgrad_max_plain": [_P, _P, _P, _I, _F, _P, _P, _F, _P, _I, _L, _I, _I, _I, _P, _P, _P],
+    "tpg_mlp_wgrad_max_plain": [_P, _P, _P, _I, _F, _P, _P, _F, _L, _I, _I, _I, _P, _P, _P],
     "tpg_mlp_bn_bwd_apply": [_P, _P, _P, _P, _L, _I, _I, _P, _P],
     "tpg_mlp_bn_bwd_apply_rowsum": [_P, _P, _P, _P, _L, _I, _I, _I, _P, _P, _P],
     "tpg_small_tail_fwd": [_P, _I, _P, _P, _F, _F, _L, _I, _I, _I, _I, _P, _P, _P],
@@ -71,7 +74,7 @@
                  "tpg_mlp_wgrad_workspace_bytes", "tpg_frnn_grid_workspace_bytes", "tpg_small_tail_workspace_bytes",
                  "tpg_chamfer_bwd_workspace_bytes", "tpg_rowlinear_wgrad_workspace_bytes", "tpg_rowlinear_supported",
                  "tpg_spectral_norm_split_rows", "tpg_spectral_norm_split_max_cn", "tpg_spectral_norm_split_max_rows",
-                 "tpg_patch_select_workspace_bytes", "tpg_patch_select_max_k")
+                 "tpg_patch_select_workspace_bytes", "tpg_patch_select_max_k", "tpg_mlp_fwd_max_tile_rows")
 STRING_GETTERS = ("tpg_version", "tpg_target_arch")
 
 STATUS = {0: "TPG_OK", -1: "TPG_ERR_ARG", -2: "TPG_ERR_LAUNCH", -3: "TPG_ERR_UNSUPPORTED"}
@@ -121,6 +124,8 @@
                  "tpg_patch_select_max_k"):
         getattr(lib, name).argtypes = []
         getattr(lib, name).restype = C.c_int
+    lib.tpg_mlp_fwd_max_tile_rows.argtypes = [C.c_int, C.c_int]
+    lib.tpg_mlp_fwd_max_tile_rows.restype = C.c_int
     lib.tpg_rowlinear_supported.argtypes = [C.c_int, C.c_int, C.c_int]
     lib.tpg_rowlinear_supported.restype = C.c_int
     _lib = lib
diff --git a/temporal-pointcloud-upsampling-gan_amd/csrc/mlp_fused.hip b/temporal-pointcloud-upsampling-gan_amd/csrc/mlp_fused.hip
--- a/temporal-pointcloud-upsampling-gan_amd/csrc/mlp_fused.hip
+++ b/temporal-pointcloud-upsampling-gan_amd/csrc/mlp_fused.hip
@@ -15,23 +15,29 @@
     return (n % T) * 16 + n / T;
 }
 
-template <int CIN, int COUT, int STRIPS>
+template <int CIN, int COUT, int STRIPS, bool MAXK>
 __global__ __launch_bounds__(ML_THREADS, 2) void mlp_fwd_kernel(
     const __hip_bfloat16 *__restrict__ x, long long P, const float *__restrict__ ss, int ss_stride, float slope,
-    const float *__restrict__ W, int w_per_seg, __hip_bfloat16 *__restrict__ y, float *__restrict__ part) {
+    const float *__restrict__ W, int w_per_seg, __hip_bfloat16 *__restrict__ y, float *__restrict__ part, int K,
+    float slope_out, uint8_t *__restrict__ arg) {
     constexpr int T = COUT / 16;
     constexpr int KS = CIN / 32;
     constexpr int BM = ML_WAVES * STRIPS * 16;
     constexpr int WROW = CIN + ML_WPAD;
+    constexpr int NSTRIPS = BM / 16;
     extern __shared__ __attribute__((aligned(16))) unsigned char ml_smem[];
     unsigned short *wl = reinterpret_cast<unsigned short *>(ml_smem);
     float *cst = reinterpret_cast<float *>(ml_smem + (size_t)COUT * WROW * 2);
+    float *zs = cst + 2 * CIN;
+    uint8_t *ks = reinterpret_cast<uint8_t *>(zs + (2 * NSTRIPS - 2) * COUT);
+    const int RT = MAXK ? (BM / K) * K : BM;
     float *red = reinterpret_cast<float *>(ml_smem);
     const int tid = threadIdx.x, lane = tid & 63, wave = tid >> 6;
     const int li = lane & 15, lq = lane >> 4;
     const int seg = blockIdx.y;
     x += (size_t)seg * P * CIN;
-    y += (size_t)seg * P * COUT;
+    if constexpr (MAXK) { y += (size_t)seg * (P / K) * COUT; arg += (size_t)seg * (P / K) * COUT; }
+    else y += (size_t)seg * P * COUT;
     {
         const float *Ws = W + (w_per_seg ? (size_t)seg * COUT * CIN : 0);
         for (int e = tid; e < COUT * CIN / 4; e += ML_THREADS) {
@@ -51,14 +57,14 @@
     for (int t = 0; t < T; ++t) { piv[t] = 0.0f; s1[t] = 0.0f; s2[t] = 0.0f; }
     bool have_piv = false;
     float nrows = 0.0f;
-    const long long ntiles = (P + BM - 1) / BM;
+    const long long ntiles = (P + RT - 1) / RT;
     const unsigned short *wfrag = wl + (size_t)li * WROW + 8 * lq;
     const float *csc = cst + 8 * lq, *csh = cst + CIN + 8 * lq;
     uint4 araw[STRIPS][KS];
     auto load_tile = [&](long long tile) {
 #pragma unroll
         for (int st = 0; st < STRIPS; ++st) {
-            long long row = tile * BM + (wave * STRIPS + st) * 16 + li;
+            long long row = tile * RT + (wave * STRIPS + st) * 16 + li;
             row = row < P ? row : P - 1;
             const __hip_bfloat16 *px = x + (size_t)row * CIN + 8 * lq;
 #pragma unroll
@@ -68,7 +74,7 @@
     long long tile = blockIdx.x;
     if (tile < ntiles) load_tile(tile);
     for (; tile < ntiles; tile += gridDim.x) {
-        const long long row_base = tile * BM + (long long)wave * STRIPS * 16;
+        const long long row_base = tile * RT + (long long)wave * STRIPS * 16;
         tpg_f32x4 acc[STRIPS][T];
 #pragma unroll
         for (int st = 0; st < STRIPS; ++st)
@@ -108,6 +114,92 @@
             }
         }
         if (tile + gridDim.x < ntiles) load_tile(tile + gridDim.x);
+        if constexpr (MAXK) {
+            const long long left = P - tile * RT;
+            const int rt = left < RT ? (int)left : RT;
+            const long long grp0 = tile * (RT / K);
+#pragma unroll
+            for (int st = 0; st < STRIPS; ++st) {
+#pragma unroll
+                for (int r = 0; r < 4; ++r)
+#pragma unroll
+                    for (int t = 0; t < T; t += 2) {
+                        const unsigned w = tpg_pack_bf16x2(acc[st][t][r], acc[st][t + 1][r]);
+                        const float v0 = tpg_bf16_lo(w), v1 = tpg_bf16_hi(w);
+                        acc[st][t][r] = v0 > 0.0f ? v0 : v0 * slope_out;
+                        acc[st][t + 1][r] = v1 > 0.0f ? v1 : v1 * slope_out;
+                    }
+                const int sg = wave * STRIPS + st, m0 = 16 * sg;
+                if (m0 >= rt) continue;
+                const int g_hi = ((m0 + 15 < rt ? m0 + 15 : rt - 1)) / K;
+                for (int g = m0 / K; g <= g_hi; ++g) {
+                    const int gs = g * K, ge = gs + K - 1;
+                    float best[T];
+                    int bk[T];
+#pragma unroll
+                    for (int t = 0; t < T; ++t) { best[t] = -INFINITY; bk[t] = 255; }
+#pragma unroll
+                    for (int r = 0; r < 4; ++r) {
+                        const int m = m0 + 4 * lq + r;
+                        const bool in = m >= gs && m <= ge;
+#pragma unroll
+                        for (int t = 0; t < T; ++t)
+                            if (in && acc[st][t][r] > best[t]) { best[t] = acc[st][t][r]; bk[t] = m - gs; }
+                    }
+#pragma unroll
+                    for (int off = 16; off < 64; off *= 2)
+#pragma unroll
+                        for (int t = 0; t < T; ++t) {
+                            const float zo = __shfl_xor(best[t], off, 64);
+                            const int ko = __shfl_xor(bk[t], off, 64);
+                            if (zo > best[t] || (zo == best[t] && ko < bk[t])) { best[t] = zo; bk[t] = ko; }
+                        }
+                    if (lq != 0) continue;
+                    if (gs >= m0 && ge <= m0 + 15) {
+                        unsigned o[T / 2], ob[T / 4];
+#pragma unroll
+                        for (int t = 0; t < T; t += 2) o[t / 2] = tpg_pack_bf16x2(best[t], best[t + 1]);
+#pragma unroll
+                        for (int t = 0; t < T; t += 4)
+                            ob[t / 4] = (unsigned)bk[t] | ((unsigned)bk[t + 1] << 8) | ((unsigned)bk[t + 2] << 16) | ((unsigned)bk[t + 3] << 24);
+                        __hip_bfloat16 *py = y + (size_t)(grp0 + g) * COUT + li * T;
+                        uint8_t *pa = arg + (size_t)(grp0 + g) * COUT + li * T;
+#pragma unroll
+                        for (int v4 = 0; v4 < T / 8; ++v4)
+                            reinterpret_cast<uint4 *>(py)[v4] = make_uint4(o[4 * v4], o[4 * v4 + 1], o[4 * v4 + 2], o[4 * v4 + 3]);
+                        if constexpr (T == 4) *reinterpret_cast<uint2 *>(py) = make_uint2(o[0], o[1]);
+                        if constexpr (T == 16) *reinterpret_cast<uint4 *>(pa) = make_uint4(ob[0], ob[1], ob[2], ob[3]);
+                        if constexpr (T == 8) *reinterpret_cast<uint2 *>(pa) = make_uint2(ob[0], ob[1]);
+                        if constexpr (T == 4) *reinterpret_cast<unsigned *>(pa) = ob[0];
+                    } else {
+                        const int slot = gs < m0 ? 2 * sg - 1 : 2 * sg;
+#pragma unroll
+                        for (int t = 0; t < T; ++t) {
+                            zs[slot * COUT + li * T + t] = best[t];
+                            ks[slot * COUT + li * T + t] = (uint8_t)bk[t];
+                        }
+                    }
+                }
+            }
+            if (16 % K != 0) {
+                __syncthreads();
+                const int c = tid % COUT;
+                for (int b = 1 + tid / COUT; b < NSTRIPS && 16 * b < rt; b += ML_THREADS / COUT) {
+                    const int g = 16 * b / K, gs = g * K, ge = gs + K - 1;
+                    if (gs >= 16 * b || gs < 16 * (b - 1)) continue;
+                    float best = zs[(2 * b - 2) * COUT + c];
+                    int bk = ks[(2 * b - 2) * COUT + c];
+                    for (int sgn = b; 16 * sgn <= ge; ++sgn) {
+                        const float z = zs[(2 * sgn - 1) * COUT + c];
+                        if (z > best) { best = z; bk = ks[(2 * sgn - 1) * COUT + c]; }
+                    }
+                    tpg_store_one(y + (size_t)(grp0 + g) * COUT + c, best);
+                    arg[(size_t)(grp0 + g) * COUT + c] = (uint8_t)bk;
+                }
+                __syncthreads();
+            }
+            continue;
+        }
         if (!have_piv) {
 #pragma unroll
             for (int t = 0; t < T; ++t) {
@@ -147,6 +239,7 @@
             nrows += (float)(left <= 0 ? 0 : (left < STRIPS * 16 ? left : STRIPS * 16));
         }
     }
+    if constexpr (MAXK) return;
 #pragma unroll
     for (int t = 0; t < T; ++t) {
         s1[t] += __shfl_xor(s1[t], 16, 64);
@@ -266,7 +359,7 @@
     if (running_mean && lane == 0) { running_mean[c] = rmean; running_var[c] = rvar; }
 }
 
-enum { MODE_DENSE = 0, MODE_MAX = 1 };
+enum { MODE_DENSE = 0, MODE_MAX = 1, MODE_MAX_PLAIN = 2 };
 
 __device__ __forceinline__ void ld8(const float *p, float (&v)[8]) {
     const float4 a = *reinterpret_cast<const float4 *>(p), b = *reinterpret_cast<const float4 *>(p + 4);
@@ -294,6 +387,18 @@
             }
         }
         o[i] = tpg_pack_bf16x2(v[0], v[1]);
+    }
+}
+
+__device__ __forceinline__ void d_plain8(const uint4 yr, const uint4 gr, const uint2 ar, int k, float slope, unsigned (&o)[4]) {
+    const unsigned yw[4] = {yr.x, yr.y, yr.z, yr.w}, gw[4] = {gr.x, gr.y, gr.z, gr.w};
+#pragma unroll
+    for (int i = 0; i < 4; ++i) {
+        const float g0 = tpg_bf16_lo(gw[i]), g1 = tpg_bf16_hi(gw[i]);
+        const unsigned ag = tpg_pack_bf16x2(tpg_bf16_lo(yw[i]) > 0.0f ? g0 : g0 * slope, tpg_bf16_hi(yw[i]) > 0.0f ? g1 : g1 * slope);
+        const int k0 = (int)__builtin_amdgcn_ubfe(i < 2 ? ar.x : ar.y, 16 * (i & 1), 8);
+        const int k1 = (int)__builtin_amdgcn_ubfe(i < 2 ? ar.x : ar.y, 16 * (i & 1) + 8, 8);
+        o[i] = tpg_pack_bf16x2(0.0f + (k0 == k ? tpg_bf16_lo(ag) : 0.0f), 0.0f + (k1 == k ? tpg_bf16_hi(ag) : 0.0f));
     }
 }
 
@@ -328,7 +433,8 @@
     const uint8_t *__restrict__ arg, int K, const float *__restrict__ cbo,
     const __hip_bfloat16 *__restrict__ x_in, const float *__restrict__ cbi, float slope_in,
     const float *__restrict__ W, int w_per_seg, long long P, __hip_bfloat16 *__restrict__ g_in,
-    float *__restrict__ part) {
+    float *__restrict__ part, float slope_out) {
+    constexpr bool PLAIN = MODE == MODE_MAX_PLAIN;
     constexpr int TI = CIN / 16;
     constexpr int KS = COUT / 32;
     constexpr int BM = ML_WAVES * STRIPS * 16;
@@ -341,7 +447,7 @@
     const int tid = threadIdx.x, lane = tid & 63, wave = tid >> 6;
     const int li = lane & 15, lq = lane >> 4;
     const int seg = blockIdx.y;
-    x_out += (size_t)seg * P * COUT;
+    x_out += (size_t)seg * (PLAIN ? P / K : P) * COUT;
     x_in += (size_t)seg * P * CIN;
     g_in += (size_t)seg * P * CIN;
     if (MODE == MODE_DENSE) g_out += (size_t)seg * P * COUT;
@@ -355,19 +461,22 @@
 #pragma unroll
             for (int i = 0; i < 4; ++i) wl[(size_t)w_lds_row<CIN>(k + i) * WROW + n] = tpg_bf16_bits(wv[i]);
         }
-        const float *cb = cbo + (size_t)seg * 4 * COUT;
-        for (int c = tid; c < COUT; c += ML_THREADS) {
-            cst[c] = cb[c];
-            cst[COUT + c] = cb[3 * COUT + c];
-            cst[2 * COUT + c] = cb[2 * COUT + c];
-            cst[3 * COUT + c] = cb[COUT + c];
+        if constexpr (!PLAIN) {
+            const float *cb = cbo + (size_t)seg * 4 * COUT;
+            for (int c = tid; c < COUT; c += ML_THREADS) {
+                cst[c] = cb[c];
+                cst[COUT + c] = cb[3 * COUT + c];
+                cst[2 * COUT + c] = cb[2 * COUT + c];
+                cst[3 * COUT + c] = cb[COUT + c];
+            }
         }
     }
     __syncthreads();
     for (int ci = tid; ci < CIN; ci += ML_THREADS) {
         const unsigned short *wr = wl + (size_t)w_lds_row<CIN>(ci) * WROW;
         float acc = 0.0f;
-        for (int co = 0; co < COUT; ++co) acc = __builtin_fmaf(cst[2 * COUT + co], __uint_as_float((unsigned)wr[co] << 16), acc);
+        if constexpr (!PLAIN)
+            for (int co = 0; co < COUT; ++co) acc = __builtin_fmaf(cst[2 * COUT + co], __uint_as_float((unsigned)wr[co] << 16), acc);
         bias[ci] = acc;
     }
     __syncthreads();
@@ -419,16 +528,16 @@
         for (int st = 0; st < STRIPS; ++st) {
             long long row = tile * BM + (wave * STRIPS + st) * 16 + li;
             row = row < P ? row : P - 1;
-            px[st] = x_out + (size_t)row * COUT + 8 * lq;
-            const long long grow = MODE == MODE_MAX ? (long long)((unsigned)row / (unsigned)K) : row;
+            const long long grow = MODE != MODE_DENSE ? (long long)((unsigned)row / (unsigned)K) : row;
+            px[st] = x_out + (size_t)(PLAIN ? grow : row) * COUT + 8 * lq;
             pg[st] = g_out + (size_t)grow * COUT + 8 * lq;
-            pa[st] = MODE == MODE_MAX ? arg + (size_t)grow * COUT + 8 * lq : nullptr;
+            pa[st] = MODE != MODE_DENSE ? arg + (size_t)grow * COUT + 8 * lq : nullptr;
         }
     };
     auto load_step = [&](int st, int s) {
         xraw[st][s] = *reinterpret_cast<const uint4 *>(px[st] + 32 * s);
         graw[st][s] = *reinterpret_cast<const uint4 *>(pg[st] + 32 * s);
-        if (MODE == MODE_MAX) araw[st][s] = *reinterpret_cast<const uint2 *>(pa[st] + 32 * s);
+        if (MODE != MODE_DENSE) araw[st][s] = *reinterpret_cast<const uint2 *>(pa[st] + 32 * s);
         else araw[st][s] = make_uint2(0u, 0u);
     };
     long long tile = blockIdx.x;
@@ -470,15 +579,20 @@
         for (int s = 0; s < KS; ++s) {
             float ca[8], cf[8], cfm[8];
             if (MODE == MODE_DENSE) ld8(cst + 32 * s + 8 * lq, ca);
-            ld8(cst + COUT + 32 * s + 8 * lq, cf);
-            ld8(cst + 3 * COUT + 32 * s + 8 * lq, cfm);
+            if constexpr (!PLAIN) {
+                ld8(cst + COUT + 32 * s + 8 * lq, cf);
+                ld8(cst + 3 * COUT + 32 * s + 8 * lq, cfm);
+            }
             bf16x8 afrag[STRIPS];
 #pragma unroll
             for (int st = 0; st < STRIPS; ++st) {
                 const long long row = row_base + st * 16 + li;
                 union { unsigned u[4]; bf16x8 v; } cv;
-                d_out8<MODE>(xraw[st][s], graw[st][s], araw[st][s], MODE == MODE_MAX ? (int)((unsigned)row % (unsigned)K) : 0, ca,
-                             cf, cfm, cv.u);
+                if constexpr (PLAIN)
+                    d_plain8(xraw[st][s], graw[st][s], araw[st][s], (int)((unsigned)row % (unsigned)K), slope_out, cv.u);
+                else
+                    d_out8<MODE>(xraw[st][s], graw[st][s], araw[st][s], MODE == MODE_MAX ? (int)((unsigned)row % (unsigned)K) : 0, ca,
+                                 cf, cfm, cv.u);
                 if (row >= P) { cv.u[0] = 0u; cv.u[1] = 0u; cv.u[2] = 0u; cv.u[3] = 0u; }
                 afrag[st] = cv.v;
                 load_step(st, s);
@@ -661,7 +775,8 @@
     const __hip_bfloat16 *__restrict__ x_out, const __hip_bfloat16 *__restrict__ g_out,
     const uint8_t *__restrict__ arg, int K, const float *__restrict__ cbo,
     const __hip_bfloat16 *__restrict__ x_in, const float *__restrict__ cbi, float slope_in, long long P,
-    float *__restrict__ slab) {
+    float *__restrict__ slab, float slope_out) {
+    constexpr bool PLAIN = MODE == MODE_MAX_PLAIN;
     constexpr int MT = COUT / 16 / ML_WAVES;
     constexpr int NT = CIN / 16;
     constexpr int DROW = COUT + WG_PAD, AROW = CIN + WG_PAD;
@@ -677,15 +792,17 @@
     const int tid = threadIdx.x, lane = tid & 63, wave = tid >> 6;
     const int lq = lane >> 4, li = lane & 15;
     const int seg = blockIdx.y;
-    x_out += (size_t)seg * P * COUT;
+    x_out += (size_t)seg * (PLAIN ? P / K : P) * COUT;
     x_in += (size_t)seg * P * CIN;
     if (MODE == MODE_DENSE) g_out += (size_t)seg * P * COUT;
     else { g_out += (size_t)seg * (P / K) * COUT; arg += (size_t)seg * (P / K) * COUT; }
     const int dch = tid % DCH, drow = tid / DCH, ach = tid % ACH, arow = tid / ACH;
     float ca[8], cf[8], cfm[8], sc[8], sh[8], asum[8];
-    ld8(cbo + ((size_t)seg * 4 + 0) * COUT + 8 * dch, ca);
-    ld8(cbo + ((size_t)seg * 4 + 3) * COUT + 8 * dch, cf);
-    ld8(cbo + ((size_t)seg * 4 + 1) * COUT + 8 * dch, cfm);
+    if constexpr (!PLAIN) {
+        ld8(cbo + ((size_t)seg * 4 + 0) * COUT + 8 * dch, ca);
+        ld8(cbo + ((size_t)seg * 4 + 3) * COUT + 8 * dch, cf);
+        ld8(cbo + ((size_t)seg * 4 + 1) * COUT + 8 * dch, cfm);
+    }
     ld8(cbi + ((size_t)seg * 4 + 0) * CIN + 8 * ach, sc);
     ld8(cbi + ((size_t)seg * 4 + 1) * CIN + 8 * ach, sh);
 #pragma unroll
@@ -704,10 +821,10 @@
         for (int i = 0; i < DN; ++i) {
             long long rr = r0 + drow + i * DR;
             rr = rr < P ? rr : P - 1;
-            const long long grow = MODE == MODE_MAX ? (long long)((unsigned)rr / (unsigned)K) : rr;
-            xr[i] = *reinterpret_cast<const uint4 *>(x_out + (size_t)rr * COUT + 8 * dch);
+            const long long grow = MODE != MODE_DENSE ? (long long)((unsigned)rr / (unsigned)K) : rr;
+            xr[i] = *reinterpret_cast<const uint4 *>(x_out + (size_t)(PLAIN ? grow : rr) * COUT + 8 * dch);
             gr[i] = *reinterpret_cast<const uint4 *>(g_out + (size_t)grow * COUT + 8 * dch);
-            ar[i] = MODE == MODE_MAX ? *reinterpret_cast<const uint2 *>(arg + (size_t)grow * COUT + 8 * dch) : make_uint2(0u, 0u);
+            ar[i] = MODE != MODE_DENSE ? *reinterpret_cast<const uint2 *>(arg + (size_t)grow * COUT + 8 * dch) : make_uint2(0u, 0u);
         }
 #pragma unroll
         for (int i = 0; i < AN; ++i) {
@@ -725,7 +842,10 @@
             const int r = drow + i * DR;
             const long long row = r0 + r;
             unsigned o[4];
-            d_out8<MODE>(xr[i], gr[i], ar[i], MODE == MODE_MAX ? (int)((unsigned)(row < P ? row : P - 1) % (unsigned)K) : 0, ca, cf, cfm, o);
+            if constexpr (PLAIN)
+                d_plain8(xr[i], gr[i], ar[i], (int)((unsigned)(row < P ? row : P - 1) % (unsigned)K), slope_out, o);
+            else
+                d_out8<MODE>(xr[i], gr[i], ar[i], MODE == MODE_MAX ? (int)((unsigned)(row < P ? row : P - 1) % (unsigned)K) : 0, ca, cf, cfm, o);
             if (row >= P) { o[0] = 0u; o[1] = 0u; o[2] = 0u; o[3] = 0u; }
             *reinterpret_cast<uint4 *>(dxt + (size_t)r * DROW + 8 * dch) = make_uint4(o[0], o[1], o[2], o[3]);
         }
@@ -742,8 +862,10 @@
                 a = fmaxf(a, a * slope_in);
                 b = fmaxf(b, b * slope_in);
                 o[q] = valid ? tpg_pack_bf16x2(a, b) : 0u;
-                asum[2 * q] += tpg_bf16_lo(o[q]);
-                asum[2 * q + 1] += tpg_bf16_hi(o[q]);
+                if constexpr (!PLAIN) {
+                    asum[2 * q] += tpg_bf16_lo(o[q]);
+                    asum[2 * q + 1] += tpg_bf16_hi(o[q]);
+                }
             }
             *reinterpret_cast<uint4 *>(at + (size_t)r * AROW + 8 * ach) = make_uint4(o[0], o[1], o[2], o[3]);
         }
@@ -765,15 +887,17 @@
         }
         __syncthreads();
     }
-#pragma unroll
-    for (int i = 0; i < 8; ++i) ssum[(size_t)arow * CIN + 8 * ach + i] = asum[i];
-    __syncthreads();
     float sv[NT];
-#pragma unroll
-    for (int n = 0; n < NT; ++n) {
-        float t = 0.0f;
-        for (int r = 0; r < AR; ++r) t += ssum[(size_t)r * CIN + 16 * n + li];
-        sv[n] = t;
+    if constexpr (!PLAIN) {
+#pragma unroll
+        for (int i = 0; i < 8; ++i) ssum[(size_t)arow * CIN + 8 * ach + i] = asum[i];
+        __syncthreads();
+#pragma unroll
+        for (int n = 0; n < NT; ++n) {
+            float t = 0.0f;
+            for (int r = 0; r < AR; ++r) t += ssum[(size_t)r * CIN + 16 * n + li];
+            sv[n] = t;
+        }
     }
     float *out = slab + ((size_t)seg * gridDim.x + blockIdx.x) * COUT * CIN;
     const float *ce = cbo + ((size_t)seg * 4 + 2) * COUT;
@@ -782,9 +906,9 @@
 #pragma unroll
         for (int r = 0; r < 4; ++r) {
             const int co = 16 * (wave * MT + m) + 4 * lq + r;
-            const float e = ce[co];
-#pragma unroll
-            for (int n = 0; n < NT; ++n) out[(size_t)co * CIN + 16 * n + li] = __builtin_fmaf(e, sv[n], acc[m][n][r]);
+            const float e = PLAIN ? 0.0f : ce[co];
+#pragma unroll
+            for (int n = 0; n < NT; ++n) out[(size_t)co * CIN + 16 * n + li] = PLAIN ? acc[m][n][r] : __builtin_fmaf(e, sv[n], acc[m][n][r]);
         }
 }
 
@@ -941,6 +1065,10 @@
     constexpr size_t w = (size_t)COUT * (CIN + ML_WPAD) * 2, red = sizeof(float) * ML_WAVES * 3 * COUT;
     return (w > red ? w : red) + sizeof(float) * 2 * CIN;
 }
+template <int CIN, int COUT> constexpr size_t fwd_max_smem() {
+    constexpr int NSTRIPS = ML_WAVES * fwd_strips<CIN, COUT>();
+    return (size_t)COUT * (CIN + ML_WPAD) * 2 + sizeof(float) * 2 * CIN + (size_t)(2 * NSTRIPS - 2) * COUT * 5;
+}
 
 int fwd_blocks(long long P, int bm, int nseg, int slots = ML_MAX_BLOCKS) {
     const long long tiles = (P + bm - 1) / bm;
@@ -955,12 +1083,29 @@
     constexpr int STRIPS = fwd_strips<CIN, COUT>();
     constexpr int BM = ML_WAVES * STRIPS * 16;
     constexpr size_t smem = fwd_smem<CIN, COUT>();
-    constexpr auto kern = mlp_fwd_kernel<CIN, COUT, STRIPS>;
+    constexpr auto kern = mlp_fwd_kernel<CIN, COUT, STRIPS, false>;
     if (smem > 64 * 1024 && !tpg_allow_dynamic_lds<kern>((int)smem)) return TPG_ERR_UNSUPPORTED;
     const int G = fwd_blocks(P, BM, nseg, 2 * smem > 160 * 1024 ? 256 : 512);
     *G_out = G;
     hipLaunchKernelGGL(kern, dim3(G, nseg), dim3(ML_THREADS), smem, st, static_cast<const __hip_bfloat16 *>(x), P, ss,
-                       ss_stride, slope, W, w_per_seg, static_cast<__hip_bfloat16 *>(y), part);
+                       ss_stride, slope, W, w_per_seg, static_cast<__hip_bfloat16 *>(y), part, 0, 0.0f, nullptr);
+    return TPG_OK;
+}
+
+template <int CIN, int COUT> constexpr int fwd_tile_rows() { return ML_WAVES * fwd_strips<CIN, COUT>() * 16; }
+
+template <int CIN, int COUT>
+int fwd_max_launch(const void *x, long long P, int nseg, float slope, const float *W, int w_per_seg, int K, float slope_out,
+                   void *y, uint8_t *arg, hipStream_t st) {
+    constexpr int STRIPS = fwd_strips<CIN, COUT>();
+    constexpr int BM = fwd_tile_rows<CIN, COUT>();
+    constexpr size_t smem = fwd_max_smem<CIN, COUT>();
+    constexpr auto kern = mlp_fwd_kernel<CIN, COUT, STRIPS, true>;
+    if (K > BM) return TPG_ERR_UNSUPPORTED;
+    if (smem > 64 * 1024 && !tpg_allow_dynamic_lds<kern>((int)smem)) return TPG_ERR_UNSUPPORTED;
+    const int G = fwd_blocks(P, (BM / K) * K, nseg, 2 * smem > 160 * 1024 ? 256 : 512);
+    hipLaunchKernelGGL(kern, dim3(G, nseg), dim3(ML_THREADS), smem, st, static_cast<const __hip_bfloat16 *>(x), P, nullptr,
+                       0, slope, W, w_per_seg, static_cast<__hip_bfloat16 *>(y), nullptr, K, slope_out, arg);
     return TPG_OK;
 }
 
@@ -975,7 +1120,7 @@
 template <int CIN, int COUT, int MODE>
 int dgrad_launch(const void *x_out, const void *g_out, const uint8_t *arg, int K, const float *cbo,
                  const void *x_in, const float *cbi, float slope_in, const float *W, int w_per_seg, long long P, int nseg,
-                 void *g_in, float *part, int *G_out, hipStream_t st) {
+                 void *g_in, float *part, int *G_out, hipStream_t st, float slope_out = 0.0f) {
     constexpr int STRIPS = bwd_strips<CIN, COUT>();
     constexpr int BM = ML_WAVES * STRIPS * 16;
     constexpr size_t smem = dgrad_smem<CIN, COUT>();
@@ -987,7 +1132,7 @@
     hipLaunchKernelGGL(kern, dim3(G, nseg), dim3(ML_THREADS), smem, st, static_cast<const __hip_bfloat16 *>(x_out),
                        static_cast<const __hip_bfloat16 *>(g_out), arg, K, cbo,
                        static_cast<const __hip_bfloat16 *>(x_in), cbi, slope_in, W, w_per_seg, P,
-                       static_cast<__hip_bfloat16 *>(g_in), part);
+                       static_cast<__hip_bfloat16 *>(g_in), part, slope_out);
     return TPG_OK;
 }
 
@@ -1008,14 +1153,14 @@
 template <int CIN, int COUT, int MODE>
 int wgrad_launch(const void *x_out, const void *g_out, const uint8_t *arg, int K, const float *cbo,
                  const void *x_in, const float *cbi, float slope_in, long long P, int nseg, float *slab, int G,
-                 hipStream_t st) {
+                 hipStream_t st, float slope_out = 0.0f) {
     constexpr size_t smem = wgrad_smem<CIN, COUT>();
     constexpr int OCC = (COUT * CIN / ML_THREADS >= 128) ? 1 : 2;
     constexpr auto kern = mlp_wgrad_kernel<CIN, COUT, MODE, OCC>;
     if (smem > 64 * 1024 && !tpg_allow_dynamic_lds<kern>((int)smem)) return TPG_ERR_UNSUPPORTED;
     hipLaunchKernelGGL(kern, dim3(G, nseg), dim3(ML_THREADS), smem, st, static_cast<const __hip_bfloat16 *>(x_out),
                        static_cast<const __hip_bfloat16 *>(g_out), arg, K, cbo,
-                       static_cast<const __hip_bfloat16 *>(x_in), cbi, slope_in, P, slab);
+                       static_cast<const __hip_bfloat16 *>(x_in), cbi, slope_in, P, slab, slope_out);
     return TPG_OK;
 }
 
@@ -1057,6 +1202,36 @@
         hipLaunchKernelGGL(mlp_stats_finalize_kernel, dim3((Cout + FIN_CH - 1) / FIN_CH), dim3(FIN_THREADS), 0, st, part, G,
                            Cout, nseg, eps, momentum, running_mean, running_var, num_batches_tracked, mean_shift,
                            gamma_out, beta_out, mean_out, rstd_out, ci_out);
+    TPG_RETURN_IF_LAUNCH_FAILED();
+    return TPG_OK;
+}
+
+extern "C" int tpg_mlp_fwd_max_tile_rows(int Cin, int Cout) {
+    int rows = 0;
+#define TPG_ML_ROWS(CI, CO) \
+    if (Cin == CI && Cout == CO) rows = fwd_tile_rows<CI, CO>();
+    TPG_ML_SHAPES(TPG_ML_ROWS)
+#undef TPG_ML_ROWS
+    return rows;
+}
+
+extern "C" int tpg_mlp_fwd_max(const void *x, long long P, int Cin, int Cout, int nseg, float slope_in, const float *W,
+                               int w_per_seg, int K, float slope_out, void *y, uint8_t *arg, void *stream) {
+    if (P <= 0 || nseg < 1 || nseg > 65535 || P % nseg || K < 1 || K > 255 || (P / nseg) % K) return TPG_ERR_ARG;
+    if (!x || !W || !y || !arg) return TPG_ERR_ARG;
+    if (!ml_shape_ok(Cin, Cout)) return TPG_ERR_UNSUPPORTED;
+    if ((reinterpret_cast<uintptr_t>(x) | reinterpret_cast<uintptr_t>(y) | reinterpret_cast<uintptr_t>(W) |
+         reinterpret_cast<uintptr_t>(arg)) & 15)
+        return TPG_ERR_UNSUPPORTED;
+    P /= nseg;
+    if (P >= 0x7fffffffLL) return TPG_ERR_UNSUPPORTED;
+    int rc = TPG_ERR_UNSUPPORTED;
+#define TPG_ML_FWD_MAX(CI, CO)                                                                              \
+    if (Cin == CI && Cout == CO)                                                                            \
+        rc = fwd_max_launch<CI, CO>(x, P, nseg, slope_in, W, w_per_seg, K, slope_out, y, arg, tpg_stream(stream));
+    TPG_ML_SHAPES(TPG_ML_FWD_MAX)
+#undef TPG_ML_FWD_MAX
+    if (rc) return rc;
     TPG_RETURN_IF_LAUNCH_FAILED();
     return TPG_OK;
 }
@@ -1120,6 +1295,30 @@
     return TPG_OK;
 }
 
+extern "C" int tpg_mlp_dgrad_max_plain(const void *y, const void *gout, const uint8_t *arg, int K, float slope_out,
+                                       const void *x_in, const float *ci_in, float slope_in, const float *W,
+                                       int w_per_seg, long long P, int Cin, int Cout, int nseg, void *g_in, void *ws,
+                                       void *stream) {
+    if (P <= 0 || nseg < 1 || nseg > 65535 || P % nseg || K < 1 || K > 255 || (P / nseg) % K) return TPG_ERR_ARG;
+    if (!y || !gout || !arg || !x_in || !ci_in || !W || !g_in || !ws) return TPG_ERR_ARG;
+    P /= nseg;
+    if (P >= 0x7fffffffLL || !ml_shape_ok(Cin, Cout)) return TPG_ERR_UNSUPPORTED;
+    if ((reinterpret_cast<uintptr_t>(y) | reinterpret_cast<uintptr_t>(gout) | reinterpret_cast<uintptr_t>(x_in) |
+         reinterpret_cast<uintptr_t>(g_in) | reinterpret_cast<uintptr_t>(W) | reinterpret_cast<uintptr_t>(ws) |
+         reinterpret_cast<uintptr_t>(arg)) & 15)
+        return TPG_ERR_UNSUPPORTED;
+    int G = 0, rc = TPG_ERR_UNSUPPORTED;
+#define TPG_ML_DGP(CI, CO)                                                                                           \
+    if (Cin == CI && Cout == CO)                                                                                     \
+        rc = dgrad_launch<CI, CO, MODE_MAX_PLAIN>(y, gout, arg, K, nullptr, x_in, ci_in, slope_in, W, w_per_seg, P,  \
+                                                  nseg, g_in, static_cast<float *>(ws), &G, tpg_stream(stream), slope_out);
+    TPG_ML_SHAPES(TPG_ML_DGP)
+#undef TPG_ML_DGP
+    if (rc) return rc;
+    TPG_RETURN_IF_LAUNCH_FAILED();
+    return TPG_OK;
+}
+
 extern "C" size_t tpg_mlp_wgrad_workspace_bytes(long long P, int Cin, int Cout, int nseg) {
     if (nseg < 1 || P <= 0) return 0;
     const int G = wgrad_blocks(P / nseg, nseg, Cin, Cout);
@@ -1156,6 +1355,32 @@
     return TPG_OK;
 }
 
+extern "C" int tpg_mlp_wgrad_max_plain(const void *y, const void *gout, const uint8_t *arg, int K, float slope_out,
+                                       const void *x_in, const float *ci_in, float slope_in, long long P, int Cin,
+                                       int Cout, int nseg, float *dW, void *ws, void *stream) {
+    if (P <= 0 || nseg < 1 || nseg > 65535 || P % nseg || K < 1 || K > 255 || (P / nseg) % K) return TPG_ERR_ARG;
+    if (!y || !gout || !arg || !x_in || !ci_in || !dW || !ws) return TPG_ERR_ARG;
+    P /= nseg;
+    if (P >= 0x7fffffffLL || !ml_shape_ok(Cin, Cout)) return TPG_ERR_UNSUPPORTED;
+    if ((reinterpret_cast<uintptr_t>(y) | reinterpret_cast<uintptr_t>(gout) | reinterpret_cast<uintptr_t>(x_in) |
+         reinterpret_cast<uintptr_t>(dW) | reinterpret_cast<uintptr_t>(ws) | reinterpret_cast<uintptr_t>(arg)) & 15)
+        return TPG_ERR_UNSUPPORTED;
+    hipStream_t st = tpg_stream(stream);
+    float *slab = static_cast<float *>(ws);
+    const int G = wgrad_blocks(P, nseg, Cin, Cout);
+    int rc = TPG_ERR_UNSUPPORTED;
+#define TPG_ML_WGP(CI, CO)                                                                                          \
+    if (Cin == CI && Cout == CO)                                                                                    \
+        rc = wgrad_launch<CI, CO, MODE_MAX_PLAIN>(y, gout, arg, K, nullptr, x_in, ci_in, slope_in, P, nseg, slab, G, st, slope_out);
+    TPG_ML_SHAPES(TPG_ML_WGP)
+#undef TPG_ML_WGP
+    if (rc) return rc;
+    const int n = Cin * Cout;
+    hipLaunchKernelGGL(mlp_wgrad_reduce_kernel, dim3((n / 4 + 63) / 64, nseg), dim3(256), 0, st, slab, G, n, dW);
+    TPG_RETURN_IF_LAUNCH_FAILED();
+    return TPG_OK;
+}
+
 extern "C" int tpg_mlp_bn_bwd_apply(const void *g, const void *x, const float *ci, const float *c12, long long P, int C,
                                     int nseg, void *dx, void *stream) {
     if (P <= 0 || nseg < 1 || nseg > 65535 || P % nseg || !g || !x || !ci || !c12 || !dx) return TPG_ERR_ARG;
diff --git a/temporal-pointcloud-upsampling-gan_amd/ops.py b/temporal-pointcloud-upsampling-gan_amd/ops.py
--- a/temporal-pointcloud-upsampling-gan_amd/ops.py
+++ b/temporal-pointcloud-upsampling-gan_amd/ops.py
@@ -608,6 +608,41 @@
         self._call("tpg_mlp_wgrad", "mlp_wgrad", 2 * P * (Cout + Cin) + (0 if mode else 2 * P * Cout), x_out,
                    _ptr(x_out), _ptr(g_out), _ptr(arg), int(K), _ptr(cb_out), _ptr(x_in), _ptr(ci_in),
                    float(slope_in), P, Cin, Cout, nseg, mode, _ptr(dW), _ptr(ws), flops=2 * P * Cin * Cout)
+        return dW
+
+    def mlp_fwd_max_rows(self, Cin, Cout):
+        return int(self.lib.tpg_mlp_fwd_max_tile_rows(int(Cin), int(Cout)))
+
+    def mlp_fwd_max(self, x, slope_in, W, K, slope_out, nseg=1):
+        P, Cin = x.shape
+        w_per_seg = int(W.dim() == 3 and W.shape[0] == nseg and nseg > 1)
+        Cout = W.shape[-2]
+        out = torch.empty((P // K, Cout), dtype=torch.bfloat16, device=x.device)
+        arg = torch.empty((P // K, Cout), dtype=torch.uint8, device=x.device)
+        self._call("tpg_mlp_fwd_max", "mlp_fwd", 2 * P * Cin + 3 * (P // K) * Cout, x,
+                   _ptr(x), P, Cin, Cout, nseg, float(slope_in), _ptr(W), w_per_seg, int(K), float(slope_out), _ptr(out),
+                   _ptr(arg), flops=2 * P * Cin * Cout)
+        return out, arg
+
+    def mlp_dgrad_max_plain(self, out, gout, arg, K, slope_out, x_in, ci_in, slope_in, W, nseg=1):
+        P, Cin = x_in.shape
+        Cout = out.shape[1]
+        w_per_seg = int(W.dim() == 3 and W.shape[0] == nseg and nseg > 1)
+        g_in = torch.empty((P, Cin), dtype=torch.bfloat16, device=out.device)
+        ws = self._mlp_ws(out, max(Cin, Cout), nseg)
+        self._call("tpg_mlp_dgrad_max_plain", "mlp_dgrad", 4 * P * Cin + 5 * (P // K) * Cout, out,
+                   _ptr(out), _ptr(gout), _ptr(arg), int(K), float(slope_out), _ptr(x_in), _ptr(ci_in), float(slope_in),
+                   _ptr(W), w_per_seg, P, Cin, Cout, nseg, _ptr(g_in), _ptr(ws), flops=2 * P * Cin * Cout)
+        return g_in
+
+    def mlp_wgrad_max_plain(self, out, gout, arg, K, slope_out, x_in, ci_in, slope_in, nseg=1):
+        P, Cin = x_in.shape
+        Cout = out.shape[1]
+        dW = torch.empty((nseg, Cout, Cin), dtype=torch.float32, device=out.device)
+        ws = self._workspace("wgrad", out, self.lib.tpg_mlp_wgrad_workspace_bytes(P, Cin, Cout, nseg) // 4)
+        self._call("tpg_mlp_wgrad_max_plain", "mlp_wgrad", 2 * P * Cin + 5 * (P // K) * Cout, out,
+                   _ptr(out), _ptr(gout), _ptr(arg), int(K), float(slope_out), _ptr(x_in), _ptr(ci_in), float(slope_in),
+                   P, Cin, Cout, nseg, _ptr(dW), _ptr(ws), flops=2 * P * Cin * Cout)
         return dW
 
     def small_tail_fwd(self, h, W1, W2, s1, s2, K):
@@ -1592,35 +1627,58 @@
     return _IDENT[key]
 
 
+PLAIN_TAIL_MAX_EPILOGUE = [os.environ.get("TPG_PLAIN_TAIL_MAX_EPILOGUE", "1") != "0"]
+
+
+def set_plain_tail_max_epilogue(flag):
+    prev, PLAIN_TAIL_MAX_EPILOGUE[0] = PLAIN_TAIL_MAX_EPILOGUE[0], bool(flag)
+    return prev
+
+
 class _MlpTailPlain(torch.autograd.Function):
 
     @staticmethod
     def forward(ctx, x0, K, slopes, *Ws):
         be = backend_for(x0)
         L = len(Ws)
+        fold = PLAIN_TAIL_MAX_EPILOGUE[0] and 0 < K <= be.mlp_fwd_max_rows(Ws[-1].shape[1], Ws[-1].shape[0])
         xs = [x0]
-        for l in range(L):
+        for l in range(L - 1 if fold else L):
             y, _ = be.mlp_fwd(xs[-1], None, slopes[l], Ws[l], 1, stats=False)
             xs.append(y)
-        out, arg = be.rowbn_fwd(xs[-1], K, 0.0, 0.0, False, None, None, None, None, slopes[L], None, None, torch.bfloat16)
+        if fold:
+            out, arg = be.mlp_fwd_max(xs[-1], slopes[L - 1], Ws[-1], K, slopes[L])
+        else:
+            out, arg = be.rowbn_fwd(xs[-1], K, 0.0, 0.0, False, None, None, None, None, slopes[L], None, None, torch.bfloat16)
         ctx.save_for_backward(*xs, *Ws, out, arg)
-        ctx.cfg = (K, slopes, L)
+        ctx.cfg = (K, slopes, L, fold)
         return out
 
     @staticmethod
     def backward(ctx, gout):
-        K, slopes, L = ctx.cfg
+        K, slopes, L, fold = ctx.cfg
         t = list(ctx.saved_tensors)
-        xs, Ws, out, arg = t[:L + 1], t[L + 1:2 * L + 1], t[2 * L + 1], t[2 * L + 2]
+        n = L if fold else L + 1
+        xs, Ws, out, arg = t[:n], t[n:n + L], t[n + L], t[n + L + 1]
         be = backend_for(xs[0])
         gout = gout.contiguous()
         if gout.dtype != torch.bfloat16:
             gout = gout.to(torch.bfloat16)
         need = ctx.needs_input_grad
         grads_w = [None] * L
-        cb = _ident_consts(out.shape[1], out.device)[0]
-        g_next, arg_next, K_next = be.mlp_max_prep(gout, out, cb, slopes[L], 1), arg, K
-        for l in range(L, 0, -1):
+        L_dense = L
+        if fold:
+            ci = _ident_consts(xs[L - 1].shape[1], out.device)[1]
+            if need[3 + L - 1]:
+                grads_w[L - 1] = be.mlp_wgrad_max_plain(out, gout, arg, K, slopes[L], xs[L - 1], ci, slopes[L - 1])[0]
+            g_next = None
+            if L > 1 or need[0]:
+                g_next = be.mlp_dgrad_max_plain(out, gout, arg, K, slopes[L], xs[L - 1], ci, slopes[L - 1], Ws[L - 1])
+            arg_next, K_next, L_dense = None, 0, L - 1
+        else:
+            cb = _ident_consts(out.shape[1], out.device)[0]
+            g_next, arg_next, K_next = be.mlp_max_prep(gout, out, cb, slopes[L], 1), arg, K
+        for l in range(L_dense, 0, -1):
             cb = _ident_consts(xs[l].shape[1], out.device)[0]
             ci = _ident_consts(xs[l - 1].shape[1], out.device)[1]
             if need[3 + l - 1]:
```
